# megvii-research/basedet

Hardware: AMD Instinct MI355X
Metric: images/sec training RetinaNet-R50-FPN 1333x800 (higher is better)
Workload: dtype bf16; 1 GPU; retinanet_r50_800x1344 train step (fwd+bwd+allreduce+SGD), DummyLoader boxes, random-init weights, inputs resident in HBM; per_gpu_batch=16, global_batch=16, parallelism=dp1

## Files before the change

### basedet_amd/_lib.py

```python
import ctypes as C
import os

import torch

_HERE = os.path.dirname(os.path.abspath(__file__))
LIB_PATH = os.environ.get("BASEDET_HIP_LIB") or os.path.join(_HERE, "lib", "libbasedet_hip.so")

BD_MAX_SEGS = 8
ABI_VERSION = 106
EPI_RELU, EPI_ADD_BEFORE, EPI_ADD_AFTER, EPI_MASK, EPI_SPARSE = 1, 2, 4, 8, 16


class BasedetHipError(RuntimeError):
    pass


class ConvDesc(C.Structure):
    _fields_ = [
        ("N", C.c_int32), ("Cin", C.c_int32), ("Cout", C.c_int32), ("R", C.c_int32), ("S", C.c_int32),
        ("stride", C.c_int32), ("pad", C.c_int32), ("nseg", C.c_int32),
        ("Hi", C.c_int32 * BD_MAX_SEGS), ("Wi", C.c_int32 * BD_MAX_SEGS),
        ("Ho", C.c_int32 * BD_MAX_SEGS), ("Wo", C.c_int32 * BD_MAX_SEGS),
        ("in_off", C.c_int32 * BD_MAX_SEGS), ("out_off", C.c_int32 * BD_MAX_SEGS),
        ("in_pix_per_img", C.c_int32), ("out_pix_per_img", C.c_int32),
        ("route", C.c_int32 * 4), ("sr_seed", C.c_uint32),
        ("gskip", C.c_int32), ("gskip_ws", C.c_void_p), ("gskip_ws_bytes", C.c_size_t),
        ("gskip_gmap", C.c_void_p), ("gskip_gmap_bytes", C.c_size_t), ("gskip_dxmap", C.c_void_p), ("gskip_dxmap_bytes", C.c_size_t),
        ("gskip_dx_clean", C.c_int32),
    ]


class PackDesc(C.Structure):
    _fields_ = [("w", C.c_void_p), ("row_scale", C.c_void_p), ("w_fwd", C.c_void_p), ("w_dgrad", C.c_void_p),
                ("Cout", C.c_int32), ("RS", C.c_int32), ("Cin", C.c_int32), ("block_start", C.c_int32)]


class ImageDesc(C.Structure):
    _fields_ = [("offset", C.c_int64), ("src_h", C.c_int32), ("src_w", C.c_int32), ("dst_h", C.c_int32), ("dst_w", C.c_int32),
                ("flip", C.c_int32), ("reserved_", C.c_int32 * 1)]


_P, _I, _L, _F, _Z = C.c_void_p, C.c_int, C.c_int64, C.c_float, C.c_size_t
_D = C.POINTER(ConvDesc)

SIGNATURES = {
    "bd_last_error_string": (C.c_char_p, []),
    "bd_version": (_I, []),
    "bd_conv_last_kernel": (C.c_char_p, []),
    "bd_probe_mfma_rate": (_I, [C.c_double, C.POINTER(C.c_double), C.POINTER(C.c_double), _P]),
    "bd_probe_kernel_clock": (_I, [C.c_char_p, _I, C.POINTER(C.c_double), C.POINTER(C.c_double)]),
    "bd_conv2d_fwd": (_I, [_D, _P, _P, _P, _P, _P, _I, _P]),
    "bd_conv2d_dgrad": (_I, [_D, _P, _P, _P, _P, _P, _I, _P]),
    "bd_conv2d_dgrad_gskip_bytes": (_Z, [_D]),
    "bd_conv2d_gskip_map_bytes": (_Z, [_D, _I]),
    "bd_gskip_map_scan": (_I, [_D, _I, _P, _P, _Z, _P]),
    "bd_conv2d_fwd_bits": (_I, [_D, _P, _P, _P, _P, _P, _P, _I, _P]),
    "bd_conv2d_fwd_ex": (_I, [_D, _P, _P, _P, _P, _P, _P, _P, _F, _I, _P]),
    "bd_conv2d_dgrad_ex": (_I, [_D, _P, _P, _P, _P, _P, _P, _P, _F, _I, _P]),
    "bd_conv2d_dgrad_bits": (_I, [_D, _P, _P, _P, _P, _P, _I, _P]),
    "bd_conv2d_wgrad_workspace_bytes": (_Z, [_D]),
    "bd_conv2d_wgrad": (_I, [_D, _P, _P, _P, _P, _I, _P, _Z, _P]),
    "bd_conv2d_wgrad_bias_workspace_bytes": (_Z, [_D]),
    "bd_conv2d_wgrad_bias": (_I, [_D, _P, _P, _P, _P, _P, _I, _P, _Z, _P]),
    "bd_fpn_deconv_pack": (_I, [_P, _I, _P, _P, _P]),
    "bd_fpn_deconv_fwd": (_I, [_P, _P, _P, _P, _I, _I, _I, _I, _I, _I, _P]),
    "bd_fpn_deconv_dgrad": (_I, [_P, _P, _P, _P, _I, _I, _I, _I, _I, _I, _P]),
    "bd_fpn_deconv_wgrad_workspace_bytes": (_Z, [_I, _I, _I, _I]),
    "bd_fpn_deconv_wgrad": (_I, [_P, _P, _P, _I, _P, _Z, _I, _I, _I, _I, _I, _I, _P]),
    "bd_wgrad_queue_create": (_I, [_P]),
    "bd_wgrad_queue_destroy": (_I, [_P]),
    "bd_wgrad_queue_pending": (_I, [_P]),
    "bd_conv2d_wgrad_queued": (_I, [_P, _D, _P, _P, _P, _P, _P, _I, _P, _Z, _P]),
    "bd_wgrad_queue_flush": (_I, [_P, _P]),
    "bd_stem_conv7x7_fwd": (_I, [_I, _I, _I, _P, _P, _P, _P, _P]),
    "bd_stem_pool_fwd": (_I, [_I, _I, _I, _P, _P, _P, _P, _P]),
    "bd_stem_weight_pack": (_I, [_P, _P, _P, _P]),
    "bd_weight_pack": (_I, [_P, _P, _P, _P, _I, _I, _I, _P]),
    "bd_weight_pack_blocks": (_I, [_I, _I, _I]),
    "bd_weight_pack_multi": (_I, [_P, _I, _I, _P]),
    "bd_colsum_workspace_bytes": (_Z, [_I]),
    "bd_colsum_bf16": (_I, [_P, _I, _L, _L, _L, _I, _P, _I, _P, _Z, _P]),
    "bd_pad_normalize": (_I, [_P, _I, _I, _I, _I, _I, _P, _P, _P, _P]),
    "bd_bottleneck_fwd_supported": (_I, [_I, _I, _I, _I, _I, _I, _I]),
    "bd_bottleneck_fwd": (_I, [_I, _I, _I, _I, _I, _I, _P, _P, _P, _P, _P, _P, _P, _P, _P, _P, _P]),
    "bd_h2d_create": (_I, [C.POINTER(C.c_void_p), _I, _I]),
    "bd_h2d_threads": (_I, [_P]),
    "bd_h2d_submit": (_I, [_P, _P, _I, _L, _P, _L, _P]),
    "bd_h2d_destroy": (_I, [_P]),
    "bd_pad_normalize_nchw": (_I, [_P, _I, _I, _I, _I, _I, _P, _P, _P, _P]),
    "bd_resize_pad_normalize": (_I, [_P, _L, C.POINTER(ImageDesc), _I, _I, _I, _P, _P, _P, _P]),
    "bd_maxpool3x3s2_fwd": (_I, [_P, _I, _I, _I, _I, _P, _P]),
    "bd_upsample2x_add_fwd": (_I, [_P, _L, _L, _P, _L, _L, _I, _I, _I, _I, _P]),
    "bd_upsample2x_add_bwd": (_I, [_P, _L, _L, _P, _L, _L, _I, _I, _I, _I, _I, _P]),
    "bd_relu_bf16": (_I, [_P, _P, _L, _P]),
    "bd_relu_bwd_bf16": (_I, [_P, _P, _P, _P, _L, _P]),
    "bd_add_bf16": (_I, [_P, _P, _P, _L, _P]),
    "bd_anchors_generate": (_I, [_I, _I, _I, _F, _P, _I, _P, _P]),
    "bd_points_generate": (_I, [_I, _I, _I, _F, _I, _P, _P]),
    "bd_box_pairwise": (_I, [_P, _I, _P, _I, _I, _P, _P]),
    "bd_box_encode": (_I, [_P, _P, _L, _P, _P, _P, _P]),
    "bd_box_decode": (_I, [_P, _P, _L, _P, _P, _P, _P]),
    "bd_retina_assign_encode": (_I, [_P, _I, _P, _P, _I, _I, _F, _F, _I, _P, _P, _P, _P, _P, _P, _P, _Z, _P]),
    "bd_fcos_assign": (_I, [_P, _I, _P, _P, _P, _I, _F, _P, _P, _I, _I, _P, _P, _P, _P, _P]),
    "bd_ota_assign_workspace_bytes": (_Z, [_I, _I]),
    "bd_ota_assign": (_I, [_P, _I, _P, _P, _I, _P, _I, _P, _P, _P, _I, _I, _F, _F, _F, _F, _I, _P, _P, _P, _P, _P, _Z, _P]),
    "bd_ota_assign_ld": (_I, [_P, _I, _P, _P, _I, _P, _I, _I, _P, _P, _P, _I, _I, _F, _F, _F, _F, _I, _P, _P, _P, _P, _P, _Z, _P]),
    "bd_ota_sinkhorn_workspace_bytes": (_Z, [_I, _I, _I]),
    "bd_ota_assign_sinkhorn": (_I, [_P, _I, _P, _P, _I, _P, _I, _P, _P, _P, _I, _I, _F, _F, _F, _F, _I, _F, _I, _P, _P, _P, _P, _P, _Z, _P]),
    "bd_ota_assign_sinkhorn_ld": (_I, [_P, _I, _P, _P, _I, _P, _I, _I, _P, _P, _P, _I, _I, _F, _F, _F, _F, _I, _F, _I, _P, _P, _P, _P, _P, _Z, _P]),
    "bd_freeanchor_workspace_bytes": (_Z, [_I, _I, _I, _I]),
    "bd_freeanchor_loss_fwd_bwd": (_I, [_P, _P, _I, _I, _P, _I, _I, _P, _P, _I, _I, _P, _P, _F, _I, _F, _F, _F, _F, _P, _P, _P, _P, _Z, _P]),
    "bd_freeanchor_loss_fwd_bwd_ld": (_I, [_P, _I, _P, _I, _I, _P, _I, _I, _P, _P, _I, _I, _P, _P, _F, _I, _F, _F, _F, _F, _P, _P, _P, _P, _Z, _P]),
    "bd_atss_assign_workspace_bytes": (_Z, [_I, _I]),
    "bd_atss_assign": (_I, [_P, _I, _P, _P, _I, _I, _F, _P, _P, _I, _I, _P, _P, _P, _P, _P, _Z, _P]),
    "bd_nms_workspace_bytes": (_Z, [_I]),
    "bd_batched_nms": (_I, [_P, _P, _P, _I, _F, _I, _P, _P, _P, _Z, _P]),
    "bd_focal_loss_fwd_bwd": (_I, [_P, _P, _L, _I, _F, _F, _P, _I, _F, _P, _P, _P]),
    "bd_focal_loss_fwd_bwd_general": (_I, [_P, _P, _L, _I, _F, _F, _P, _I, _F, _P, _P, _P]),
    "bd_focal_loss_fwd_bwd_ld": (_I, [_P, _P, _L, _I, _I, _F, _F, _P, _I, _F, _P, _P, _I, _P]),
    "bd_smooth_l1_fwd_bwd": (_I, [_P, _P, _P, _L, _I, _I, _F, _P, _I, _F, _P, _P, _P]),
    "bd_loss_grid_cap": (_I, []),
    "bd_iou_ltrb_fwd_bwd": (_I, [_P, _P, _P, _P, _L, _I, _P, _F, _P, _P, _P]),
    "bd_giou_ltrb_fwd_bwd": (_I, [_P, _P, _P, _P, _L, _P, _F, _P, _P, _P]),
    "bd_bce_logits_fwd_bwd": (_I, [_P, _I, _I, _P, _P, _L, _P, _P, _P, _P]),
    "bd_groupnorm_workspace_bytes": (_Z, [_I, _I, _I, _L]),
    "bd_groupnorm_fwd": (_I, [_P, _P, _P, _I, _I, _P, _P, _L, _I, _F, _I, _P, _P, _P, _Z, _P]),
    "bd_conv2d_fwd_gnstats_bytes": (_Z, [_D]),
    "bd_conv2d_fwd_gnstats": (_I, [_D, _P, _P, _P, _P, _P, _Z, _P]),
    "bd_groupnorm_fwd_parts": (_I, [_D, _P, _P, _P, _P, _F, _I, _P, _P, _P]),
    "bd_groupnorm_bwd": (_I, [_P, _P, _P, _P, _P, _I, _I, _P, _P, _L, _I, _I, _P, _P, _P, _I, _P, _Z, _P]),
    "bd_fcos_offsets_fwd": (_I, [_P, _I, _P, _I, _I, _P, _P, _P, _L, _P, _P]),
    "bd_fcos_offsets_workspace_bytes": (_Z, []),
    "bd_fcos_offsets_bwd": (_I, [_P, _I, _P, _I, _I, _P, _P, _P, _L, _P, _P, _P, _P, _P, _Z, _P]),
    "bd_rpn_assign_encode": (_I, [_P, _I, _P, _P, _I, _I, _F, _F, _I, _P, _P, _P, _P, _P, _P, _P, _Z, _P]),
    "bd_sample_labels": (_I, [_P, _P, _P, _I, _I, _I, _I, _P, _P]),
    "bd_segment_topk": (_I, [_P, _I, _I, _L, _I, _I, _I, _I, _P, _P, _I, _F, _I, _P, _P, _P, _P]),
    "bd_nms_batched_workspace_bytes": (_Z, [_I, _I]),
    "bd_nms_batched": (_I, [_P, _P, _P, _I, _I, _F, _I, _I, _P, _P, _P, _Z, _P]),
    "bd_rpn_proposals_workspace_bytes": (_Z, [_I, _I, _P, _I, _I, _I]),
    "bd_rpn_proposals": (_I, [_P, _I, _I, _I, _I, _I, _L, _I, _P, _P, _P, _P, _I, _P, _P, _I, _F, _I, _P, _P, _P, _Z, _P]),
    "bd_rpn_proposals_joint": (_I, [_P, _I, _I, _I, _I, _I, _L, _I, _P, _P, _P, _P, _I, _P, _P, _I, _F, _I, _P, _P, _P, _Z, _P]),
    "bd_rcnn_sample_targets": (_I, [_P, _P, _I, _P, _P, _I, _I, _P, _P, _I, _I, _I, _F, _F, _F, _P, _P, _P, _P, _P, _P, _P, _P]),
    "bd_roi_align_fwd": (_I, [_P, _L, _I, _I, _P, _P, _P, _P, _P, _P, _I, _I, _I, _I, _I, _P, _P]),
    "bd_conv1x1_thin_bwd_workspace_bytes": (_Z, []),
    "bd_conv1x1_thin_fwd": (_I, [_P, _P, _P, _L, _I, _I, _P, _P]),
    "bd_conv1x1_thin_bwd": (_I, [_P, _P, _P, _L, _I, _I, _P, _P, _P, _I, _P, _Z, _P]),
    "bd_roi_align_bwd": (_I, [_P, _L, _I, _I, _P, _P, _P, _P, _P, _P, _I, _I, _I, _I, _I, _P, _P]),
    "bd_roi_align_bwd_bf16_workspace_bytes": (_Z, [_I, _I, _P, _P, _I]),
    "bd_roi_align_bwd_bf16": (_I, [_P, _L, _I, _I, _I, _P, _P, _P, _P, _P, _P, _I, _I, _I, _I, _I, _P, _I, _P, _Z, _P]),
    "bd_roi_pool_fwd": (_I, [_P, _L, _I, _I, _P, _P, _P, _P, _P, _P, _I, _I, _I, _I, _P, _P]),
    "bd_roi_pool_bwd_bf16_workspace_bytes": (_Z, [_I, _I, _P, _P, _I]),
    "bd_roi_pool_bwd_bf16": (_I, [_P, _P, _L, _I, _I, _I, _P, _P, _P, _P, _P, _P, _I, _I, _I, _I, _P, _I, _P, _Z, _P]),
    "bd_subsample2x_fwd": (_I, [_P, _L, _L, _I, _I, _P, _L, _L, _I, _I, _P]),
    "bd_subsample2x_bwd_add": (_I, [_P, _L, _L, _P, _L, _L, _I, _I, _I, _I, _P]),
    "bd_f32_to_bf16": (_I, [_P, _P, _L, _P]),
    "bd_f32_to_bf16_add": (_I, [_P, _P, _L, _P]),
    "bd_rpn_loss_fwd_bwd": (_I, [_P, _I, _I, _I, _I, _P, _P, _L, _F, _P, _P, _P, _P]),
    "bd_rcnn_loss_fwd_bwd": (_I, [_P, _I, _I, _I, _P, _P, _I, _F, _P, _P, _P, _P]),
    "bd_det_scores": (_I, [_P, _P, _I, _I, _L, _I, _P, _P]),
    "bd_det_scores_ld": (_I, [_P, _I, _P, _I, _I, _L, _I, _P, _P]),
    "bd_det_select_workspace_bytes": (_Z, [_I, _I, _L, _I, _I]),
    "bd_det_select": (_I, [_P, _P, _I, _I, _I, _L, _I, _I, _P, _P, _I, _F, _P, _P, _P, _P, _Z, _P]),
    "bd_det_select_ld": (_I, [_P, _I, _P, _I, _I, _I, _L, _I, _I, _P, _P, _I, _F, _P, _P, _P, _P, _Z, _P]),
    "bd_rcnn_predict": (_I, [_P, _I, _I, _I, _P, _P, _I, _I, _P, _P, _P, _P, _P]),
    "bd_det_candidates": (_I, [_I, _P, _P, _P, _I, _I, _P, _I, _P, _P, _I, _I, _P, _P, _P, _P, _P, _P, _P]),
    "bd_det_finalize": (_I, [_P, _P, _P, _P, _P, _I, _P, _P, _P, _P, _P]),
    "bd_det_candidates_batched": (_I, [_I, _P, _P, _P, _I, _I, _I, _P, _I, _P, _P, _L, _I, _I, _P, _P, _P, _L, _P, _P, _P, _P]),
    "bd_det_finalize_batched": (_I, [_P, _P, _P, _P, _P, _I, _I, _I, _P, _I, _P, _P, _P, _P]),
    "bd_sgd_momentum_step": (_I, [_P, _P, _P, _L, _F, _F, _F, _F, _P]),
    "bd_ema_update": (_I, [_P, _P, _L, _F, _F, _P]),
    "bd_sgd_momentum_ema_step": (_I, [_P, _P, _P, _P, _L, _F, _F, _F, _F, _F, _F, _P]),
    "bd_swap_f32": (_I, [_P, _P, _L, _P]),
    "bd_adam_step": (_I, [_P, _P, _P, _P, _L] + [_F] * 10 + [_I, _P]),
    "bd_adam_ema_step": (_I, [_P, _P, _P, _P, _P, _L] + [_F] * 10 + [_I, _F, _F, _P]),
    "bd_sgd_nesterov_step": (_I, [_P, _P, _P, _L, _F, _F, _F, _F, _P]),
    "bd_sgd_nesterov_ema_step": (_I, [_P, _P, _P, _P, _L, _F, _F, _F, _F, _F, _F, _P]),
    "bd_clip_grad_value": (_I, [_P, _L, _F, _F, _F, _P]),
    "bd_clip_grad_norm_workspace_bytes": (_Z, []),
    "bd_clip_grad_norm": (_I, [_P, _L, _F, _F, _F, _P, _P, _Z, _P]),
    "bd_quantize_fp8": (_I, [_P, _L, _F, _P, _P]),
    "bd_weight_pack_fp8": (_I, [_P, _P, _I, _I, _I, _F, _P, _P, _P]),
    "bd_conv2d_fwd_fp8": (_I, [_D, _P, _P, _P, _P, _P, _P, _I, _P]),
    "bd_conv2d_fwd_fp8_ex": (_I, [_D, _P, _P, _P, _P, _P, _P, _P, _F, _I, _P]),
    "bd_quantize_bf8": (_I, [_P, _L, _F, _P, C.c_uint32, _P]),
    "bd_absmax_bf16": (_I, [_P, _L, _P, _P]),
    "bd_weight_pack_fp8_t": (_I, [_P, _P, _I, _I, _I, _F, _P, _P, _P]),
    "bd_conv2d_dgrad_fp8": (_I, [_D, _P, _P, _P, _P, _P, _P, _P, _F, _I, _P]),
    "bd_conv2d_wgrad_fp8_workspace_bytes": (_Z, [_D]),
    "bd_conv2d_wgrad_fp8": (_I, [_D, _P, _P, _F, _P, _P, _I, _P, _Z, _P]),
    "bd_conv1x1_fp8": (_I, [_D, _I, _P, _P, _P, _P, _P, _P, _P, _P, _P, _P, _F, _I, _P]),
    "bd_sigmoid_focal_loss_elem": (_I, [_P, _P, _L, _F, _F, _P, _P, _P, _P]),
    "bd_bce_elem": (_I, [_P, _P, _L, _I, _P, _P, _P, _P]),
    "bd_smooth_l1_elem": (_I, [_P, _P, _L, _F, _P, _P, _P, _P]),
    "bd_iou_loss_ltrb": (_I, [_P, _P, _L, _I, _F, _P, _P, _P, _P, _P]),
    "bd_iou_to_loss": (_I, [_P, _L, _I, _F, _P, _P]),
    "bd_matcher_matrix": (_I, [_P, _I, _L, _P, _P, _I, _I, _P, _P, _P, _P]),
    "bd_assign_roi_levels": (_I, [_P, _I, _I, _I, _I, _P, _P]),
    "bd_roi_pool_max_fwd": (_I, [_P, _I, _I, _I, _I, _P, _I, _F, _I, _I, _P, _P]),
    "bd_comm_unique_id": (_I, [_P]),
    "bd_comm_init": (_I, [C.POINTER(C.c_void_p), _P, _I, _I, _I]),
    "bd_comm_rank": (_I, [_P]),
    "bd_comm_world": (_I, [_P]),
    "bd_comm_stream": (_P, [_P]),
    "bd_comm_bcast": (_I, [_P, _P, _Z, _I, _I, _P]),
    "bd_comm_allreduce": (_I, [_P, _P, _Z, _I, _I, _P]),
    "bd_comm_allreduce_async": (_I, [_P, _P, _Z, _I, _I, C.POINTER(C.c_void_p), _I]),
    "bd_comm_allreduce_async_bf16": (_I, [_P, _P, _P, _Z, _I, C.POINTER(C.c_void_p), _I]),
    "bd_comm_wait": (_I, [_P, _P]),
# ... 58 lines not shown
```

### basedet_amd/csrc/common.h

```cpp
#pragma once
#include <hip/hip_runtime.h>
#include <stdint.h>
#include <stdio.h>
#include <mutex>
#include <string>

#include "../../include/basedet_hip.h"

typedef unsigned short bf16_raw;
typedef __attribute__((ext_vector_type(8))) __bf16 bf16x8_t;
typedef __attribute__((ext_vector_type(4))) __bf16 bf16x4_t;
typedef __attribute__((ext_vector_type(4))) float f32x4_t;
typedef __attribute__((ext_vector_type(2))) float f32x2_t;
typedef __attribute__((ext_vector_type(4))) short s16x4_t;
typedef __attribute__((ext_vector_type(4))) unsigned int u32x4_t;
typedef __attribute__((ext_vector_type(2))) unsigned int u32x2_t;

__device__ __forceinline__ float bf2f(bf16_raw h) { return __uint_as_float(((uint32_t)h) << 16); }
__device__ __forceinline__ bf16_raw f2bf(float f) {
    __bf16 b = (__bf16)f;
    return __builtin_bit_cast(bf16_raw, b);
}
extern thread_local unsigned g_fp8_sr_seed;
__device__ __forceinline__ unsigned bd_mix32(unsigned x) {
    x ^= x >> 16; x *= 0x7feb352du; x ^= x >> 15; x *= 0x846ca68bu; x ^= x >> 16;
    return x;
}
__device__ __forceinline__ unsigned bd_pack4_e5m2_sr(float a, float b, float c, float d, unsigned r) {
    a = fminf(fmaxf(a, -57344.f), 57344.f); b = fminf(fmaxf(b, -57344.f), 57344.f);
    c = fminf(fmaxf(c, -57344.f), 57344.f); d = fminf(fmaxf(d, -57344.f), 57344.f);
    int v = 0;
    v = __builtin_amdgcn_cvt_sr_bf8_f32(a, r, v, 0);
    v = __builtin_amdgcn_cvt_sr_bf8_f32(b, __builtin_rotateright32(r, 8), v, 1);
    v = __builtin_amdgcn_cvt_sr_bf8_f32(c, __builtin_rotateright32(r, 16), v, 2);
    v = __builtin_amdgcn_cvt_sr_bf8_f32(d, __builtin_rotateright32(r, 24), v, 3);
    return (unsigned)v;
}

__device__ __forceinline__ unsigned pack4_e4m3(float a, float b, float c, float d) {
    a = fminf(fmaxf(a, -448.f), 448.f); b = fminf(fmaxf(b, -448.f), 448.f);
    c = fminf(fmaxf(c, -448.f), 448.f); d = fminf(fmaxf(d, -448.f), 448.f);
    int v = __builtin_amdgcn_cvt_pk_fp8_f32(a, b, 0, false);
    v = __builtin_amdgcn_cvt_pk_fp8_f32(c, d, v, true);
    return (unsigned)v;
}

__device__ __forceinline__ unsigned pack4_e5m2(float a, float b, float c, float d) {
    a = fminf(fmaxf(a, -57344.f), 57344.f); b = fminf(fmaxf(b, -57344.f), 57344.f);
    c = fminf(fmaxf(c, -57344.f), 57344.f); d = fminf(fmaxf(d, -57344.f), 57344.f);
    int v = __builtin_amdgcn_cvt_pk_bf8_f32(a, b, 0, false);
    v = __builtin_amdgcn_cvt_pk_bf8_f32(c, d, v, true);
    return (unsigned)v;
}

__device__ __forceinline__ u32x2_t e5m2_pair(const float* v, float qs, unsigned seed, long long idx) {
    u32x2_t o8;
    if (seed) {
        const unsigned g0 = (unsigned)(idx >> 2);
        const unsigned r0 = bd_mix32(seed ^ g0);
        o8[0] = bd_pack4_e5m2_sr(v[0] * qs, v[1] * qs, v[2] * qs, v[3] * qs, r0);
        o8[1] = bd_pack4_e5m2_sr(v[4] * qs, v[5] * qs, v[6] * qs, v[7] * qs, r0 * 0x9e3779b1u + 0x7f4a7c15u);
    } else {
        o8[0] = pack4_e5m2(v[0] * qs, v[1] * qs, v[2] * qs, v[3] * qs);
        o8[1] = pack4_e5m2(v[4] * qs, v[5] * qs, v[6] * qs, v[7] * qs);
    }
    return o8;
}

__device__ __forceinline__ u32x4_t twin_pair(u32x2_t h0, u32x2_t h1, int cg, int* off) {
    const bool odd = cg & 1;
    const u32x2_t send = odd ? h0 : h1;
    u32x2_t recv;
    recv[0] = (unsigned)__shfl_xor((int)send[0], 16, 64);
    recv[1] = (unsigned)__shfl_xor((int)send[1], 16, 64);
    *off = odd ? 32 + 8 * (cg - 1) : 8 * cg;
    return odd ? (u32x4_t){recv[0], recv[1], h1[0], h1[1]} : (u32x4_t){h0[0], h0[1], recv[0], recv[1]};
}

__device__ __forceinline__ uint32_t pack_bf2(float lo, float hi) {
    return (uint32_t)f2bf(lo) | ((uint32_t)f2bf(hi) << 16);
}
__device__ __forceinline__ float bf_lo(uint32_t u) { return __uint_as_float(u << 16); }
__device__ __forceinline__ float bf_hi(uint32_t u) { return __uint_as_float(u & 0xffff0000u); }

__device__ __forceinline__ float wave_sum(float v) {
#pragma unroll
    for (int o = 32; o > 0; o >>= 1) v += __shfl_xor(v, o, 64);
    return v;
}

__device__ __forceinline__ float ema_elem(float e, float w, float m, float one_minus_m) {
#pragma clang fp contract(off)
    const float a = e * m;
    const float b = one_minus_m * w;
    return a + b;
}

__device__ __forceinline__ void bd_clk_mark(unsigned long long* acc, bool end) {
#ifdef BD_NO_CLK_PROBE
    return;
#endif
    const unsigned long long c = __builtin_amdgcn_s_memtime(), r = __builtin_amdgcn_s_memrealtime();
    atomicAdd(acc, end ? c : 0ull - c);
    atomicAdd(acc + 1, end ? r : 0ull - r);
}

#define BD_KNOB thread_local
struct BdRouteScope {
    int rc;
    explicit BdRouteScope(const bd_conv_desc* d);
};
#define BD_ROUTE(d)                                   \
    BdRouteScope route_scope__(d);                    \
    if (route_scope__.rc != BD_OK) return route_scope__.rc

void bd_set_error(const char* fmt, ...);
void bd_note_kernel(const char* name);

#define BD_REQUIRE(cond, ...)            \
    do {                                 \
        if (!(cond)) {                   \
            bd_set_error(__VA_ARGS__);   \
            return BD_EINVAL;            \
        }                                \
    } while (0)

#define BD_CHECK_LAUNCH(name)                                                     \
    do {                                                                          \
        hipError_t e__ = hipGetLastError();                                       \
        if (e__ != hipSuccess) {                                                  \
            bd_set_error("%s: launch failed: %s", name, hipGetErrorString(e__)); \
            return BD_ELAUNCH;                                                    \
        }                                                                         \
    } while (0)

#ifdef BD_TUNING
#include <stdlib.h>
static inline int bd_tune_env(const char* name, int dflt) { const char* e = getenv(name); return e ? atoi(e) : dflt; }
static inline const char* bd_tune_env_str(const char* name) { return getenv(name); }
#else
static inline int bd_tune_env(const char*, int dflt) { return dflt; }
static inline const char* bd_tune_env_str(const char*) { return nullptr; }
#endif

struct BdGskipMap { int p4, p8, m4, m8, live, list; size_t ints; };
void bd_gskip_map_layout(const bd_conv_desc* d, int side, BdGskipMap* out);

static inline int grid_for(long long n, int block = 256, int cap = 4096) {
    long long g = (n + block - 1) / block;
    if (g < 1) g = 1;
    return (int)(g < cap ? g : cap);
}
static inline int64_t cdiv64(int64_t a, int64_t b) { return (a + b - 1) / b; }
static inline int cdiv(int a, int b) { return (a + b - 1) / b; }

struct BdDeviceOnce {
    std::mutex mu;
    unsigned long long done[4] = {0, 0, 0, 0};
    struct Guard {
        BdDeviceOnce& o; int dev = 0; bool first_;
        explicit Guard(BdDeviceOnce& o_) : o(o_) {
            o.mu.lock();
            if (hipGetDevice(&dev) != hipSuccess || dev < 0 || dev > 255) dev = 0;
            first_ = !((o.done[dev >> 6] >> (dev & 63)) & 1ull);
        }
        bool first() const { return first_; }
        ~Guard() { if (first_) o.done[dev >> 6] |= 1ull << (dev & 63); o.mu.unlock(); }
    };
};
#define BD_ONCE_PER_DEVICE(...)                 \
    do {                                        \
        static BdDeviceOnce once__;             \
        BdDeviceOnce::Guard guard__(once__);    \
        if (guard__.first()) { __VA_ARGS__; }   \
    } while (0)
int bd_num_cus();
```

### basedet_amd/csrc/conv3x3_pp.hip

```cpp
#include "conv3x3_pp128_body.h"

namespace {

constexpr int PH = 4, PW = 16, IH = PH + 2, IW = PW + 2;
constexpr int NPATCH = 4;
constexpr int XROWS = NPATCH * IH * IW;
constexpr int X_PITCH = 144;
constexpr int X_BYTES = XROWS * X_PITCH;
constexpr int XPASSES = 7;
constexpr int TILE_CO = 256;
constexpr int W_SLOT = TILE_CO * 128;
constexpr int NSLOT = 3;
constexpr int W_BYTES = NSLOT * W_SLOT;
constexpr int GTAB_TILES = 16;
constexpr int GTAB_BYTES = GTAB_TILES * NPATCH * 32;
constexpr int LDS_BYTES = W_BYTES + X_BYTES + TILE_CO * 4 + GTAB_BYTES;
constexpr int MAX_SEG = BD_MAX_SEGS;
constexpr int TAIL_CO = 64;

struct PSeg { int patch_start, H, W, pw, src_off, dst_off; float inv_pw; };

struct PParams {
    const bf16_raw* src;
    const bf16_raw* w;
    const float* bias;
    const bf16_raw* add;
    const bf16_raw* mask;
    bf16_raw* dst;
    int CK, CO, flags, nseg;
    int src_ppi, dst_ppi;
    unsigned src_bytes;
    int patches_per_img, total_patches, n_tiles;
    int main_grid;
    int px_tiles;
    int tail_end;
    float inv_ppi;
    PSeg seg[MAX_SEG];
    float* gn_part;
    const int* sp_live;
    const int* sp_list;
    const int* sp_count;
    int sp_keep_dead;
    const int* sp_hdr;
    int* sp_ohdr;
    const int* sp_olist;
    int sp_stride, sp_clean;
};

typedef __attribute__((address_space(3))) void lds_void_t;
typedef __attribute__((address_space(1))) const void glb_void_t;

__device__ __forceinline__ int pp_div(int n, int d, float inv) {
    int q = (int)((float)n * inv);
    const int r = n - q * d;
    q += (r >= d) - (r < 0);
    return q;
}

__device__ __forceinline__ int swz(int row, int chunk) { return row * 128 + ((chunk ^ (row & 7)) << 4); }
__device__ __forceinline__ int colperm(int f) { return f < 4 ? 2 * f : (f < 12 ? 2 * (f - 4) + 1 : 2 * (f - 8)); }
__device__ __forceinline__ int xpos(int chunk) { return (chunk >> 2) * 64 + ((((chunk & 1) << 1) | ((chunk >> 1) & 1)) << 4); }

#ifdef BD_PP_STAMP
__device__ unsigned long long g_pp_stamp[64];
__device__ unsigned long long g_pp_span[2048];
#endif
#ifndef BD_PP_ABLATE
#define BD_PP_ABLATE 0
#endif
__device__ unsigned long long g_pp_clk[2];
#define PP_FENCE() __builtin_amdgcn_sched_barrier(0)
#define PP_BARRIER() do { asm volatile("" ::: "memory"); __builtin_amdgcn_s_barrier(); asm volatile("" ::: "memory"); } while (0)

template <int MODE, bool GNS = false, bool SPARSE = false>
__global__ __launch_bounds__(512, 1) void conv3x3_pp_kernel(const PParams p) {
    extern __shared__ __attribute__((aligned(16))) unsigned char smem[];
    if (!SPARSE && (int)blockIdx.x >= p.main_grid) {
        pp128::body<MODE, TAIL_CO>(p, smem, (int)blockIdx.x - p.main_grid, (int)gridDim.x - p.main_grid, p.total_patches, p.tail_end,
                                   (p.CO + TAIL_CO - 1) / TAIL_CO);
        return;
    }
    if (!SPARSE && blockIdx.x == 0 && threadIdx.x == 0) bd_clk_mark(g_pp_clk, false);
    unsigned char* wbuf = smem;
    unsigned char* xbuf = smem + W_BYTES;
    float* sbias = reinterpret_cast<float*>(smem + W_BYTES + X_BYTES);

#ifdef BD_PP_STAMP
    int st_n = 0;
    const bool st_on = blockIdx.x == 100 % gridDim.x && threadIdx.x == 0;
#define PP_STAMP() do { if (st_on && st_n < 62) g_pp_stamp[st_n] = __builtin_amdgcn_s_memtime(); ++st_n; } while (0)
    PP_STAMP();
    if (st_on) g_pp_stamp[62] = __builtin_amdgcn_s_memrealtime();
    if (threadIdx.x == 0 && blockIdx.x < 1024) g_pp_span[2 * blockIdx.x] = __builtin_amdgcn_s_memrealtime();
#else
#define PP_STAMP() do { } while (0)
#endif
    const int tid = threadIdx.x, lane = tid & 63, wave = __builtin_amdgcn_readfirstlane(tid >> 6);
    const int wm = wave >> 2, wp = wave & 3;
    int bid = blockIdx.x;
    {
        const int nwg = p.main_grid;
        const int q = nwg >> 3, r = nwg & 7, xcd = bid & 7;
        bid = (xcd < r ? xcd * (q + 1) : r * (q + 1) + (xcd - r) * q) + (bid >> 3);
    }
    const int ct = bid % p.n_tiles;
    int pt = bid / p.n_tiles;
    const int pt_step = p.main_grid / p.n_tiles;
    const int co0 = ct * TILE_CO;

    auto zero_dead = [&](int z0, int zn) {
        if (p.sp_keep_dead) return;
        const int cpp = p.CO >> 3;
        const int items = PH * PW * cpp;
        int zt = p.total_patches;
        const int* plist = nullptr;
        if (p.sp_clean) {
            const int oc = __builtin_amdgcn_readfirstlane(p.sp_ohdr[0]) & 1;
            const int pc = __builtin_amdgcn_readfirstlane(p.sp_ohdr[2 + oc]);
            zt = pc < 0 ? 0 : (pc < zt ? pc : zt);
            plist = p.sp_olist + oc * p.sp_stride;
        }
        for (int k0 = 0; z0 + k0 * zn < zt; k0 += 512) {
            const int k = k0 + wave * 64 + lane;
            const int idx = z0 + k * zn;
            int q = idx;
            if (plist) q = idx < zt ? plist[idx] : -1;
            const bool dead = idx < zt && q >= 0 && q < p.total_patches && p.sp_live[q] == 0;
            unsigned long long m = __ballot(dead);
            while (m) {
                const int l = __builtin_ctzll(m);
                m &= m - 1;
                const int qq = __builtin_amdgcn_readfirstlane(__shfl(q, l, 64));
                const int n = qq / p.patches_per_img, rem = qq - n * p.patches_per_img;
                int sgi = 0;
#pragma unroll
                for (int z = 1; z < MAX_SEG; ++z)
                    if (z < p.nseg && rem >= p.seg[z].patch_start) sgi = z;
                const int H = p.seg[sgi].H, W = p.seg[sgi].W, pwn = p.seg[sgi].pw;
                const int local = rem - p.seg[sgi].patch_start, by = local / pwn, bx = local - by * pwn;
                const long long img = (long long)n * p.dst_ppi + p.seg[sgi].dst_off;
                for (int i = lane; i < items; i += 64) {
                    const int px = i / cpp, ch = i - px * cpp;
                    const int y = by * PH + px / PW, x = bx * PW + (px & (PW - 1));
                    if (y < H && x < W)
                        *reinterpret_cast<u32x4_t*>(p.dst + (img + (long long)y * W + x) * p.CO + ch * 8) = (u32x4_t){0u, 0u, 0u, 0u};
                }
            }
        }
    };
    int n_px = p.px_tiles, n_live = p.total_patches;
    int z_first = 0;
    const int* sp_list = p.sp_list;
    if constexpr (SPARSE) {
        if (p.sp_ohdr && blockIdx.x == 0 && threadIdx.x == 0) p.sp_ohdr[1] = 0;
        const int cur = p.sp_hdr ? __builtin_amdgcn_readfirstlane(p.sp_hdr[0]) & 1 : 0;
        const int* cntp = p.sp_hdr ? p.sp_hdr + 2 + cur : p.sp_count;
        n_live = __builtin_amdgcn_readfirstlane(*cntp);
        sp_list += cur * p.sp_stride;
        n_live = __builtin_amdgcn_readfirstlane(n_live < 0 ? 0 : (n_live < p.total_patches ? n_live : p.total_patches));
        n_px = (n_live + NPATCH - 1) / NPATCH;
        z_first = n_px * p.n_tiles < p.main_grid ? n_px * p.n_tiles : p.main_grid;
        if (pt >= n_px) {
            zero_dead(bid - z_first, p.main_grid - z_first);
            return;
        }
    }

    constexpr unsigned X_NONE = 0x80000000u;
    const int x_lds0 = (tid >> 3) * X_PITCH + xpos(tid & 7);
    unsigned x_off[XPASSES];

    int* gtab = reinterpret_cast<int*>(smem + W_BYTES + X_BYTES + TILE_CO * 4);
    const int pt_first = pt;
    auto build_table = [&](int k0) {
        const int k = k0 + (lane >> 2);
        const int ptile = pt_first + k * pt_step;
        int pid = ptile * NPATCH + (lane & (NPATCH - 1));
        if (SPARSE) pid = (ptile < n_px && pid < n_live) ? sp_list[pid] : p.total_patches;
        int vH = 0, vW = 0, vy = 0, vx = 0, vs = 0, vd = 0;
        if (ptile < n_px && pid < p.total_patches) {
            const int n = pp_div(pid, p.patches_per_img, p.inv_ppi);
            const int rem = pid - n * p.patches_per_img;
            int g_start = p.seg[0].patch_start, g_H = p.seg[0].H, g_W = p.seg[0].W, g_pw = p.seg[0].pw;
            int g_src = p.seg[0].src_off, g_dst = p.seg[0].dst_off;
            float g_inv = p.seg[0].inv_pw;
#pragma unroll
            for (int q = 1; q < MAX_SEG; ++q) {
                const bool in = q < p.nseg && rem >= p.seg[q].patch_start;
                g_start = in ? p.seg[q].patch_start : g_start; g_H = in ? p.seg[q].H : g_H; g_W = in ? p.seg[q].W : g_W;
                g_pw = in ? p.seg[q].pw : g_pw; g_src = in ? p.seg[q].src_off : g_src; g_dst = in ? p.seg[q].dst_off : g_dst;
                g_inv = in ? p.seg[q].inv_pw : g_inv;
            }
            const int local = rem - g_start;
            const int by = pp_div(local, g_pw, g_inv), bx = local - by * g_pw;
            vy = by * PH; vx = bx * PW; vH = g_H; vW = g_W;
            vs = n * p.src_ppi + g_src;
            vd = n * p.dst_ppi + g_dst;
        }
        typedef __attribute__((ext_vector_type(4))) int i32x4_t;
        i32x4_t* e = reinterpret_cast<i32x4_t*>(gtab + ((k & (GTAB_TILES - 1)) * NPATCH + (lane & (NPATCH - 1))) * 8);
        e[0] = (i32x4_t){vy, vx, vH, vW};
        e[1] = (i32x4_t){vs, vd, 0, 0};
    };
    auto decode = [&](int k, int& e_oy0, int& e_px0, int& e_H, int& e_W, int& e_dst) {
        int py0[NPATCH], px0[NPATCH], pH[NPATCH], pWd[NPATCH];
        int psrc[NPATCH], pdst[NPATCH];
        int tq = tid;
        asm volatile("" : "+v"(tq));
        {
            typedef __attribute__((ext_vector_type(4))) int i32x4_t;
            const i32x4_t* e = reinterpret_cast<const i32x4_t*>(gtab + ((k & (GTAB_TILES - 1)) * NPATCH + (tq & (NPATCH - 1))) * 8);
            const i32x4_t e0 = e[0], e1 = e[1];
#pragma unroll
            for (int q = 0; q < NPATCH; ++q) {
                py0[q] = __builtin_amdgcn_readlane(e0[0], q); px0[q] = __builtin_amdgcn_readlane(e0[1], q);
                pH[q] = __builtin_amdgcn_readlane(e0[2], q); pWd[q] = __builtin_amdgcn_readlane(e0[3], q);
                psrc[q] = __builtin_amdgcn_readlane(e1[0], q); pdst[q] = __builtin_amdgcn_readlane(e1[1], q);
            }
        }
#pragma unroll
        for (int k = 0; k < XPASSES; ++k) {
            const int row = (tq >> 3) + 64 * k;
            unsigned off = X_NONE;
            if (row < XROWS) {
                const int lo = (64 * k) / (IH * IW), hi = (64 * k + 63) / (IH * IW) < NPATCH ? (64 * k + 63) / (IH * IW) : NPATCH - 1;
                const bool up = row >= hi * (IH * IW);
                const int pk = up ? hi : lo;
                const int rr = row - pk * (IH * IW);
                const int iy = rr / IW, ix = rr - iy * IW;
                const int qy = up ? py0[hi] : py0[lo], qx = up ? px0[hi] : px0[lo], H = up ? pH[hi] : pH[lo];
                const int W = up ? pWd[hi] : pWd[lo], qs = up ? psrc[hi] : psrc[lo];
                const int y = qy - 1 + iy, x = qx - 1 + ix;
                if (y >= 0 && x >= 0 && y < H && x < W) off = (unsigned)((qs + y * W + x) * p.CK + (tq & 7) * 8) * 2u;
            }
            x_off[k] = off;
        }
        e_oy0 = py0[0]; e_px0 = px0[0]; e_H = pH[0]; e_W = pWd[0]; e_dst = pdst[0];
#pragma unroll
        for (int q = 1; q < NPATCH; ++q)
            if (wp == q) { e_oy0 = py0[q]; e_px0 = px0[q]; e_H = pH[q]; e_W = pWd[q]; e_dst = pdst[q]; }
    };
    int c_oy0, c_px0, c_H, c_W, c_dst;
    int kt = 0;
    if (wave == 0) build_table(0);
    asm volatile("s_waitcnt lgkmcnt(0)" ::: "memory");
    PP_BARRIER();
    decode(0, c_oy0, c_px0, c_H, c_W, c_dst);
    const __amdgpu_buffer_rsrc_t x_rsrc =
        __builtin_amdgcn_make_buffer_rsrc(const_cast<bf16_raw*>(p.src), 0, p.src_bytes, 0x00020000);
    u32x4_t rx[XPASSES];
    auto load_x = [&](int cb) {
        int so = cb * 128;
        asm volatile("" : "+s"(so));
        const bool dead = cb * 64 + (tid & 7) * 8 >= p.CK;
#pragma unroll
        for (int k = 0; k < XPASSES; ++k) rx[k] = __builtin_amdgcn_raw_buffer_load_b128(x_rsrc, dead ? X_NONE : x_off[k], so, 0);
    };
    auto write_x = [&]() {
#pragma unroll
        for (int k = 0; k < XPASSES; ++k)
            if (k < XPASSES - 1 || (tid >> 3) + 64 * k < XROWS)
                *reinterpret_cast<u32x4_t*>(xbuf + x_lds0 + k * (64 * X_PITCH)) = rx[k];
    };

    unsigned dma_src[4];
#pragma unroll
    for (int k = 0; k < 4; ++k) {
        const int pc = wave + 8 * k;
        const int lrow = 8 * pc + (lane >> 3);
        const int chunk = (lane & 7) ^ (lane >> 3);
        const int rho = lrow & 15;
        int co = co0 + (lrow & 192) + 32 * ((lrow >> 5) & 1) + 8 * (rho >> 2) + 4 * ((lrow >> 4) & 1) + (rho & 3);
        if (co >= p.CO) co = p.CO - 1;
        dma_src[k] = (unsigned)(co * 9 * p.CK + chunk * 8) * 2u;
    }
    const __amdgpu_buffer_rsrc_t w_rsrc =
        __builtin_amdgcn_make_buffer_rsrc(const_cast<bf16_raw*>(p.w), 0, (unsigned)(p.CO * 9 * p.CK) * 2u, 0x00020000);
    bool dma_on = true;
    auto dma_piece = [&](int tap, int cb, int slot, int k) {
        if ((BD_PP_ABLATE & 2) && !dma_on) return;
        unsigned char* l = wbuf + slot * W_SLOT + (wave + 8 * k) * 1024;
        int so = (tap * p.CK + cb * 64) * 2;
        asm volatile("" : "+s"(so));
        __builtin_amdgcn_raw_ptr_buffer_load_lds(w_rsrc, (lds_void_t*)l, 16, dma_src[k], so, 0, 0);
    };

    f32x4_t acc[8][4];

    const int frow = lane & 15, fchunk = lane >> 4;
    const unsigned char* a_base[2];
#pragma unroll
    for (int kk = 0; kk < 2; ++kk) a_base[kk] = wbuf + swz(wm * 128 + frow, kk * 4 + fchunk);
    typedef __attribute__((address_space(3))) const unsigned char lds_u8_t;
    typedef __attribute__((address_space(3))) const bf16x8_t lds_bf16x8_t;
    unsigned a_hi[2];
#pragma unroll
    for (int kk = 0; kk < 2; ++kk) {
        a_hi[kk] = (unsigned)(size_t)(lds_u8_t*)(a_base[kk]) + 2 * W_SLOT;
        asm volatile("" : "+v"(a_hi[kk]));
    }
    const unsigned char* b_base = xbuf + (wp * (IH * IW) + colperm(frow)) * X_PITCH + xpos(fchunk);

    bf16x8_t fa[8], fb[4];
    auto load_a = [&](int kk, int slot) {
#pragma unroll
        for (int i = 0; i < 8; ++i) {
            if (slot == 2) fa[i] = *(lds_bf16x8_t*)(size_t)(a_hi[kk] + i * 2048);
// ... 194 lines not shown
                PP_STAMP();
                if (more) asm volatile("s_waitcnt vmcnt(4)" ::: "memory");
                else asm volatile("s_waitcnt vmcnt(0)" ::: "memory");
                PP_STAMP();
                PP_FENCE();
#pragma unroll
                for (int j = 0; j < 4; ++j) {
                    if (BD_PP_ABLATE & 4) asm volatile("" :: "v"(o0[j]));
                    else if (okh && okj[j]) *reinterpret_cast<u32x4_t*>(drow[j]) = o0[j];
                }
            } else {
#pragma unroll
                for (int j = 0; j < 4; ++j) {
                    const u32x4_t o = unit(h, j, b0, b1);
                    if (BD_PP_ABLATE & 4) asm volatile("" :: "v"(o));
                    else if (okh && okj[j]) *reinterpret_cast<u32x4_t*>(drow[j] + 32 * h) = o;
                }
            }
        }
        if constexpr (GNS) {
            const int pid = pt * NPATCH + wp;
#pragma unroll
            for (int h = 0; h < 4; ++h) {
                float a = gsum[h], b = gsq[h];
#pragma unroll
                for (int m = 8; m >= 1; m >>= 1) { a += __shfl_xor(a, m, 64); b += __shfl_xor(b, m, 64); }
                if (erow == 0 && pid < p.total_patches && cbase + 32 * h < p.CO) {
                    float* o = p.gn_part + ((long long)pid * 32 + ((cbase + 32 * h) >> 3)) * 2;
                    *reinterpret_cast<f32x2_t*>(o) = (f32x2_t){a, b};
                }
            }
        }
    } else {
    if (more) {
#pragma unroll
        for (int k = 0; k < 4; ++k) dma_piece(2, 0, 2, k);
    }
    long long erow_off[4];
#pragma unroll
    for (int j = 0; j < 4; ++j) erow_off[j] = (long long)(dbase + (oy0 + j) * W + ox) * p.CO + cbase;
#pragma unroll
    for (int hp = 0; hp < 2; ++hp) {
        u32x4_t av[2][4], mv[2][4];
#pragma unroll
        for (int hh = 0; hh < 2; ++hh) {
            const int h = 2 * hp + hh;
#pragma unroll
            for (int j = 0; j < 4; ++j) {
                const int oy = oy0 + j;
                const bool ok = cbase + 32 * h < p.CO && oy < H && ox < W;
                const long long idx = erow_off[j] + 32 * h;
                av[hh][j] = (u32x4_t){0u, 0u, 0u, 0u}; mv[hh][j] = (u32x4_t){0u, 0u, 0u, 0u};
                if (ok && (add_before || add_after)) av[hh][j] = *reinterpret_cast<const u32x4_t*>(p.add + idx);
                if (ok && do_mask) mv[hh][j] = *reinterpret_cast<const u32x4_t*>(p.mask + idx);
            }
        }
        if (hp == 0) asm volatile("s_waitcnt vmcnt(0)" ::: "memory");
#pragma unroll
        for (int hh = 0; hh < 2; ++hh) {
            const int h = 2 * hp + hh;
            if (cbase + 32 * h >= p.CO) continue;
            float bias[8];
            {
                const f32x4_t b0 = *reinterpret_cast<const f32x4_t*>(sbias + wm * 128 + 8 * cg + 32 * h);
                const f32x4_t b1 = *reinterpret_cast<const f32x4_t*>(sbias + wm * 128 + 8 * cg + 32 * h + 4);
#pragma unroll
                for (int k = 0; k < 4; ++k) { bias[k] = b0[k]; bias[4 + k] = b1[k]; }
            }
#pragma unroll
            for (int j = 0; j < 4; ++j) {
                const int oy = oy0 + j;
                if (oy >= H || ox >= W) continue;
                const long long idx = erow_off[j] + 32 * h;
                float v[8];
#pragma unroll
                for (int k = 0; k < 8; ++k) v[k] = acc[2 * h + (k >> 2)][j][k & 3] + bias[k];
                const u32x4_t a4 = av[hh][j], m4 = mv[hh][j];
                if (add_before) {
#pragma unroll
                    for (int k = 0; k < 4; ++k) { v[2 * k] += bf_lo(a4[k]); v[2 * k + 1] += bf_hi(a4[k]); }
                }
                if (do_relu) {
#pragma unroll
                    for (int k = 0; k < 8; ++k) v[k] = fmaxf(v[k], 0.f);
                }
                if (do_mask) {
#pragma unroll
                    for (int k = 0; k < 4; ++k) {
                        if (!(bf_lo(m4[k]) > 0.f)) v[2 * k] = 0.f;
                        if (!(bf_hi(m4[k]) > 0.f)) v[2 * k + 1] = 0.f;
                    }
                }
                if (add_after) {
#pragma unroll
                    for (int k = 0; k < 4; ++k) { v[2 * k] += bf_lo(a4[k]); v[2 * k + 1] += bf_hi(a4[k]); }
                }
                u32x4_t o;
#pragma unroll
                for (int k = 0; k < 4; ++k) o[k] = pack_bf2(v[2 * k], v[2 * k + 1]);
                *reinterpret_cast<u32x4_t*>(p.dst + idx) = o;
            }
        }
    }
    }
    PP_STAMP();
    if (!more) break;
    ++kt;
    pt = pt_next;
    c_oy0 = n_oy0; c_px0 = n_px0; c_H = n_H; c_W = n_W; c_dst = n_dst;
    PP_FENCE();
    PP_STAMP();
    }
    if constexpr (SPARSE) {
        if (z_first == p.main_grid) zero_dead(bid, p.main_grid);
    }
    if (!SPARSE && blockIdx.x == 0 && threadIdx.x == 0) bd_clk_mark(g_pp_clk, true);
#ifdef BD_PP_STAMP
    if (st_on) { g_pp_stamp[63] = __builtin_amdgcn_s_memrealtime(); g_pp_stamp[61] = __builtin_amdgcn_s_memtime(); }
    if (threadIdx.x == 0 && blockIdx.x < 1024) { asm volatile("s_waitcnt vmcnt(0)" ::: "memory"); g_pp_span[2 * blockIdx.x + 1] = __builtin_amdgcn_s_memrealtime(); }
#endif
}

}

BD_KNOB int g_pp_tail_split = 1;
BD_KNOB int g_pp_persistent = 1;
extern BD_KNOB int g_patch_pp;
int bd_gskip_patches(const bd_conv_desc* d, int ph, int pw);
void bd_gskip_fill(const bd_conv_desc* d, int side, const void* t, const int* live_in, int* map, hipStream_t stream);
void bd_gskip_scan(const bd_conv_desc* d, const void* g, int ph, int pw, int* mask, hipStream_t stream);
void bd_gskip_compact(const bd_conv_desc* d, int ph, int pw, const int* mask, int* live, int* list, int* count, hipStream_t stream);

extern "C" size_t bd_conv2d_dgrad_gskip_bytes(const bd_conv_desc* d) {
    if (!d || d->nseg < 1 || d->nseg > BD_MAX_SEGS || !(d->R == 3 && d->S == 3 && d->stride == 1 && d->pad == 1)) return 0;
    return ((size_t)3 * bd_gskip_patches(d, PH, PW) + 4) * sizeof(int);
}

static bool pp_sparse_epilogue(int flags, const void* add, const void* dst) {
    const bool in_place = (flags & BD_EPI_ADD_BEFORE) && add && add == dst;
    return !(flags & BD_EPI_ADD_AFTER) && (!((flags & BD_EPI_ADD_BEFORE) && add) || (in_place && !(flags & BD_EPI_MASK)));
}

bool bd_conv3x3_pp_maps_ok(const bd_conv_desc* d, int flags, const void* add, const void* dst) {
    if (g_patch_pp < 2 || !(d->R == 3 && d->S == 3 && d->stride == 1 && d->pad == 1)) return false;
    if (d->Cout % 8 != 0 || d->Cin <= 128 || d->Cin % 8 != 0) return false;
    if ((long long)d->N * d->out_pix_per_img * d->Cout * 2 >= 0x7fffffffll || (long long)d->N * d->in_pix_per_img >= 0x7fffffffll ||
        (long long)d->Cin * 9 * d->Cout >= 0x7fffffffll) return false;
    for (int s = 0; s < d->nseg; ++s)
        if (d->Hi[s] != d->Ho[s] || d->Wi[s] != d->Wo[s]) return false;
    if (bd_gskip_patches(d, PH, PW) >= (1 << 24)) return false;
    const bool in_place = (flags & BD_EPI_ADD_BEFORE) && add && add == dst;
    if (d->gskip_dxmap && in_place) return false;
    return pp_sparse_epilogue(flags, add, dst);
}

static int pp_launch(const bd_conv_desc* d, int mode, const void* src, const void* w, const float* bias, const void* add,
                     const void* mask, void* dst, int flags, float* gn_part, hipStream_t stream) {
    PParams p{};
    p.gn_part = gn_part;
    p.CK = mode == 0 ? d->Cin : d->Cout;
    p.CO = mode == 0 ? d->Cout : d->Cin;
    p.src_ppi = mode == 0 ? d->in_pix_per_img : d->out_pix_per_img;
    p.dst_ppi = mode == 0 ? d->out_pix_per_img : d->in_pix_per_img;
    if (p.CK % 8 != 0 || p.CO <= 128 || p.CO % 8 != 0) return 1;
    if ((long long)d->N * p.src_ppi * p.CK * 2 >= 0x7fffffffll || (long long)d->N * p.dst_ppi >= 0x7fffffffll ||
        (long long)p.CO * 9 * p.CK >= 0x7fffffffll) return 1;
    p.src = (const bf16_raw*)src; p.w = (const bf16_raw*)w; p.bias = bias;
    p.add = (const bf16_raw*)add; p.mask = (const bf16_raw*)mask; p.dst = (bf16_raw*)dst;
    p.flags = flags; p.nseg = d->nseg;
    p.src_bytes = (unsigned)((long long)d->N * p.src_ppi * p.CK * 2);
    int ps = 0;
    for (int s = 0; s < d->nseg; ++s) {
        PSeg& sg = p.seg[s];
        sg.patch_start = ps; sg.H = d->Ho[s]; sg.W = d->Wo[s]; sg.pw = cdiv(d->Wo[s], PW); sg.inv_pw = 1.0f / (float)sg.pw;
        sg.src_off = mode == 0 ? d->in_off[s] : d->out_off[s];
        sg.dst_off = mode == 0 ? d->out_off[s] : d->in_off[s];
        ps += cdiv(d->Ho[s], PH) * sg.pw;
    }
    p.patches_per_img = ps;
    p.inv_ppi = 1.0f / (float)ps;
    p.total_patches = ps * d->N;
    if (p.total_patches >= (1 << 24)) return 1;
    p.n_tiles = cdiv(p.CO, TILE_CO);
    int grid = cdiv(p.total_patches, NPATCH) * p.n_tiles;
    int tail_wgs = 0;
    int px_tiles = cdiv(p.total_patches, NPATCH);
    p.tail_end = p.total_patches;
    const int num_cus = bd_num_cus();
    const bool in_place = (flags & BD_EPI_ADD_BEFORE) && add && add == dst;
    const bool sparse = mode == 1 && d->gskip && !gn_part && pp_sparse_epilogue(flags, add, dst);
    if (g_pp_tail_split && !sparse && !gn_part && p.n_tiles == 1 && px_tiles > num_cus) {
        const int r = px_tiles % num_cus;
        if (r > 0 && r * (TILE_CO / TAIL_CO) <= num_cus) {
            px_tiles -= r;
            p.total_patches = px_tiles * NPATCH;
            tail_wgs = cdiv(p.tail_end - p.total_patches, NPATCH) * cdiv(p.CO, TAIL_CO);
        }
    }
    p.px_tiles = px_tiles;
    p.main_grid = px_tiles * p.n_tiles;
    if (g_pp_persistent) {
        const int g1 = (num_cus / p.n_tiles) * p.n_tiles;
        const int rounds = cdiv(px_tiles * p.n_tiles, g1 * GTAB_TILES);
        if (g1 * rounds < p.main_grid) p.main_grid = g1 * rounds;
    }
    {
        const int grid128 = cdiv(p.total_patches, NPATCH) * cdiv(p.CO, 128);
        if (!gn_part && g_patch_pp < 2 && 3 * cdiv(grid, 256) >= 2 * cdiv(grid128, 256)) return 1;
    }
    BD_ONCE_PER_DEVICE(
        (void)hipFuncSetAttribute(reinterpret_cast<const void*>(&conv3x3_pp_kernel<0>), hipFuncAttributeMaxDynamicSharedMemorySize, LDS_BYTES);
        (void)hipFuncSetAttribute(reinterpret_cast<const void*>(&conv3x3_pp_kernel<1>), hipFuncAttributeMaxDynamicSharedMemorySize, LDS_BYTES);
        (void)hipFuncSetAttribute(reinterpret_cast<const void*>(&conv3x3_pp_kernel<1, false, true>), hipFuncAttributeMaxDynamicSharedMemorySize,
                                  LDS_BYTES));
    bd_note_kernel("conv3x3_pp_kernel");
    if (sparse) {
        const int tot = p.total_patches;
        p.sp_keep_dead = in_place ? 1 : 0;
        p.sp_stride = tot;
        if (d->gskip_gmap) {
            BdGskipMap gm;
            bd_gskip_map_layout(d, 0, &gm);
            const int* m = (const int*)d->gskip_gmap;
            p.sp_hdr = m; p.sp_live = m + gm.live; p.sp_list = m + gm.list;
        } else {
            int* mk = (int*)d->gskip_ws;
            p.sp_live = mk + tot; p.sp_list = mk + 2 * tot; p.sp_count = mk + 3 * tot;
            bd_gskip_scan(d, src, PH, PW, mk, stream);
            bd_gskip_compact(d, PH, PW, mk, mk + tot, mk + 2 * tot, mk + 3 * tot, stream);
        }
        if (d->gskip_dxmap) {
            BdGskipMap xm;
            bd_gskip_map_layout(d, 1, &xm);
            p.sp_ohdr = (int*)d->gskip_dxmap; p.sp_olist = p.sp_ohdr + xm.list;
            p.sp_clean = d->gskip_dx_clean ? 1 : 0;
        }
        hipLaunchKernelGGL((conv3x3_pp_kernel<1, false, true>), dim3(p.main_grid), dim3(512), LDS_BYTES, stream, p);
        if (d->gskip_dxmap) bd_gskip_fill(d, 1, dst, p.sp_live, (int*)d->gskip_dxmap, stream);
    } else if (gn_part) {
        BD_ONCE_PER_DEVICE((void)hipFuncSetAttribute(reinterpret_cast<const void*>(&conv3x3_pp_kernel<0, true>), hipFuncAttributeMaxDynamicSharedMemorySize, LDS_BYTES));
        hipLaunchKernelGGL((conv3x3_pp_kernel<0, true>), dim3(p.main_grid), dim3(512), LDS_BYTES, stream, p);
    } else if (mode == 0) hipLaunchKernelGGL((conv3x3_pp_kernel<0>), dim3(p.main_grid + tail_wgs), dim3(512), LDS_BYTES, stream, p);
    else hipLaunchKernelGGL((conv3x3_pp_kernel<1>), dim3(p.main_grid + tail_wgs), dim3(512), LDS_BYTES, stream, p);
    return 0;
}

int bd_pp_clk_read(unsigned long long* out2, int reset) {
    if (hipMemcpyFromSymbol(out2, HIP_SYMBOL(g_pp_clk), 16) != hipSuccess) return 1;
    if (reset) { const unsigned long long z[2] = {0, 0}; if (hipMemcpyToSymbol(HIP_SYMBOL(g_pp_clk), z, 16) != hipSuccess) return 1; }
    return 0;
}

#ifdef BD_PP_STAMP
extern "C" int bd_debug_pp_stamp(unsigned long long* out2) {
    return hipMemcpyFromSymbol(out2, HIP_SYMBOL(g_pp_stamp), 512) == hipSuccess ? 0 : 1;
}
extern "C" int bd_debug_pp_span(unsigned long long* out2048) {
    return hipMemcpyFromSymbol(out2048, HIP_SYMBOL(g_pp_span), 2048 * 8) == hipSuccess ? 0 : 1;
}
#endif

int bd_conv3x3_pp_launch(const bd_conv_desc* d, int mode, const void* src, const void* w, const float* bias, const void* add,
                         const void* mask, void* dst, int flags, hipStream_t stream) {
    return pp_launch(d, mode, src, w, bias, add, mask, dst, flags, nullptr, stream);
}

int bd_conv3x3_pp_patch_starts(const bd_conv_desc* d, int* starts) {
    int ps = 0;
    for (int s = 0; s < d->nseg; ++s) { starts[s] = ps; ps += cdiv(d->Ho[s], PH) * cdiv(d->Wo[s], PW); }
    starts[d->nseg] = ps;
    return ps;
}

extern "C" size_t bd_conv2d_fwd_gnstats_bytes(const bd_conv_desc* d) {
    if (!d || d->nseg < 1 || d->nseg > BD_MAX_SEGS) return 0;
    int starts[BD_MAX_SEGS + 1];
    return (size_t)d->N * bd_conv3x3_pp_patch_starts(d, starts) * 32 * 2 * sizeof(float);
}

extern "C" int bd_conv2d_fwd_gnstats(const bd_conv_desc* d, const void* x, const void* w_packed, const float* bias, void* y, float* part,
                                     size_t part_bytes, bd_stream_t stream) {
    BD_ROUTE(d);
    BD_REQUIRE(d && x && w_packed && y && part, "conv2d_fwd_gnstats: null pointer");
    BD_REQUIRE(d->R == 3 && d->S == 3 && d->stride == 1 && d->pad == 1 && d->Cout == 256 && d->Cin % 64 == 0,
               "conv2d_fwd_gnstats: 3x3 / stride 1 / pad 1 into 256 channels (GroupNorm(32, 256)) only; got %dx%d s%d p%d %d -> %d", d->R, d->S,
               d->stride, d->pad, d->Cin, d->Cout);
    for (int s = 0; s < d->nseg; ++s)
        BD_REQUIRE(d->Hi[s] == d->Ho[s] && d->Wi[s] == d->Wo[s], "conv2d_fwd_gnstats: level %d changes size", s);
    if (part_bytes < bd_conv2d_fwd_gnstats_bytes(d)) { bd_set_error("conv2d_fwd_gnstats: statistics buffer too small"); return BD_EWORKSPACE; }
    if (pp_launch(d, 0, x, w_packed, bias, nullptr, nullptr, y, 0, part, (hipStream_t)stream) != 0) {
        bd_set_error("conv2d_fwd_gnstats: shape not taken by conv3x3_pp_kernel (tensor too large for 32-bit offsets?)");
        return BD_EINVAL;
    }
    BD_CHECK_LAUNCH("bd_conv2d_fwd_gnstats");
    return BD_OK;
}
```

### basedet_amd/csrc/conv_igemm.hip

```cpp
#include "igemm_params.h"

using namespace igemm;

namespace {

template <int BK>
struct Cfg {
    static constexpr int CHUNKS = BK / 8;
    static constexpr int ROWS_PER_PASS = 256 / CHUNKS;
    static constexpr int PASSES = 128 / ROWS_PER_PASS;
    static constexpr int LDS_STRIDE = BK == 64 ? 160 : 64;
    static constexpr int TILE_BYTES = 128 * LDS_STRIDE;
    __device__ static __forceinline__ int off(int row, int chunk) {
        if constexpr (BK == 64) return row * LDS_STRIDE + chunk * 16;
        else return row * 64 + ((chunk ^ ((row >> 1) & 3)) << 4);
    }
};

template <int BK, bool PRE, bool BUF>
__global__ __launch_bounds__(256) void conv_igemm_kernel(const IgemmParams p) {
    using C = Cfg<BK>;
    extern __shared__ __attribute__((aligned(16))) unsigned char smem[];
    unsigned char* tiles = smem;
    unsigned int* s_tapmask = reinterpret_cast<unsigned int*>(smem);
// ... 234 lines not shown
    }
    __syncthreads();
    int cur = 0;
    for (int t = 0; t < nsteps; ++t) {
        const bool more = (t + 1 < nsteps);
        if (more) stage_load();
        compute(cur);
        if (more) stage_write(cur ^ 1);
        __syncthreads();
        cur ^= 1;
    }

    const int cg = lane >> 4;
    const bool do_relu = p.flags & BD_EPI_RELU;
    const bool add_before = (p.flags & BD_EPI_ADD_BEFORE) && p.add;
    const bool add_after = (p.flags & BD_EPI_ADD_AFTER) && p.add;
    const bool do_mask = (p.flags & BD_EPI_MASK) && p.mask;
    const int cbase = co0 + wc * 64 + 8 * cg;
    float bias[16];
#pragma unroll
    for (int k = 0; k < 16; ++k) bias[k] = 0.f;
    if (p.bias) {
#pragma unroll
        for (int q = 0; q < 4; ++q)
            if (cbase + 32 * (q >> 1) + 4 * (q & 1) < p.CO) {
                const f32x4_t bv = *reinterpret_cast<const f32x4_t*>(p.bias + cbase + 32 * (q >> 1) + 4 * (q & 1));
                bias[4 * q] = bv[0]; bias[4 * q + 1] = bv[1]; bias[4 * q + 2] = bv[2]; bias[4 * q + 3] = bv[3];
            }
    }
#pragma unroll
    for (int j = 0; j < 4; ++j) {
        const int m = m0 + wp * 64 + j * 16 + (lane & 15);
        if (m >= p.M) continue;
        int dstpix;
        if (p.linear_dst) dstpix = m;
        else {
            int s = 0;
#pragma unroll
            for (int k = 1; k < MAX_SUB; ++k)
                if (k < p.nsub && m >= p.sub[k].m_start) s = k;
            const SubSeg ss = p.sub[s];
            const int local = m - ss.m_start;
            int n, rem, yy, xx;
            fast_divmod(local, ss.Hs * ss.Ws, ss.inv_per_img, n, rem);
            fast_divmod(rem, ss.Ws, ss.inv_ws, yy, xx);
            dstpix = n * p.dst_pix_per_img + ss.dst_off + (ss.y0 + ss.step * yy) * ss.Wd + ss.x0 + ss.step * xx;
        }
        const long long base = (long long)dstpix * p.CO + cbase;
#pragma unroll
        for (int half = 0; half < 2; ++half) {
            if (cbase + 32 * half >= p.CO) continue;
            const long long idx = base + 32 * half;
            float v[8];
#pragma unroll
            for (int k = 0; k < 8; ++k) v[k] = acc[2 * half + (k >> 2)][j][k & 3] + bias[8 * half + k];
            if (add_before) {
                const u32x4_t av = PRE ? pre_add[j * 2 + half] : *reinterpret_cast<const u32x4_t*>(p.add + idx);
#pragma unroll
                for (int k = 0; k < 4; ++k) { v[2 * k] += bf_lo(av[k]); v[2 * k + 1] += bf_hi(av[k]); }
            }
            if (do_relu) {
#pragma unroll
                for (int k = 0; k < 8; ++k) v[k] = fmaxf(v[k], 0.f);
            }
            if (do_mask) {
                const u32x4_t mv = PRE ? pre_mask[j * 2 + half] : *reinterpret_cast<const u32x4_t*>(p.mask + idx);
#pragma unroll
                for (int k = 0; k < 4; ++k) {
                    if (!(bf_lo(mv[k]) > 0.f)) v[2 * k] = 0.f;
                    if (!(bf_hi(mv[k]) > 0.f)) v[2 * k + 1] = 0.f;
                }
            }
            if (add_after) {
                const u32x4_t av = PRE ? pre_add[j * 2 + half] : *reinterpret_cast<const u32x4_t*>(p.add + idx);
#pragma unroll
                for (int k = 0; k < 4; ++k) { v[2 * k] += bf_lo(av[k]); v[2 * k + 1] += bf_hi(av[k]); }
            }
            u32x4_t o;
#pragma unroll
            for (int k = 0; k < 4; ++k) o[k] = pack_bf2(v[2 * k], v[2 * k + 1]);
            *reinterpret_cast<u32x4_t*>(p.dst + idx) = o;
        }
    }
}

BD_KNOB int g_igemm_prefetch_epi = 1;
BD_KNOB int g_igemm_buf = 1;

template <int BK>
int launch_igemm(const IgemmParams& p, hipStream_t stream) {
    using C = Cfg<BK>;
    const size_t lds = 4 * C::TILE_BYTES;
    BD_ONCE_PER_DEVICE(
        (void)hipFuncSetAttribute(reinterpret_cast<const void*>(&conv_igemm_kernel<BK, false, false>),
                                  hipFuncAttributeMaxDynamicSharedMemorySize, (int)lds);
        (void)hipFuncSetAttribute(reinterpret_cast<const void*>(&conv_igemm_kernel<BK, true, false>),
                                  hipFuncAttributeMaxDynamicSharedMemorySize, (int)lds);
        (void)hipFuncSetAttribute(reinterpret_cast<const void*>(&conv_igemm_kernel<BK, false, true>),
                                  hipFuncAttributeMaxDynamicSharedMemorySize, (int)lds);
        (void)hipFuncSetAttribute(reinterpret_cast<const void*>(&conv_igemm_kernel<BK, true, true>),
                                  hipFuncAttributeMaxDynamicSharedMemorySize, (int)lds));
    const int grid = p.m_tiles * p.n_tiles;
    bd_note_kernel(BK == 32 ? "conv_igemm_kernel<32>" : "conv_igemm_kernel<64>");
    const bool epi_ops = ((p.flags & (BD_EPI_ADD_BEFORE | BD_EPI_ADD_AFTER)) && p.add) || ((p.flags & BD_EPI_MASK) && p.mask);
    const int ksteps = (p.CK + BK - 1) / BK * p.R * p.S;
    const bool pre = g_igemm_prefetch_epi && p.linear_dst && epi_ops && ksteps <= 4;
    const bool buf = g_igemm_buf && p.src_bytes != 0 && p.w_bytes != 0;
    if (pre && buf) hipLaunchKernelGGL((conv_igemm_kernel<BK, true, true>), dim3(grid), dim3(256), lds, stream, p);
    else if (pre) hipLaunchKernelGGL((conv_igemm_kernel<BK, true, false>), dim3(grid), dim3(256), lds, stream, p);
    else if (buf) hipLaunchKernelGGL((conv_igemm_kernel<BK, false, true>), dim3(grid), dim3(256), lds, stream, p);
    else hipLaunchKernelGGL((conv_igemm_kernel<BK, false, false>), dim3(grid), dim3(256), lds, stream, p);
    return 0;
}

int check_desc(const bd_conv_desc* d) {
    BD_REQUIRE(d != nullptr, "conv: null descriptor");
    BD_REQUIRE(d->nseg >= 1 && d->nseg <= BD_MAX_SEGS, "conv: nseg=%d out of range", d->nseg);
    BD_REQUIRE(d->N >= 1 && d->Cin >= 1 && d->Cout >= 1, "conv: bad N/Cin/Cout");
    BD_REQUIRE(d->stride == 1 || d->stride == 2, "conv: stride %d unsupported (1 or 2)", d->stride);
    BD_REQUIRE(d->R * d->S <= 32, "conv: %dx%d kernel unsupported by the generic path", d->R, d->S);
    for (int s = 0; s < d->nseg; ++s) {
        BD_REQUIRE((d->Hi[s] + 2 * d->pad - d->R) / d->stride + 1 == d->Ho[s] &&
                   (d->Wi[s] + 2 * d->pad - d->S) / d->stride + 1 == d->Wo[s],
                   "conv: level %d output size inconsistent with input/stride/pad", s);
    }
    return 0;
}

void set_buffer_sizes(IgemmParams& p, int N) {
    const long long sb = (long long)N * p.src_pix_per_img * p.CK * 2, wb = (long long)p.CO * p.R * p.S * p.CK * 2;
    p.src_bytes = (sb > 0 && sb < 0x7fffffffll) ? (unsigned)sb : 0u;
    p.w_bytes = (wb > 0 && wb < 0x7fffffffll) ? (unsigned)wb : 0u;
}

bool is_3x3s1(const bd_conv_desc* d) {
    if (!(d->R == 3 && d->S == 3 && d->stride == 1 && d->pad == 1)) return false;
    for (int s = 0; s < d->nseg; ++s)
        if (d->Hi[s] != d->Ho[s] || d->Wi[s] != d->Wo[s]) return false;
    return true;
}
BD_KNOB int g_use_patch3x3 = 1;
#ifdef BD_AB_SKIP
BD_KNOB int g_skip_s2_3x3 = 0;
#endif
BD_KNOB int g_bk32_for_1x1 = 1;
BD_KNOB int g_bk32_s2 = 1;

}


int bd_conv3x3_patch_launch(const bd_conv_desc* d, int mode, const void* src, const void* w, const float* bias,
                            const void* add, const void* mask, void* dst, int flags, hipStream_t stream);
bool bd_conv3x3_pp_maps_ok(const bd_conv_desc* d, int flags, const void* add, const void* dst);

extern BD_KNOB int g_patch_dma;
extern BD_KNOB int g_patch_pp;
extern BD_KNOB int g_patch_pp128;
extern BD_KNOB int g_conv1x1_s2;
extern BD_KNOB int g_pp_tail_split;
extern BD_KNOB int g_pp_persistent;
static int bd_route_patch3x3(int enable) {
#ifdef BD_AB_SKIP
    g_skip_s2_3x3 = (enable >> 4) & 1;
#else
    if ((enable >> 4) & 1) {
        bd_set_error("bd_conv_desc.route[1]: bit 4 (skip the 3x3 / stride-2 launches: a timing A/B that leaves stale outputs) exists in "
                     "-DBD_AB_SKIP diagnostic builds only");
        return BD_EINVAL;
    }
#endif
    g_use_patch3x3 = enable & 1; g_bk32_for_1x1 = (enable >> 1) & 1;
    g_patch_dma = ((enable >> 3) & 1) ^ 1;
    g_patch_pp = ((enable >> 6) & 1) ? 0 : (((enable >> 7) & 1) ? 1 : 2);
    g_patch_pp128 = ((enable >> 9) & 1) ? -1 : ((enable >> 8) & 1);
    g_bk32_s2 = ((enable >> 10) & 1) ^ 1;
    g_igemm_prefetch_epi = ((enable >> 5) & 1) ^ 1;
    g_igemm_buf = ((enable >> 11) & 1) ^ 1;
    g_conv1x1_s2 = ((enable >> 12) & 1) ^ 1;
    g_pp_tail_split = ((enable >> 13) & 1) ^ 1;
    g_pp_persistent = ((enable >> 14) & 1) ^ 1;
    if ((enable >> 16) & 1) {
        bd_set_error("bd_conv_desc.route[1]: bit 16 (conv_igemm_wide.hip) is gone since round 6");
        return BD_EINVAL;
    }
    return BD_OK;
}

int bd_route_dense1x1(int depth);
int bd_route_wgrad(int use_tr);
extern BD_KNOB int g_fp8_patch;

BdRouteScope::BdRouteScope(const bd_conv_desc* d) : rc(BD_OK) {
    const int r0 = d ? d->route[0] : 0, r1 = d ? d->route[1] : 0, r2 = d ? d->route[2] : 0, r3 = d ? d->route[3] : 0;
    if (r0 < 0 || r1 < 0 || r2 < 0 || r3 < 0) {
        bd_set_error("bd_conv_desc.route: negative word (0 = the library's choice, otherwise the route + 1)");
        rc = BD_EINVAL;
        return;
    }
    if ((rc = bd_route_dense1x1(r0 ? r0 - 1 : 1)) != BD_OK) return;
    if ((rc = bd_route_patch3x3(r1 ? r1 - 1 : 3)) != BD_OK) return;
    if ((rc = bd_route_wgrad(r2 ? r2 - 1 : 1)) != BD_OK) return;
    g_fp8_patch = r3 ? (r3 - 1 != 0) : 1;
    g_fp8_sr_seed = d ? d->sr_seed : 0u;
}

int bd_conv1x1_dense_launch(const void* x, const void* w, const float* bias, const void* add, const void* mask, const unsigned* maskbits,
                            void* y, unsigned* ybits, void* y8, float q_scale, int y8_bf8, long long M, int CK, int CO, int flags,
                            hipStream_t stream);

int bd_conv1x1_s2_launch(const bd_conv_desc* d, int mode, const void* src, const void* w, const float* bias, const void* add, const void* mask,
                         const unsigned* maskbits, void* dst, int flags, hipStream_t stream);
namespace {
bool is_dense_1x1(const bd_conv_desc* d) {
    return d->R == 1 && d->S == 1 && d->stride == 1 && d->pad == 0 && d->nseg == 1 && d->in_off[0] == 0 && d->out_off[0] == 0 &&
           d->in_pix_per_img == d->Hi[0] * d->Wi[0] && d->out_pix_per_img == d->Ho[0] * d->Wo[0];
}
}

static int conv2d_fwd_impl(const bd_conv_desc* d, const void* x, const void* w_packed, const float* bias, const void* add, void* y,
                           unsigned* ybits, void* y8, float q_scale, int flags, bd_stream_t stream) {
    if (int e = check_desc(d)) return e;
    BD_REQUIRE(x && w_packed && y, "conv2d_fwd: null pointer");
    BD_REQUIRE(d->Cin % 8 == 0, "conv2d_fwd: Cin=%d must be a multiple of 8", d->Cin);
    BD_REQUIRE(d->Cout % 8 == 0, "conv2d_fwd: Cout=%d must be a multiple of 8", d->Cout);
    BD_REQUIRE(!(flags & BD_EPI_MASK), "conv2d_fwd: BD_EPI_MASK is a dgrad-only flag");
    if (is_dense_1x1(d) &&
        bd_conv1x1_dense_launch(x, w_packed, bias, add, nullptr, nullptr, y, ybits, y8, q_scale, 0, (long long)d->N * d->out_pix_per_img,
                                d->Cin, d->Cout, flags, (hipStream_t)stream) == 0) {
        BD_CHECK_LAUNCH("bd_conv2d_fwd(dense 1x1)");
        return BD_OK;
    }
    if (!ybits && !y8 && d->stride == 2 && d->R == 1 &&
        bd_conv1x1_s2_launch(d, 0, x, w_packed, bias, add, nullptr, nullptr, y, flags, (hipStream_t)stream) == 0) {
        BD_CHECK_LAUNCH("bd_conv2d_fwd(1x1 stride 2)");
        return BD_OK;
    }
    BD_REQUIRE(ybits == nullptr && y8 == nullptr, "conv2d_fwd_bits / _ex: the bit-packed ReLU mask and the e4m3 twin are written by the dense "
               "1x1 kernel only (1x1 / stride 1 over one dense level, Cout %% 32 == 0, tensors < 2 GB)");
#ifdef BD_AB_SKIP
    if (g_skip_s2_3x3 && d->R == 3 && d->S == 3 && d->stride == 2) return BD_OK;
#endif
    if (g_use_patch3x3 && is_3x3s1(d)) {
        bd_conv3x3_patch_launch(d, 0, x, w_packed, bias, add, nullptr, y, flags, (hipStream_t)stream);
        BD_CHECK_LAUNCH("bd_conv2d_fwd(3x3 patch)");
        return BD_OK;
    }
    IgemmParams p{};
    p.src = (const bf16_raw*)x; p.w = (const bf16_raw*)w_packed; p.bias = bias;
    p.add = (const bf16_raw*)add; p.mask = nullptr; p.dst = (bf16_raw*)y;
    p.CK = d->Cin; p.CO = d->Cout; p.R = d->R; p.S = d->S; p.stride = d->stride; p.pad = d->pad;
    p.mode = 0; p.flags = flags;
    p.nsub = d->nseg;
    long long m = 0;
    for (int s = 0; s < d->nseg; ++s) {
        SubSeg& ss = p.sub[s];
        ss.m_start = (int)m;
        ss.Hs = d->Ho[s]; ss.Ws = d->Wo[s]; ss.y0 = 0; ss.x0 = 0; ss.step = 1;
        ss.Wd = d->Wo[s]; ss.dst_off = d->out_off[s];
        ss.Hsrc = d->Hi[s]; ss.Wsrc = d->Wi[s]; ss.src_off = d->in_off[s];
        ss.inv_per_img = 1.0f / (float)(ss.Hs * ss.Ws); ss.inv_ws = 1.0f / (float)ss.Ws;
        m += (long long)d->N * d->Ho[s] * d->Wo[s];
    }
    BD_REQUIRE(m < (1ll << 24), "conv2d_fwd: too many pixels (2^24 limit of the fast index decode)");
    p.linear_dst = (d->nseg == 1 && d->out_off[0] == 0 && d->out_pix_per_img == d->Ho[0] * d->Wo[0]) ? 1 : 0;
    p.linear_src = (p.linear_dst && d->R == 1 && d->S == 1 && d->stride == 1 && d->pad == 0 && d->in_off[0] == 0 &&
                    d->in_pix_per_img == d->Hi[0] * d->Wi[0]) ? 1 : 0;
    p.M = (int)m;
    p.src_pix_per_img = d->in_pix_per_img; p.dst_pix_per_img = d->out_pix_per_img;
    set_buffer_sizes(p, d->N);
    p.m_tiles = cdiv(p.M, TILE_P); p.n_tiles = cdiv(p.CO, TILE_C);
    if (p.CK > 32 && !(g_bk32_for_1x1 && p.R * p.S == 1) && !(g_bk32_s2 && p.stride == 2 && p.m_tiles * p.n_tiles >= 512))
        launch_igemm<64>(p, (hipStream_t)stream);
    else launch_igemm<32>(p, (hipStream_t)stream);
    BD_CHECK_LAUNCH("bd_conv2d_fwd");
    return BD_OK;
}

extern "C" int bd_conv2d_fwd(const bd_conv_desc* d, const void* x, const void* w_packed, const float* bias,
                             const void* add, void* y, int flags, bd_stream_t stream) {
    BD_ROUTE(d);
    return conv2d_fwd_impl(d, x, w_packed, bias, add, y, nullptr, nullptr, 1.f, flags, stream);
}

extern "C" int bd_conv2d_fwd_ex(const bd_conv_desc* d, const void* x, const void* w_packed, const float* bias, const void* add, void* y,
                                uint32_t* ybits, void* y8, float q_scale, int flags, bd_stream_t stream) {
    BD_ROUTE(d);
    return conv2d_fwd_impl(d, x, w_packed, bias, add, y, ybits, y8, q_scale, flags, stream);
}

extern "C" int bd_conv2d_fwd_bits(const bd_conv_desc* d, const void* x, const void* w_packed, const float* bias, const void* add, void* y,
                                  uint32_t* ybits, int flags, bd_stream_t stream) {
    BD_ROUTE(d);
    BD_REQUIRE(ybits != nullptr, "conv2d_fwd_bits: null ybits");
    return conv2d_fwd_impl(d, x, w_packed, bias, add, y, ybits, nullptr, 1.f, flags, stream);
}

static int conv2d_dgrad_impl(const bd_conv_desc* d, const void* g, const void* w_packed_t, const void* add, const void* mask,
                             const unsigned* maskbits, void* dx, void* dx8, float q_scale, int flags, bd_stream_t stream) {
    if (int e = check_desc(d)) return e;
    BD_REQUIRE(g && w_packed_t && dx, "conv2d_dgrad: null pointer");
    if (d->gskip && is_3x3s1(d) && !d->gskip_gmap) {
        const size_t need = bd_conv2d_dgrad_gskip_bytes(d);
        BD_REQUIRE(d->gskip_ws && d->gskip_ws_bytes >= need, "conv2d_dgrad: gskip scratch %zu < required %zu bytes (or NULL)",
                   (size_t)d->gskip_ws_bytes, need);
    }
    if (d->gskip_gmap || d->gskip_dxmap || d->gskip_dx_clean) {
        BD_REQUIRE(d->gskip && is_3x3s1(d) && g_use_patch3x3 && !maskbits && !dx8 && bd_conv3x3_pp_maps_ok(d, flags, add, dx),
                   "conv2d_dgrad: liveness maps need gskip on a 3x3 / stride 1 / pad 1 descriptor into more than 128 channels with an overwriting "
                   "(or, without gskip_dxmap, in-place accumulating) epilogue on the default route");
        BD_REQUIRE(!d->gskip_gmap || d->gskip_gmap_bytes >= bd_conv2d_gskip_map_bytes(d, 0), "conv2d_dgrad: gskip_gmap %zu < required %zu bytes",
                   (size_t)d->gskip_gmap_bytes, bd_conv2d_gskip_map_bytes(d, 0));
        BD_REQUIRE(!d->gskip_dxmap || d->gskip_dxmap_bytes >= bd_conv2d_gskip_map_bytes(d, 1), "conv2d_dgrad: gskip_dxmap %zu < required %zu bytes",
                   (size_t)d->gskip_dxmap_bytes, bd_conv2d_gskip_map_bytes(d, 1));
        BD_REQUIRE(!d->gskip_dx_clean || d->gskip_dxmap, "conv2d_dgrad: gskip_dx_clean needs gskip_dxmap (the list the promise refers to)");
    }
    if (d->stride == 1) flags &= ~BD_EPI_SPARSE;
    BD_REQUIRE(d->Cout % 8 == 0, "conv2d_dgrad: Cout=%d must be a multiple of 8 (pad the gradient)", d->Cout);
    BD_REQUIRE(d->Cin % 8 == 0, "conv2d_dgrad: Cin=%d must be a multiple of 8", d->Cin);
    BD_REQUIRE(!(flags & BD_EPI_RELU), "conv2d_dgrad: BD_EPI_RELU is a forward-only flag");
    if (is_dense_1x1(d) &&
        bd_conv1x1_dense_launch(g, w_packed_t, nullptr, add, mask, maskbits, dx, nullptr, dx8, q_scale, 1, (long long)d->N * d->in_pix_per_img,
                                d->Cout, d->Cin, flags, (hipStream_t)stream) == 0) {
        BD_CHECK_LAUNCH("bd_conv2d_dgrad(dense 1x1)");
        return BD_OK;
    }
    if (!dx8 && d->stride == 2 && d->R == 1 &&
        bd_conv1x1_s2_launch(d, 1, g, w_packed_t, nullptr, add, mask, maskbits, dx, flags, (hipStream_t)stream) == 0) {
        BD_CHECK_LAUNCH("bd_conv2d_dgrad(1x1 stride 2)");
        return BD_OK;
    }
    BD_REQUIRE(maskbits == nullptr && dx8 == nullptr, "conv2d_dgrad_bits / _ex: the bit-packed ReLU mask is read, and the e5m2 twin written, by "
               "the dense 1x1 kernel only (1x1 / stride 1 over one dense level, Cin %% 32 == 0, tensors < 2 GB)");
#ifdef BD_AB_SKIP
    if (g_skip_s2_3x3 && d->R == 3 && d->S == 3 && d->stride == 2) return BD_OK;
#endif
    if (g_use_patch3x3 && is_3x3s1(d)) {
        bd_conv3x3_patch_launch(d, 1, g, w_packed_t, nullptr, add, mask, dx, flags, (hipStream_t)stream);
        BD_CHECK_LAUNCH("bd_conv2d_dgrad(3x3 patch)");
        return BD_OK;
    }
    IgemmParams p{};
    p.src = (const bf16_raw*)g; p.w = (const bf16_raw*)w_packed_t; p.bias = nullptr;
    p.add = (const bf16_raw*)add; p.mask = (const bf16_raw*)mask; p.dst = (bf16_raw*)dx;
    p.CK = d->Cout; p.CO = d->Cin; p.R = d->R; p.S = d->S; p.stride = d->stride; p.pad = d->pad;
    p.mode = 1; p.flags = flags;
    long long m = 0;
    int ns = 0;
    const int st = d->stride;
    const bool sparse = (flags & BD_EPI_SPARSE) && st > 1;
    BD_REQUIRE(!(flags & BD_EPI_SPARSE) || ((flags & BD_EPI_ADD_BEFORE) && add == dx),
               "conv2d_dgrad: BD_EPI_SPARSE needs an in-place accumulate (BD_EPI_ADD_BEFORE with add == dx)");
    p.flags = flags & ~BD_EPI_SPARSE;
    for (int s = 0; s < d->nseg; ++s) {
        for (int qy = 0; qy < st; ++qy)
            for (int qx = 0; qx < st; ++qx) {
                const int Hs = (d->Hi[s] - qy + st - 1) / st, Ws = (d->Wi[s] - qx + st - 1) / st;
                if (Hs <= 0 || Ws <= 0) continue;
                if (sparse) {
                    bool ry = false, rx = false;
                    for (int r = 0; r < d->R; ++r) ry = ry || ((qy + d->pad - r) % st + st) % st == 0;
                    for (int c = 0; c < d->S; ++c) rx = rx || ((qx + d->pad - c) % st + st) % st == 0;
                    if (!(ry && rx)) continue;
                }
                BD_REQUIRE(ns < MAX_SUB, "conv2d_dgrad: too many sub-segments (levels x stride^2 > %d)", MAX_SUB);
                SubSeg& ss = p.sub[ns++];
                ss.m_start = (int)m;
                ss.Hs = Hs; ss.Ws = Ws; ss.y0 = qy; ss.x0 = qx; ss.step = st;
                ss.Wd = d->Wi[s]; ss.dst_off = d->in_off[s];
                ss.Hsrc = d->Ho[s]; ss.Wsrc = d->Wo[s]; ss.src_off = d->out_off[s];
                ss.inv_per_img = 1.0f / (float)(Hs * Ws); ss.inv_ws = 1.0f / (float)Ws;
                m += (long long)d->N * Hs * Ws;
            }
    }
    p.nsub = ns;
    BD_REQUIRE(m < (1ll << 24), "conv2d_dgrad: too many pixels (2^24 limit of the fast index decode)");
    p.linear_dst = (d->nseg == 1 && st == 1 && d->in_off[0] == 0 && d->in_pix_per_img == d->Hi[0] * d->Wi[0]) ? 1 : 0;
    p.linear_src = (p.linear_dst && d->R == 1 && d->S == 1 && d->pad == 0 && d->out_off[0] == 0 &&
                    d->out_pix_per_img == d->Ho[0] * d->Wo[0]) ? 1 : 0;
// ... 31 lines not shown
```

### basedet_amd/csrc/gskip.hip

```cpp
#include "common.h"

namespace {

enum { GS_ANY = 1, GS_TOP = 2, GS_BOT = 4, GS_LEFT = 8, GS_RIGHT = 16, GS_TL = 32, GS_TR = 64, GS_BL = 128, GS_BR = 256 };

struct GsSeg { int patch_start, H, W, pw, off; };

struct GsParams {
    const bf16_raw* g;
    int* mask;
    int C, ppi, ph, pw_px, nseg, patches_per_img, total;
    GsSeg seg[BD_MAX_SEGS];
};

__device__ __forceinline__ int gs_level(const GsParams& p, int rem) {
    int s = 0;
#pragma unroll
    for (int k = 1; k < BD_MAX_SEGS; ++k)
        if (k < p.nseg && rem >= p.seg[k].patch_start) s = k;
    return s;
}

__global__ __launch_bounds__(256) void gskip_scan_kernel(const GsParams p) {
    __shared__ int sbits;
// ... 56 lines not shown
__device__ __forceinline__ void gs_compact_body(const GsParams& p, int* live, int* list, int* count, int* wsum) {
    constexpr int KP = 8;
    const int tid = threadIdx.x, wv = tid >> 6, ln = tid & 63;
    int base = 0;
    for (int c0 = 0; c0 < p.total; c0 += 1024 * KP) {
        int lv[KP];
#pragma unroll
        for (int j = 0; j < KP; ++j) {
            const int q = c0 + tid * KP + j;
            lv[j] = 0;
            if (q < p.total) {
                const int n = q / p.patches_per_img, rem = q - n * p.patches_per_img;
                const int s = gs_level(p, rem);
                const int pwn = p.seg[s].pw, rows = (p.seg[s].H + p.ph - 1) / p.ph;
                const int local = rem - p.seg[s].patch_start, by = local / pwn, bx = local - by * pwn;
                const int* m = p.mask + (long long)n * p.patches_per_img + p.seg[s].patch_start;
                const bool up = by > 0, dn = by + 1 < rows, lf = bx > 0, rt = bx + 1 < pwn;
                int v = gs_mask<FRESH>(m, by * pwn + bx) & GS_ANY;
                if (up) v |= gs_mask<FRESH>(m, (by - 1) * pwn + bx) & GS_BOT;
                if (dn) v |= gs_mask<FRESH>(m, (by + 1) * pwn + bx) & GS_TOP;
                if (lf) v |= gs_mask<FRESH>(m, by * pwn + bx - 1) & GS_RIGHT;
                if (rt) v |= gs_mask<FRESH>(m, by * pwn + bx + 1) & GS_LEFT;
                if (up && lf) v |= gs_mask<FRESH>(m, (by - 1) * pwn + bx - 1) & GS_BR;
                if (up && rt) v |= gs_mask<FRESH>(m, (by - 1) * pwn + bx + 1) & GS_BL;
                if (dn && lf) v |= gs_mask<FRESH>(m, (by + 1) * pwn + bx - 1) & GS_TR;
                if (dn && rt) v |= gs_mask<FRESH>(m, (by + 1) * pwn + bx + 1) & GS_TL;
                lv[j] = v != 0;
            }
        }
        int cnt = 0;
#pragma unroll
        for (int j = 0; j < KP; ++j) cnt += lv[j];
        int inc = cnt;
#pragma unroll
        for (int o = 1; o < 64; o <<= 1) {
            const int y = __shfl_up(inc, o, 64);
            if (ln >= o) inc += y;
        }
        if (ln == 63) wsum[wv] = inc;
        __syncthreads();
        int off = base + inc - cnt, tot = 0;
#pragma unroll
        for (int w = 0; w < 16; ++w) {
            off += w < wv ? wsum[w] : 0;
            tot += wsum[w];
        }
#pragma unroll
        for (int j = 0; j < KP; ++j) {
            const int q = c0 + tid * KP + j;
            if (q < p.total) live[q] = lv[j];
            if (lv[j]) list[off++] = q;
        }
        base += tot;
        __syncthreads();
    }
    if (tid == 0) *count = base;
}

__global__ __launch_bounds__(1024) void gskip_compact_kernel(const GsParams p, int* live, int* list, int* count) {
    __shared__ int wsum[16];
    gs_compact_body<false>(p, live, list, count, wsum);
}

enum { GM_HDR = 8 };

struct GmSeg { int H, W, off, s4, s8, ss; };

struct GmParams {
    const bf16_raw* t;
    const int* live_in;
    int* map;
    int C, ppi, nseg, pi4, pi8, pis, tot4, tot8;
    GmSeg seg[BD_MAX_SEGS];
};

__global__ __launch_bounds__(1024) void gskip_fill_kernel(const GmParams p, const GsParams cp, int total) {
    __shared__ int sbits, slast;
    __shared__ int wsum[16];
    const int tid = threadIdx.x;
    int* m4 = p.map + GM_HDR;
    int* m8 = m4 + p.tot4;
    const int cpp = p.C >> 3;
    const int items = 4 * 16 * cpp;
    for (int pid = blockIdx.x; pid < total; pid += gridDim.x) {
        const int n = pid / p.pis, rem = pid - n * p.pis;
        int s = 0;
#pragma unroll
        for (int k = 1; k < BD_MAX_SEGS; ++k)
            if (k < p.nseg && rem >= p.seg[k].ss) s = k;
        const int H = p.seg[s].H, W = p.seg[s].W;
        const int sc = (W + 15) >> 4, r4 = (H + 3) >> 2, c8 = (W + 7) >> 3;
        const int local = rem - p.seg[s].ss, sy = local / sc, sx = local - sy * sc;
        int q4[2], q8[2];
        bool ok4[2], ok8[2], lv[2];
#pragma unroll
        for (int h = 0; h < 2; ++h) {
            ok4[h] = 2 * sy + h < r4;
            q4[h] = n * p.pi4 + p.seg[s].s4 + (2 * sy + h) * sc + sx;
            ok8[h] = 2 * sx + h < c8;
            q8[h] = n * p.pi8 + p.seg[s].s8 + sy * c8 + 2 * sx + h;
            lv[h] = ok4[h] && (p.live_in == nullptr || p.live_in[q4[h]] != 0);
        }
        int b = 0;
        if (lv[0] || lv[1]) {
            if (tid == 0) sbits = 0;
            __syncthreads();
            const long long img = (long long)n * p.ppi + p.seg[s].off;
            int bits = 0;
#pragma unroll
            for (int h = 0; h < 2; ++h) {
                if (!lv[h]) continue;
                for (int i = tid; i < items; i += 1024) {
                    const int px = i / cpp, ch = i - px * cpp;
                    const int py = px >> 4, pxx = px & 15;
                    const int y = 8 * sy + 4 * h + py, x = 16 * sx + pxx;
                    if (y < H && x < W) {
                        const u32x4_t v = *reinterpret_cast<const u32x4_t*>(p.t + (img + (long long)y * W + x) * p.C + ch * 8);
                        if (v[0] | v[1] | v[2] | v[3]) {
                            const bool t = py == 0, bo = py == 3, l = pxx == 0, r = pxx == 15;
                            const int w = GS_ANY | (t ? GS_TOP : 0) | (bo ? GS_BOT : 0) | (l ? GS_LEFT : 0) | (r ? GS_RIGHT : 0) |
                                          (t && l ? GS_TL : 0) | (t && r ? GS_TR : 0) | (bo && l ? GS_BL : 0) | (bo && r ? GS_BR : 0);
                            bits |= (w << (9 * h)) | (1 << (18 + (pxx >> 3)));
                        }
                    }
                }
            }
#pragma unroll
            for (int m = 32; m >= 1; m >>= 1) bits |= __shfl_xor(bits, m, 64);
            if ((tid & 63) == 0 && bits) atomicOr(&sbits, bits);
            __syncthreads();
            b = sbits;
            __syncthreads();
        }
        if (tid == 0) {
            if (ok4[0]) m4[q4[0]] = b & 511;
            if (ok4[1]) m4[q4[1]] = (b >> 9) & 511;
            if (ok8[0]) m8[q8[0]] = (b >> 18) & 1;
            if (ok8[1]) m8[q8[1]] = (b >> 19) & 1;
        }
    }
    if (tid == 0) {
        __builtin_amdgcn_fence(__ATOMIC_RELEASE, "agent");
        slast = atomicAdd(p.map + 1, 1) == (int)gridDim.x - 1;
    }
    __syncthreads();
    if (!slast) return;
    __builtin_amdgcn_fence(__ATOMIC_ACQUIRE, "agent");
    const int nxt = (p.map[0] & 1) ^ 1;
    int* live = m8 + p.tot8;
    gs_compact_body<true>(cp, live, live + p.tot4 * (1 + nxt), p.map + 2 + nxt, wsum);
    if (tid == 0) { p.map[0] = nxt; p.map[1] = 0; }
}

GsParams gs_params(const bd_conv_desc* d, int ph, int pw, int side = 0) {
    GsParams p{};
    p.C = side ? d->Cin : d->Cout; p.ppi = side ? d->in_pix_per_img : d->out_pix_per_img; p.ph = ph; p.pw_px = pw; p.nseg = d->nseg;
    int ps = 0;
    for (int s = 0; s < d->nseg; ++s) {
        GsSeg& sg = p.seg[s];
        const int H = side ? d->Hi[s] : d->Ho[s], W = side ? d->Wi[s] : d->Wo[s];
        sg.patch_start = ps; sg.H = H; sg.W = W; sg.pw = cdiv(W, pw); sg.off = side ? d->in_off[s] : d->out_off[s];
        ps += cdiv(H, ph) * sg.pw;
    }
    p.patches_per_img = ps;
    p.total = ps * d->N;
    return p;
}

}

int bd_gskip_patches(const bd_conv_desc* d, int ph, int pw) {
    return gs_params(d, ph, pw).total;
}

void bd_gskip_scan(const bd_conv_desc* d, const void* g, int ph, int pw, int* mask, hipStream_t stream) {
    GsParams p = gs_params(d, ph, pw);
    p.g = (const bf16_raw*)g; p.mask = mask;
    if (p.total > 0) hipLaunchKernelGGL(gskip_scan_kernel, dim3(p.total), dim3(256), 0, stream, p);
}

void bd_gskip_compact(const bd_conv_desc* d, int ph, int pw, const int* mask, int* live, int* list, int* count, hipStream_t stream) {
    GsParams p = gs_params(d, ph, pw);
    p.mask = const_cast<int*>(mask);
    hipLaunchKernelGGL(gskip_compact_kernel, dim3(1), dim3(1024), 0, stream, p, live, list, count);
}

void bd_gskip_map_layout(const bd_conv_desc* d, int side, BdGskipMap* out) {
    const int p4 = gs_params(d, 4, 16, side).total, p8 = gs_params(d, 8, 8, side).total;
    out->p4 = p4; out->p8 = p8;
    out->m4 = GM_HDR; out->m8 = GM_HDR + p4; out->live = out->m8 + p8; out->list = out->live + p4;
    out->ints = (size_t)GM_HDR + (size_t)4 * p4 + p8;
}

extern "C" size_t bd_conv2d_gskip_map_bytes(const bd_conv_desc* d, int of_dx) {
    if (!d || d->nseg < 1 || d->nseg > BD_MAX_SEGS || !(d->R == 3 && d->S == 3 && d->stride == 1 && d->pad == 1)) return 0;
    BdGskipMap m;
    bd_gskip_map_layout(d, of_dx ? 1 : 0, &m);
    return m.ints * sizeof(int);
}

void bd_gskip_fill(const bd_conv_desc* d, int side, const void* t, const int* live_in, int* map, hipStream_t stream) {
    const GsParams g4 = gs_params(d, 4, 16, side), g8 = gs_params(d, 8, 8, side), gs = gs_params(d, 8, 16, side);
    GmParams p{};
    p.t = (const bf16_raw*)t; p.live_in = live_in; p.map = map;
    p.C = g4.C; p.ppi = g4.ppi; p.nseg = g4.nseg;
    p.pi4 = g4.patches_per_img; p.pi8 = g8.patches_per_img; p.pis = gs.patches_per_img; p.tot4 = g4.total; p.tot8 = g8.total;
    for (int s = 0; s < g4.nseg; ++s)
        p.seg[s] = GmSeg{g4.seg[s].H, g4.seg[s].W, g4.seg[s].off, g4.seg[s].patch_start, g8.seg[s].patch_start, gs.seg[s].patch_start};
    GsParams cp = g4;
    cp.mask = map + GM_HDR;
    const int grid = gs.total < 128 ? gs.total : 128;
    if (grid > 0) hipLaunchKernelGGL(gskip_fill_kernel, dim3(grid), dim3(1024), 0, stream, p, cp, gs.total);
}

extern "C" int bd_gskip_map_scan(const bd_conv_desc* d, int of_dx, const void* t, void* map, size_t map_bytes, bd_stream_t stream) {
    BD_REQUIRE(d && t && map, "gskip_map_scan: null pointer");
    const size_t need = bd_conv2d_gskip_map_bytes(d, of_dx);
    BD_REQUIRE(need > 0, "gskip_map_scan: liveness maps belong to 3x3 / stride 1 / pad 1 descriptors");
    BD_REQUIRE(map_bytes >= need, "gskip_map_scan: map %zu < required %zu bytes", map_bytes, need);
    const int side = of_dx ? 1 : 0;
    BdGskipMap m;
    bd_gskip_map_layout(d, side, &m);
    int* mp = (int*)map;
    if (hipMemsetAsync(mp, 0, GM_HDR * sizeof(int), (hipStream_t)stream) != hipSuccess) { bd_set_error("gskip_map_scan: memset failed"); return BD_ELAUNCH; }
    GsParams p4 = gs_params(d, 4, 16, side), p8 = gs_params(d, 8, 8, side);
    p4.g = p8.g = (const bf16_raw*)t;
    p4.mask = mp + m.m4; p8.mask = mp + m.m8;
    if (p4.total > 0) {
        hipLaunchKernelGGL(gskip_scan_kernel, dim3(p4.total), dim3(256), 0, (hipStream_t)stream, p4);
        hipLaunchKernelGGL(gskip_scan_kernel, dim3(p8.total), dim3(256), 0, (hipStream_t)stream, p8);
    }
    hipLaunchKernelGGL(gskip_compact_kernel, dim3(1), dim3(1024), 0, (hipStream_t)stream, p4, mp + m.live, mp + m.list, mp + 2);
    BD_CHECK_LAUNCH("bd_gskip_map_scan");
    return BD_OK;
}
```

### basedet_amd/csrc/image_ops.hip

```cpp
#include <stdarg.h>

#include <cmath>
#include "common.h"

static thread_local std::string g_bd_error = "";
int bd_num_cus() {
    static std::mutex mu;
    static int cached[256] = {0};
    int dev = 0;
    if (hipGetDevice(&dev) != hipSuccess || dev < 0 || dev > 255) return 256;
    std::lock_guard<std::mutex> g(mu);
    if (!cached[dev]) {
        int n = 0;
        cached[dev] = (hipDeviceGetAttribute(&n, hipDeviceAttributeMultiprocessorCount, dev) == hipSuccess && n > 0) ? n : 256;
    }
    return cached[dev];
}

void bd_set_error(const char* fmt, ...) {
    char buf[512];
    va_list ap;
    va_start(ap, fmt);
    vsnprintf(buf, sizeof(buf), fmt, ap);
    va_end(ap);
    g_bd_error = buf;
}
extern "C" const char* bd_last_error_string(void) { return g_bd_error.c_str(); }
static thread_local const char* g_bd_last_kernel = "";
void bd_note_kernel(const char* name) { g_bd_last_kernel = name; }
extern "C" const char* bd_conv_last_kernel(void) { return g_bd_last_kernel; }
extern "C" int bd_version(void) { return 106; }

namespace {

constexpr int HALO_Y = 3, HALO_X = 4;

__global__ void pad_normalize_kernel(const float* __restrict__ in, int N, int H, int W, int Hp, int Wp,
                                     float m0, float m1, float m2, float s0, float s1, float s2,
                                     bf16_raw* __restrict__ out) {
    const int Hb = Hp + 2 * HALO_Y, Wb = Wp + 2 * HALO_X;
    const long long total = (long long)N * Hb * Wb;
    for (long long i = (long long)blockIdx.x * blockDim.x + threadIdx.x; i < total; i += (long long)gridDim.x * blockDim.x) {
        const int xb = (int)(i % Wb);
        const long long t = i / Wb;
        const int yb = (int)(t % Hb);
        const int n = (int)(t / Hb);
        const int y = yb - HALO_Y, x = xb - HALO_X;
        u32x2_t o = {0u, 0u};
        if (y >= 0 && y < Hp && x >= 0 && x < Wp) {
            float v0 = 0.f, v1 = 0.f, v2 = 0.f;
            if (y < H && x < W) {
                const long long base = ((long long)n * 3 * H + y) * W + x;
                v0 = in[base]; v1 = in[base + (long long)H * W]; v2 = in[base + 2ll * H * W];
            }
            o[0] = pack_bf2((v0 - m0) / s0, (v1 - m1) / s1);
            o[1] = pack_bf2((v2 - m2) / s2, 0.f);
        }
        *reinterpret_cast<u32x2_t*>(out + i * 4) = o;
    }
}

__global__ void pad_normalize_nchw_kernel(const float* __restrict__ in, int N, int H, int W, int Hp, int Wp,
                                          float m0, float m1, float m2, float s0, float s1, float s2,
                                          float* __restrict__ out) {
    const long long total = (long long)N * 3 * Hp * Wp;
    for (long long i = (long long)blockIdx.x * blockDim.x + threadIdx.x; i < total; i += (long long)gridDim.x * blockDim.x) {
        const int x = (int)(i % Wp);
        long long t = i / Wp;
        const int y = (int)(t % Hp);
        t /= Hp;
        const int c = (int)(t % 3);
        const int n = (int)(t / 3);
        float v = 0.f;
        if (y < H && x < W) v = in[(((long long)n * 3 + c) * H + y) * W + x];
        const float m = c == 0 ? m0 : (c == 1 ? m1 : m2);
        const float s = c == 0 ? s0 : (c == 1 ? s1 : s2);
        out[i] = (v - m) / s;
    }
}

__device__ __forceinline__ u32x4_t max_bf16x8(u32x4_t a, u32x4_t b) {
    u32x4_t r;
#pragma unroll
    for (int k = 0; k < 4; ++k) r[k] = pack_bf2(fmaxf(bf_lo(a[k]), bf_lo(b[k])), fmaxf(bf_hi(a[k]), bf_hi(b[k])));
    return r;
}

__global__ void maxpool3x3s2_kernel(const bf16_raw* __restrict__ x, int N, int H, int W, int C, bf16_raw* __restrict__ y) {
    const int Ho = (H + 2 - 3) / 2 + 1, Wo = (W + 2 - 3) / 2 + 1;
    const int cv = C / 8;
    const long long total = (long long)N * Ho * Wo * cv;
    for (long long i = (long long)blockIdx.x * blockDim.x + threadIdx.x; i < total; i += (long long)gridDim.x * blockDim.x) {
        const int c = (int)(i % cv);
        long long t = i / cv;
        const int ox = (int)(t % Wo);
        t /= Wo;
        const int oy = (int)(t % Ho);
        const int n = (int)(t / Ho);
        const unsigned int NEG = 0xff80ff80u;
        u32x4_t m = {NEG, NEG, NEG, NEG};
#pragma unroll
        for (int r = 0; r < 3; ++r) {
            const int iy = 2 * oy - 1 + r;
            if (iy < 0 || iy >= H) continue;
#pragma unroll
            for (int s = 0; s < 3; ++s) {
                const int ix = 2 * ox - 1 + s;
                if (ix < 0 || ix >= W) continue;
                const u32x4_t v = *reinterpret_cast<const u32x4_t*>(x + (((long long)n * H + iy) * W + ix) * C + c * 8);
                m = max_bf16x8(m, v);
            }
        }
        *reinterpret_cast<u32x4_t*>(y + i * 8) = m;
    }
}

__device__ __forceinline__ void up2_taps(int o, int n, int& i0, int& i1, float& w0, float& w1) {
    const int j = o >> 1;
    if (o & 1) { i0 = j; i1 = j + 1 < n ? j + 1 : n - 1; w0 = 0.75f; w1 = 0.25f; }
    else       { i0 = j - 1 >= 0 ? j - 1 : 0; i1 = j; w0 = 0.25f; w1 = 0.75f; }
}

__global__ void upsample2x_add_fwd_kernel(const bf16_raw* __restrict__ top, long long top_ppi, long long top_off,
                                          bf16_raw* __restrict__ lat, long long lat_ppi, long long lat_off,
                                          int N, int H, int W, int C) {
    const int cv = C / 8, H2 = 2 * H, W2 = 2 * W;
    const long long total = (long long)N * H2 * W2 * cv;
    for (long long i = (long long)blockIdx.x * blockDim.x + threadIdx.x; i < total; i += (long long)gridDim.x * blockDim.x) {
        const int c = (int)(i % cv);
        long long t = i / cv;
        const int x = (int)(t % W2);
        t /= W2;
        const int y = (int)(t % H2);
        const int n = (int)(t / H2);
        int y0, y1, x0, x1; float wy0, wy1, wx0, wx1;
        up2_taps(y, H, y0, y1, wy0, wy1);
        up2_taps(x, W, x0, x1, wx0, wx1);
        const bf16_raw* tb = top + ((long long)n * top_ppi + top_off) * C + c * 8;
        const u32x4_t a = *reinterpret_cast<const u32x4_t*>(tb + ((long long)y0 * W + x0) * C);
        const u32x4_t b = *reinterpret_cast<const u32x4_t*>(tb + ((long long)y0 * W + x1) * C);
        const u32x4_t cc = *reinterpret_cast<const u32x4_t*>(tb + ((long long)y1 * W + x0) * C);
        const u32x4_t d = *reinterpret_cast<const u32x4_t*>(tb + ((long long)y1 * W + x1) * C);
        bf16_raw* lp = lat + (((long long)n * lat_ppi + lat_off) + (long long)y * W2 + x) * C + c * 8;
        u32x4_t l = *reinterpret_cast<u32x4_t*>(lp);
        u32x4_t o;
#pragma unroll
        for (int k = 0; k < 4; ++k) {
            const float lo = wy0 * (wx0 * bf_lo(a[k]) + wx1 * bf_lo(b[k])) + wy1 * (wx0 * bf_lo(cc[k]) + wx1 * bf_lo(d[k]));
            const float hi = wy0 * (wx0 * bf_hi(a[k]) + wx1 * bf_hi(b[k])) + wy1 * (wx0 * bf_hi(cc[k]) + wx1 * bf_hi(d[k]));
            o[k] = pack_bf2(bf_lo(l[k]) + lo, bf_hi(l[k]) + hi);
        }
        *reinterpret_cast<u32x4_t*>(lp) = o;
    }
}

__device__ __forceinline__ float up2_bwd_weight(int o, int j, int n) {
    int i0, i1; float w0, w1;
    up2_taps(o, n, i0, i1, w0, w1);
    float w = 0.f;
    if (i0 == j) w += w0;
    if (i1 == j) w += w1;
    return w;
}

__global__ void upsample2x_add_bwd_kernel(const bf16_raw* __restrict__ dlat, long long lat_ppi, long long lat_off,
                                          bf16_raw* __restrict__ dtop, long long top_ppi, long long top_off,
                                          int N, int H, int W, int C, int accumulate) {
    const int cv = C / 8, H2 = 2 * H, W2 = 2 * W;
    const long long total = (long long)N * H * W * cv;
    for (long long i = (long long)blockIdx.x * blockDim.x + threadIdx.x; i < total; i += (long long)gridDim.x * blockDim.x) {
        const int c = (int)(i % cv);
        long long t = i / cv;
        const int x = (int)(t % W);
        t /= W;
        const int y = (int)(t % H);
        const int n = (int)(t / H);
        float acc[8] = {0.f, 0.f, 0.f, 0.f, 0.f, 0.f, 0.f, 0.f};
        const bf16_raw* lb = dlat + ((long long)n * lat_ppi + lat_off) * C + c * 8;
        for (int oy = 2 * y - 1; oy <= 2 * y + 2; ++oy) {
            if (oy < 0 || oy >= H2) continue;
            const float wy = up2_bwd_weight(oy, y, H);
            if (wy == 0.f) continue;
            for (int ox = 2 * x - 1; ox <= 2 * x + 2; ++ox) {
                if (ox < 0 || ox >= W2) continue;
// ... 436 lines not shown
```

### basedet_amd/models/engine.py

```python
import numpy as np
import torch

from .. import ops
from ..ops import Geom

BN_EPS = 1e-5


class ParamArena:

    def __init__(self, device):
        self.device = device
        self.entries = []
        self.total = 0
        self.w = self.g = self.v = None

    def reserve(self, name, shape):
        n = int(np.prod(shape))
        off = self.total
        self.entries.append((name, tuple(shape), off, n))
        self.total += (n + 63) // 64 * 64
        return len(self.entries) - 1

    def allocate(self):
        self.w = torch.zeros(self.total, dtype=torch.float32, device=self.device)
        self.g = torch.zeros(self.total, dtype=torch.float32, device=self.device)
        self.v = torch.zeros(self.total, dtype=torch.float32, device=self.device)

    def view(self, which, idx):
        _, shape, off, n = self.entries[idx]
        return getattr(self, which)[off:off + n].view(shape)


class ConvLayer:

    def __init__(self, name, cin, cout, k, stride, pad, device, bn_prefix=None, has_bias=False, trainable=True,
                 cout_pad=None):
        self.name, self.cin, self.cout_real, self.k, self.stride, self.pad = name, cin, cout, k, stride, pad
        self.cout = cout_pad or cout
        self.bn_prefix, self.has_bias, self.trainable = bn_prefix, has_bias, trainable
        self.device = device
        self.w = self.b = self.gw = self.gb = None
        self.row_scale = None
        self.w_fwd = torch.empty((self.cout, k * k, cin), dtype=torch.bfloat16, device=device)
        self.w_dgrad = torch.empty((cin, k * k, self.cout), dtype=torch.bfloat16, device=device) if trainable else None
        self._desc_cache = {}
        self.gskip = False
        self._gskip_cache = {}
        self._gskip_ws = None
        self._chain = (None, None, False)
        self._chain_cache = {}
        self.fp8 = False
        self.fp8_dgrad = False
        self.fp8_wgrad = False
        self.fp8_1x1 = False
        self.fp8_1x1_dgrad = False
        self.w_q8 = self.w_scale8 = self.w_q8t = self.w_scale8t = None
        self.act_scale = 1.0
        self.grad_scale = 4096.0
        self.amax_slot = None
        self.probe_ctl = None
        self.q8_scratch = None

    def bind(self, arena, params):
        w = torch.from_numpy(params[self.name + ".weight"]).permute(0, 2, 3, 1).contiguous()
        if self.cout != self.cout_real:
            pad = torch.zeros((self.cout - self.cout_real,) + tuple(w.shape[1:]))
            w = torch.cat([w, pad], 0)
        if self.trainable:
            self.w = arena.view("w", self._wi); self.gw = arena.view("g", self._wi)
            self.w.copy_(w)
        else:
            self.w = w.to(self.device)
        if self.bn_prefix:
            g, b = params[self.bn_prefix + ".weight"], params[self.bn_prefix + ".bias"]
            m, v = params[self.bn_prefix + ".running_mean"], params[self.bn_prefix + ".running_var"]
            scale = g / np.sqrt(v + BN_EPS)
            self.row_scale = torch.from_numpy(scale.astype(np.float32)).to(self.device)
            self.b = torch.from_numpy((b - m * scale).astype(np.float32)).to(self.device)
        elif self.has_bias:
            b = torch.from_numpy(params[self.name + ".bias"])
            if self.cout != self.cout_real:
                b = torch.cat([b, torch.zeros(self.cout - self.cout_real)])
            if self.trainable:
                self.b = arena.view("w", self._bi); self.gb = arena.view("g", self._bi)
                self.b.copy_(b)
            else:
                self.b = b.to(self.device)

    def reserve(self, arena):
        if not self.trainable:
            return
        self._wi = arena.reserve(self.name + ".weight", (self.cout, self.k, self.k, self.cin))
        if self.has_bias:
            self._bi = arena.reserve(self.name + ".bias", (self.cout,))

    def export(self, out):
        out[self.name + ".weight"] = self.w[: self.cout_real].permute(0, 3, 1, 2).contiguous().cpu().numpy()
        if self.has_bias and not self.bn_prefix:
            out[self.name + ".bias"] = self.b[: self.cout_real].cpu().numpy().copy()

    def export_grad(self, out):
        out[self.name + ".weight"] = self.gw[: self.cout_real].permute(0, 3, 1, 2).contiguous().cpu()
        if self.gb is not None:
            out[self.name + ".bias"] = self.gb[: self.cout_real].cpu().clone()

    def enable_fp8(self, q8_scratch, act_scale=1.0, dgrad=False, grad_scale=4096.0, wgrad=False):
        assert self.cin % 16 == 0 and self.cout % 8 == 0
        self.fp8, self.q8_scratch, self.act_scale = True, q8_scratch, float(act_scale)
        self.w_q8 = torch.empty((self.cout, self.k * self.k, self.cin), dtype=torch.uint8, device=self.device)
        self.w_scale8 = torch.empty((self.cout,), dtype=torch.float32, device=self.device)
        if wgrad and self.trainable and self.k == 3 and self.stride == 1 and self.cin % 16 == 0 and self.cout % 16 == 0:
            self.fp8_wgrad, self.grad_scale = True, float(grad_scale)
        if dgrad and self.trainable and self.k == 3 and self.stride == 1 and self.cin > 128 and self.cout % 16 == 0:
            self.fp8_dgrad, self.grad_scale = True, float(grad_scale)
            self.w_q8t = torch.empty((self.cin, self.k * self.k, self.cout), dtype=torch.uint8, device=self.device)
            self.w_scale8t = torch.empty((self.cin,), dtype=torch.float32, device=self.device)

    def enable_fp8_1x1(self, act_scale=1.0, dgrad=False, grad_scale=4096.0, expanding=True):
        assert self.k == 1 and self.stride == 1 and self.cin % 32 == 0 and self.cout % 32 == 0
        self.act_scale, self.grad_scale = float(act_scale), float(grad_scale)
        if self.cin % 128 == 0 and (self.cin >= 2 * self.cout or expanding):
            self.fp8_1x1 = True
            self.w_q8 = torch.empty((self.cout, 1, self.cin), dtype=torch.uint8, device=self.device)
            self.w_scale8 = torch.empty((self.cout,), dtype=torch.float32, device=self.device)
        if dgrad and self.trainable and self.cout % 128 == 0 and (self.cout >= 2 * self.cin or expanding):
            self.fp8_1x1_dgrad = True
            self.w_q8t = torch.empty((self.cin, 1, self.cout), dtype=torch.uint8, device=self.device)
            self.w_scale8t = torch.empty((self.cin,), dtype=torch.float32, device=self.device)

    def pack_fp8(self):
        if self.k == 1 and (self.fp8_1x1 or self.fp8_1x1_dgrad):
            if self.fp8_1x1:
                ops.weight_pack_fp8(self.w, self.row_scale, self.cout, 1, self.cin, self.act_scale, self.w_q8, self.w_scale8)
            if self.fp8_1x1_dgrad:
                ops.weight_pack_fp8_t(self.w, self.row_scale, self.cout, 1, self.cin, self.grad_scale, self.w_q8t, self.w_scale8t)
            return
        ops.weight_pack_fp8(self.w, self.row_scale, self.cout, self.k * self.k, self.cin, self.act_scale, self.w_q8, self.w_scale8)
        if self.fp8_dgrad:
            ops.weight_pack_fp8_t(self.w, self.row_scale, self.cout, self.k * self.k, self.cin, self.grad_scale, self.w_q8t, self.w_scale8t)

    def pack(self):
        ops.weight_pack(self.w, self.row_scale, self.w_fwd, self.w_dgrad, self.cout, self.k * self.k, self.cin)
        if self.fp8 or self.fp8_1x1 or self.fp8_1x1_dgrad:
            self.pack_fp8()

    def desc(self, gin: Geom, gout: Geom):
        key = (gin.N, tuple(gin.H), tuple(gin.W), tuple(gin.off), gin.pix_per_img,
               tuple(gout.H), tuple(gout.W), tuple(gout.off), gout.pix_per_img)
        d = self._desc_cache.get(key)
        if d is None:
            d = ops.conv_desc(gin, gout, self.cin, self.cout, self.k, self.k, self.stride, self.pad)
            self._desc_cache[key] = d
        return d

    def bwd_desc(self, gin: Geom, gout: Geom):
        d = self.desc(gin, gout)
        if not self.gskip:
            return d
        h = self._gskip_cache.get(id(d))
        if h is None:
            n = (max(ops.conv2d_dgrad_gskip_bytes(d), 4) + 3) // 4
            if self._gskip_ws is None or self._gskip_ws.numel() < n:
                self._gskip_ws = torch.empty(n, dtype=torch.int32, device=self.device)
                self._gskip_cache.clear()
            h = self._gskip_cache[id(d)] = (ops.gskip_desc(d, self._gskip_ws), d)
        gmap, dxmap, clean = self._chain
        if gmap is None and dxmap is None:
            return h[0]
        key = (id(d), self._gskip_ws.data_ptr(), gmap.data_ptr() if gmap is not None else 0, dxmap.data_ptr() if dxmap is not None else 0, clean)
        c = self._chain_cache.get(key)
        if c is None:
            if len(self._chain_cache) > 64:
                self._chain_cache.clear()
            c = self._chain_cache[key] = (ops.gskip_desc(d, self._gskip_ws, gmap=gmap, dxmap=dxmap, dx_clean=clean), d)
        return c[0]

    def set_chain(self, gmap=None, dxmap=None, dx_clean=False):
        self._chain = (gmap, dxmap, bool(dx_clean) and dxmap is not None) if self.gskip else (None, None, False)

    def forward(self, x, gin, gout, y, add=None, relu=False, bits=None, x8=None, y8=None, q_scale=1.0):
        flags = (ops.EPI_RELU if relu else 0) | (ops.EPI_ADD_BEFORE if add is not None else 0)
        if self.fp8_1x1 and x8 is not None and ops.conv1x1_fp8_ok(self.desc(gin, gout), 0):
            return ops.conv1x1_fp8(self.desc(gin, gout), 0, x8, self.w_q8, self.w_scale8, self.b, y, add=add, bits=bits, y8=y8,
                                   q_scale=q_scale, flags=flags)
        if self.fp8 and bits is None:
            xq = x8 if x8 is not None else ops.quantize_fp8(x, self.act_scale, self.q8_scratch(x.numel())[: x.numel()])
            return ops.conv2d_fwd_fp8(self.desc(gin, gout), xq, self.w_q8, self.w_scale8, self.b, y, add=add, flags=flags, y8=y8,
                                      q_scale=self.act_scale)
        return ops.conv2d_fwd(self.desc(gin, gout), x, self.w_fwd, self.b, y, add=add, flags=flags, bits=bits,
                              y8=y8 if (y8 is not None and ops.dense_1x1_bits_ok(self.desc(gin, gout))) else None, q_scale=q_scale)

    def gnstats_ok(self):
        return (not self.fp8) and self.k == 3 and self.stride == 1 and self.pad == 1 and self.cout == 256 and self.cin % 64 == 0

    def forward_gnstats(self, x, gin, gout, y, part):
        return ops.conv2d_fwd_gnstats(self.desc(gin, gout), x, self.w_fwd, self.b, y, part)

    def dgrad(self, g, gin, gout, dx, first=True, mask=None, add_after=None, maskbits=None, g8=None, dx8=None, q_scale=1.0,
              add_before=None, sparse=False):
        flags, add = 0, None
        if add_after is not None:
            flags |= ops.EPI_ADD_AFTER
            add = add_after
        elif add_before is not None:
            flags |= ops.EPI_ADD_BEFORE
            add = add_before
        elif not first:
            flags |= ops.EPI_ADD_BEFORE
            add = dx
            if sparse and self.stride > 1:
                flags |= ops.EPI_SPARSE
        if mask is not None or maskbits is not None:
            flags |= ops.EPI_MASK
        if maskbits is not None:
            mask = None
        d = self.bwd_desc(gin, gout)
        if self.amax_slot is not None and self.probe_ctl[0] and (self.fp8_1x1_dgrad or self.fp8_dgrad):
            ops.absmax_bf16(g, self.amax_slot)
        if self.fp8_1x1_dgrad and g8 is not None and ops.conv1x1_fp8_ok(d, 1):
            ops.conv1x1_fp8(d, 1, g8, self.w_q8t, self.w_scale8t, None, dx, add=add, mask=mask, maskbits=maskbits, y8=dx8,
                            q_scale=q_scale, flags=flags)
            return dx8 is not None
        if self.fp8_dgrad and maskbits is None:
            gq = g8 if g8 is not None else ops.quantize_bf8(g, self.grad_scale, self.q8_scratch(g.numel())[: g.numel()])
            ops.conv2d_dgrad_fp8(d, gq, self.w_q8t, self.w_scale8t, dx, add=add, mask=mask, flags=flags, dx8=dx8, q_scale=q_scale)
            return dx8 is not None
        if dx8 is not None and not ops.dense_1x1_bits_ok(d):
            dx8 = None
        ops.conv2d_dgrad(d, g, self.w_dgrad, dx, add=add, mask=mask, flags=flags, maskbits=maskbits, dx8=dx8, q_scale=q_scale)
        return dx8 is not None

    def dgrad_writes_twin(self, gin, gout):
        return self.fp8_dgrad or ops.dense_1x1_bits_ok(self.desc(gin, gout))

    def wgrad(self, x, g, gin, gout, ws, colsum_ws=None, x8=None, g8=None, queue=None):
        d = self.bwd_desc(gin, gout)
        if self.fp8_wgrad and x8 is not None and g8 is not None:
            ops.conv2d_wgrad_fp8(d, x8, g8, 1.0 / (self.act_scale * self.grad_scale), self.gw, ws, row_scale=self.row_scale)
            if self.gb is not None:
                ops.colsum_bf16(g, g.shape[0], self.cout, self.gb, colsum_ws)
            return
        if queue is not None:
            queue.wgrad(d, x, g, self.gw, self.gb, ws, row_scale=self.row_scale)
        elif self.gb is not None:
            ops.conv2d_wgrad_bias(d, x, g, self.gw, self.gb, ws, row_scale=self.row_scale)
        else:
            ops.conv2d_wgrad(d, x, g, self.gw, ws, row_scale=self.row_scale)

    def thin_backward_ok(self, gin: Geom):
        return (self.k == 1 and self.stride == 1 and self.pad == 0 and self.cin == 256 and self.cout == 16 and self.trainable
                and self.row_scale is None and self.gb is not None and not (self.fp8 or self.fp8_1x1)
                and sum(h * w for h, w in zip(gin.H, gin.W)) == gin.pix_per_img)

    def thin_forward(self, x, gin: Geom, y):
        ops.conv1x1_thin_fwd(x, self.w, self.b, gin.pixels, self.cin, self.cout, y)

    def thin_backward(self, x, g, gin: Geom, dx, ws):
        ops.conv1x1_thin_bwd(x, g, self.w, gin.pixels, self.cin, self.cout, dx, self.gw, self.gb, self.cout_real, ws)

    def wgrad_ws_bytes(self, gin, gout):
        d = self.bwd_desc(gin, gout)
        n = ops.conv2d_wgrad_bias_workspace_bytes(d) if self.gb is not None else ops.conv2d_wgrad_workspace_bytes(d)
        return max(n, ops.conv2d_wgrad_fp8_workspace_bytes(d)) if self.fp8_wgrad else n


class FusedPredConv(ConvLayer):

    def __init__(self, name, parts, cin, k, stride, pad, device, cout_pad):
        self.parts = parts
        super().__init__(name, cin, sum(c for _, c in parts), k, stride, pad, device, has_bias=True, trainable=True, cout_pad=cout_pad)

    def bind(self, arena, params):
        merged = dict(params)
        merged[self.name + ".weight"] = np.concatenate([params[n + ".weight"] for n, _ in self.parts], 0)
        merged[self.name + ".bias"] = np.concatenate([params[n + ".bias"] for n, _ in self.parts], 0)
        super().bind(arena, merged)

    def export(self, out):
        o = 0
        for n, c in self.parts:
            out[n + ".weight"] = self.w[o:o + c].permute(0, 3, 1, 2).contiguous().cpu().numpy()
            out[n + ".bias"] = self.b[o:o + c].cpu().numpy().copy()
            o += c

    def export_grad(self, out):
        o = 0
        for n, c in self.parts:
            out[n + ".weight"] = self.gw[o:o + c].permute(0, 3, 1, 2).contiguous().cpu()
            out[n + ".bias"] = self.gb[o:o + c].cpu().clone()
            o += c


def cls_ld(K):
    return (int(K) + 7) // 8 * 8


def pad_class_rows(a, A, K):
    ld = cls_ld(K)
    a = np.asarray(a)
    assert a.shape[0] == A * K, (a.shape, A, K)
    if ld == K:
        return a
    out = np.zeros((A, ld) + a.shape[1:], a.dtype)
    out[:, :K] = a.reshape((A, K) + a.shape[1:])
    return out.reshape((A * ld,) + a.shape[1:])


def unpad_class_rows(a, A, K):
    ld = cls_ld(K)
    assert a.shape[0] == A * ld, (a.shape, A, K)
    if ld == K:
        return a
    return a.reshape((A, ld) + tuple(a.shape[1:]))[:, :K].reshape((A * K,) + tuple(a.shape[1:]))


class PaddedClsConv(ConvLayer):

    def __init__(self, name, cin, A, K, k, stride, pad, device):
        self.A, self.K, self.cls_ld = int(A), int(K), cls_ld(K)
        super().__init__(name, cin, self.A * self.K, k, stride, pad, device, has_bias=True, trainable=True, cout_pad=self.A * self.cls_ld)

    def bind(self, arena, params):
        w = pad_class_rows(np.asarray(params[self.name + ".weight"], np.float32), self.A, self.K)
        b = pad_class_rows(np.asarray(params[self.name + ".bias"], np.float32), self.A, self.K)
        self.w = arena.view("w", self._wi); self.gw = arena.view("g", self._wi)
        self.w.copy_(torch.from_numpy(w).permute(0, 2, 3, 1).contiguous())
        self.b = arena.view("w", self._bi); self.gb = arena.view("g", self._bi)
        self.b.copy_(torch.from_numpy(b))

    def export(self, out):
        out[self.name + ".weight"] = unpad_class_rows(self.w, self.A, self.K).permute(0, 3, 1, 2).contiguous().cpu().numpy()
        out[self.name + ".bias"] = unpad_class_rows(self.b, self.A, self.K).cpu().numpy().copy()

    def export_grad(self, out):
# ... 77 lines not shown
```

### basedet_amd/models/retinanet.py

```python
import torch

from .. import ops
from ..streams import fork, join
from ..utils.registry import registers
from . import params as P
from .engine import PaddedClsConv
from .fpn_base import FPNDetector, _round_up


@registers.models.register()
class RetinaNet(FPNDetector):
    READS_MATCHER = True

    @staticmethod
    def init_params(cfg, seed=0):
        return P.init_retinanet_params(cfg, seed)

    @classmethod
    def check_config(cls, cfg):
        super().check_config(cfg)
        cls.check_anchor_config(cfg, matcher=cls.READS_MATCHER)
        if not cfg.MODEL.HEAD.get("WITH_NORM", True):
            raise ValueError("MODEL.HEAD.WITH_NORM = False is not supported for the RetinaNet family: only True (the default) is implemented")

    def _build_head(self, add, params):
        m = self.cfg.MODEL
        ch = self.fpn_ch
        self.num_anchors = len(m.ANCHOR.SCALES[0]) * len(m.ANCHOR.RATIOS[0])
        nc = m.HEAD.NUM_CONVS
        self.cls_tower = [add(f"head.cls_subnet.{2 * i}", ch, ch, 3, 1, 1, bias=True) for i in range(nc)]
        self.box_tower = [add(f"head.bbox_subnet.{2 * i}", ch, ch, 3, 1, 1, bias=True) for i in range(nc)]
        A, K = self.num_anchors, self.num_classes
        self.cls_score = self.convs["head.cls_score"] = PaddedClsConv("head.cls_score", ch, A, K, 3, 1, 1, self.device)
        self.cls_ld = self.cls_score.cls_ld
        self.box_ld = _round_up(A * 4, 8)
        self.bbox_pred = add("head.bbox_pred", ch, A * 4, 3, 1, 1, bias=True, cout_pad=self.box_ld)
        if bool(m.get("SPARSE_BOX_BWD", True)) and m.get("WEIGHT_DTYPE", "bf16") == "bf16":
            for c in self.box_tower + [self.bbox_pred]:
                c.gskip = True
        self.sparse_chain = bool(m.get("SPARSE_BOX_CHAIN", True))
        self._build_base_anchors()

    def _head_convs(self):
        return self.cls_tower + self.box_tower + [self.cls_score, self.bbox_pred]

    def _plan_head(self, pl):
        ch = self.fpn_ch
        N = pl.N
        C = pl._carve
        bf = torch.bfloat16

        def act(g, c):
            return C.empty((g.pixels, c), bf)

        nc = len(self.cls_tower)
        pl.cls_act = [act(pl.pyr, ch) for _ in range(nc)]
        pl.box_act = [act(pl.pyr, ch) for _ in range(nc)]
        A, K = self.num_anchors, self.num_classes
        pl.logits = act(pl.pyr, A * self.cls_ld)
        pl.offsets = act(pl.pyr, self.box_ld)
        pl.d_logits = C.like(pl.logits)
        pl.d_offsets = C.like(pl.offsets)
        pl.g_tower = [[act(pl.pyr, ch) for _ in range(nc)] for _ in range(2)]
        pl.g_map = None
        if self.sparse_chain and all(c.gskip for c in self.box_tower + [self.bbox_pred]):
            nb = ops.conv2d_gskip_map_bytes(self.box_tower[0].desc(pl.pyr, pl.pyr))
            if nb:
                pl.g_map = [C.empty(((nb + 3) // 4,), torch.int32) for _ in range(nc)]
        pl.chain_epoch = None
        tw = lambda: C.empty((pl.pyr.pixels, ch), torch.uint8)
        pl.cls_act8 = [tw() if c.fp8 else None for c in self.cls_tower]
        pl.box_act8 = [tw() if c.fp8 else None for c in self.box_tower]
        tg = self.fp8_grad_twins
        pl.g_tower8 = [[tw() if (c.fp8_dgrad and tg) else None for c in tower] for tower in (self.cls_tower, self.box_tower)]
        pl.g_P8 = tw() if (tg and all(t[0].fp8_dgrad for t in (self.cls_tower, self.box_tower))) else None
        self._plan_anchors(pl)
        tot = pl.A_total
        pl.labels = C.empty((N, tot), torch.int32)
        pl.match_idx = C.empty((N, tot), torch.int32)
        pl.gt_offsets = C.empty((N, tot, 4), torch.float32)
        pl.num_fg = C.zeros((1,), torch.int32)
        pl.loss_buf = C.zeros((2,), torch.float32)

    def head_forward(self, pl):
        concurrent = bool(self.cfg.MODEL.get("HEAD_TOWERS_CONCURRENT", True)) and self.weight_dtype != "fp8_e4m3"
        side = self.streams.aux() if concurrent else None
        with fork(side):
            t, t8 = pl.P, getattr(pl, "P8", None)
            for c, a, a8 in zip(self.box_tower, pl.box_act, pl.box_act8):
                c.forward(t, pl.pyr, pl.pyr, a, relu=True, x8=t8, y8=a8); t, t8 = a, a8
            self.bbox_pred.forward(t, pl.pyr, pl.pyr, pl.offsets, x8=t8)
        t, t8 = pl.P, getattr(pl, "P8", None)
        for c, a, a8 in zip(self.cls_tower, pl.cls_act, pl.cls_act8):
            c.forward(t, pl.pyr, pl.pyr, a, relu=True, x8=t8, y8=a8); t, t8 = a, a8
        self.cls_score.forward(t, pl.pyr, pl.pyr, pl.logits, x8=t8)
        join(side)

    def get_losses(self, inputs):
        assert self.training
        pre = self.pre_process(inputs)
        pl = pre["plan"]
        self._cur = pl
        m = self.cfg.MODEL
        gt = pre["gt_boxes"]
        num_gt = pre["img_info"][:, 4].to(torch.int32).contiguous()
        N, Gmax = gt.shape[0], gt.shape[1]
        ws = self._scratch("assign", N * Gmax * 4).view(torch.float32)
        thr = m.MATCHER.THRESHOLDS
        side = self.streams.aux() if m.get("ASSIGN_ON_SIDE_STREAM", True) else None
        with fork(side):
            ops.retina_assign_encode(pl.anchors, gt, num_gt, thr[0], thr[1], m.MATCHER.ALLOW_LOW_QUALITY, m.BOX_REG.MEAN,
                                     m.BOX_REG.STD, pl.labels, pl.match_idx, pl.gt_offsets, pl.num_fg, ws)
        self.network_forward(pl)
        join(side)
        pl.loss_buf.zero_()
        rows = N * pl.A_total
        ops.focal_loss_fwd_bwd(pl.logits, pl.labels, rows, self.num_classes, m.LOSSES.FOCAL_LOSS_ALPHA,
                               m.LOSSES.FOCAL_LOSS_GAMMA, pl.num_fg, 1.0, pl.loss_buf[0:1], pl.d_logits,
                               ld=self.cls_ld if self.cls_ld != self.num_classes else None)
        ops.smooth_l1_fwd_bwd(pl.offsets, pl.gt_offsets, pl.labels, pl.pyr.pixels, self.num_anchors, self.box_ld,
                              m.LOSSES.SMOOTH_L1_BETA, pl.num_fg, m.LOSSES.REG_LOSS_WEIGHT, pl.loss_buf[1:2], pl.d_offsets)
        cls_loss, reg_loss = pl.loss_buf[0], pl.loss_buf[1]
        return {"total_loss": cls_loss + reg_loss, "cls_loss": cls_loss, "reg_loss": reg_loss}

    def head_backward(self, pl, ws, cws):
        pyr = pl.pyr
        for ti, (tower, acts, pred, dpred) in enumerate(((self.cls_tower, pl.cls_act, self.cls_score, pl.d_logits),
                                                         (self.box_tower, pl.box_act, self.bbox_pred, pl.d_offsets))):
            gbuf, g8 = pl.g_tower[ti], pl.g_tower8[ti]
            n = len(tower)
            maps = pl.g_map if (ti == 1 and self.sparse_chain and all(c.gskip for c in tower + [pred])) else None
            if ti == 1:
                clean = maps is not None and pl.chain_epoch == self.plan_arena.epoch
                pl.chain_epoch = self.plan_arena.epoch if maps is not None else None
                if maps is not None:
                    pred.set_chain(None, maps[n - 1], clean)
                    for i in range(n):
                        tower[i].set_chain(maps[i], maps[i - 1] if i > 0 else None, clean)
            gs = tower[n - 1].grad_scale
            self._wgrad(pred, acts[-1], dpred, pyr, pyr, ws, cws)
            tw = g8[n - 1] if pred.dgrad_writes_twin(pyr, pyr) else None
            if not pred.dgrad(dpred, pyr, pyr, gbuf[n - 1], mask=acts[-1], dx8=tw, q_scale=gs):
                tw = None
            act8 = pl.cls_act8 if ti == 0 else pl.box_act8
            for i in range(n - 1, -1, -1):
                x = acts[i - 1] if i > 0 else pl.P
                x8 = (act8[i - 1] if i > 0 else pl.P8) if tw is not None else None
                self._wgrad(tower[i], x, gbuf[i], pyr, pyr, ws, cws, x8=x8, g8=tw)
                if i > 0:
                    nxt = g8[i - 1] if tower[i].dgrad_writes_twin(pyr, pyr) else None
                    wrote = tower[i].dgrad(gbuf[i], pyr, pyr, gbuf[i - 1], mask=acts[i - 1], g8=tw, dx8=nxt, q_scale=tower[i - 1].grad_scale)
                    tw = nxt if wrote else None
                else:
                    wrote_p = tower[i].dgrad(gbuf[i], pyr, pyr, pl.g_P, first=(ti == 0), g8=tw,
                                             dx8=pl.g_P8 if tower[i].dgrad_writes_twin(pyr, pyr) else None,
                                             q_scale=self.output[self.fpn_stages[0]].grad_scale)
        for c in self.box_tower + [self.bbox_pred]:
            c.set_chain()
        pl.g_P8_ready = pl.g_P8 is not None and bool(wrote_p)

    def _debug_head(self, pl, out, lvl):
        for i in range(pl.pyr.nlev):
            for k in range(len(self.cls_tower)):
                out[f"cls{k}_{i}"] = lvl(pl.cls_act[k], i)
                out[f"box{k}_{i}"] = lvl(pl.box_act[k], i)
            lg = lvl(pl.logits, i)
            out[f"logits_{i}"] = self.cls_score.real_logits(lg.permute(0, 2, 3, 1)).permute(0, 3, 1, 2).contiguous()
            out[f"offs_{i}"] = lvl(pl.offsets, i, self.num_anchors * 4)

    def inference_batch(self, inputs):
        assert not self.training
        pre = self.pre_process(inputs)
        pl = pre["plan"]
        self.network_forward(pl)
        K, A = self.num_classes, self.num_anchors
        m = self.cfg.MODEL
        return self._detect(pl.N, [h * w * A for h, w in pl.sizes], K, 0, pre["img_info"], logits=pl.logits, anchors=pl.anchors,
                            offsets=pl.offsets, off_ld=self.box_ld, A=A, mean=m.BOX_REG.MEAN, std=m.BOX_REG.STD, cls_ld=self.cls_ld)
```

### basedet_amd/ops.py

```python
import ctypes as C
from dataclasses import dataclass, field
from typing import List, Optional

import torch

from . import _lib
from ._lib import ConvDesc, EPI_ADD_AFTER, EPI_ADD_BEFORE, EPI_MASK, EPI_RELU, EPI_SPARSE, check, f32arr, i32arr, ptr, stream_ptr


@dataclass
class Geom:
    N: int
    H: List[int]
    W: List[int]
    off: List[int] = field(default_factory=list)
    pix_per_img: int = 0

    def __post_init__(self):
        if not self.off:
            o = 0
            self.off = []
            for h, w in zip(self.H, self.W):
                self.off.append(o)
                o += h * w
            if not self.pix_per_img:
                self.pix_per_img = o
        if not self.pix_per_img:
            self.pix_per_img = sum(h * w for h, w in zip(self.H, self.W))

    @property
    def nlev(self):
        return len(self.H)

    @property
    def pixels(self):
        return self.N * self.pix_per_img

    def level(self, i):
        return Geom(self.N, [self.H[i]], [self.W[i]], [self.off[i]], self.pix_per_img)

    def conv_out(self, R, stride, pad):
        H = [(h + 2 * pad - R) // stride + 1 for h in self.H]
        W = [(w + 2 * pad - R) // stride + 1 for w in self.W]
        return Geom(self.N, H, W)


def single(N, H, W):
    return Geom(N, [H], [W])


def conv_desc(gin: Geom, gout: Geom, Cin, Cout, R, S, stride, pad) -> ConvDesc:
    d = ConvDesc()
    d.N, d.Cin, d.Cout, d.R, d.S, d.stride, d.pad, d.nseg = gin.N, Cin, Cout, R, S, stride, pad, gin.nlev
    assert gin.nlev == gout.nlev <= _lib.BD_MAX_SEGS
    for i in range(gin.nlev):
        d.Hi[i], d.Wi[i], d.Ho[i], d.Wo[i] = gin.H[i], gin.W[i], gout.H[i], gout.W[i]
        d.in_off[i], d.out_off[i] = gin.off[i], gout.off[i]
    d.in_pix_per_img, d.out_pix_per_img = gin.pix_per_img, gout.pix_per_img
    return d


def L():
    return _lib.load()


_ROUTE = [0, 0, 0, 0]
_SR_SEED = [0]
_ROUTE_NAMES = {"dense1x1": 0, "patch3x3": 1, "wgrad": 2, "fp8_patch": 3}


def set_route(**kw):
    for k, v in kw.items():
        _ROUTE[_ROUTE_NAMES[k]] = 0 if v is None else int(v) + 1


def reset_route():
    _ROUTE[:] = [0, 0, 0, 0]
    _SR_SEED[0] = 0


def _stamp(d):
    d.route[0], d.route[1], d.route[2], d.route[3] = _ROUTE
    d.sr_seed = _SR_SEED[0]
    return d


def conv2d_fwd(d, x, w_packed, bias, y, add=None, flags=0, bits=None, y8=None, q_scale=1.0):
    if y8 is not None:
        check(L().bd_conv2d_fwd_ex(C.byref(_stamp(d)), ptr(x), ptr(w_packed), ptr(bias), ptr(add), ptr(y), ptr(bits), ptr(y8), float(q_scale), flags,
                                   stream_ptr()), "bd_conv2d_fwd_ex")
        return y
    if bits is not None:
        check(L().bd_conv2d_fwd_bits(C.byref(_stamp(d)), ptr(x), ptr(w_packed), ptr(bias), ptr(add), ptr(y), ptr(bits), flags, stream_ptr()),
              "bd_conv2d_fwd_bits")
        return y
    check(L().bd_conv2d_fwd(C.byref(_stamp(d)), ptr(x), ptr(w_packed), ptr(bias), ptr(add), ptr(y), flags, stream_ptr()), "bd_conv2d_fwd")
    return y


def conv2d_dgrad(d, g, w_packed_t, dx, add=None, mask=None, flags=0, maskbits=None, dx8=None, q_scale=1.0):
    if dx8 is not None:
        check(L().bd_conv2d_dgrad_ex(C.byref(_stamp(d)), ptr(g), ptr(w_packed_t), ptr(add), ptr(mask), ptr(maskbits), ptr(dx), ptr(dx8),
                                     float(q_scale), flags, stream_ptr()), "bd_conv2d_dgrad_ex")
        return dx
    if maskbits is not None:
        check(L().bd_conv2d_dgrad_bits(C.byref(_stamp(d)), ptr(g), ptr(w_packed_t), ptr(add), ptr(maskbits), ptr(dx), flags, stream_ptr()),
              "bd_conv2d_dgrad_bits")
        return dx
    check(L().bd_conv2d_dgrad(C.byref(_stamp(d)), ptr(g), ptr(w_packed_t), ptr(add), ptr(mask), ptr(dx), flags, stream_ptr()), "bd_conv2d_dgrad")
    return dx


def conv2d_dgrad_gskip_bytes(d):
    return int(L().bd_conv2d_dgrad_gskip_bytes(C.byref(d)))


def conv2d_gskip_map_bytes(d, of_dx=False):
    return int(L().bd_conv2d_gskip_map_bytes(C.byref(d), int(bool(of_dx))))


def gskip_map_scan(d, t, gmap, of_dx=False):
    check(L().bd_gskip_map_scan(C.byref(d), int(bool(of_dx)), ptr(t), ptr(gmap), gmap.numel() * gmap.element_size(), stream_ptr()),
          "bd_gskip_map_scan")
    return gmap


def gskip_desc(d, scratch=None, gmap=None, dxmap=None, dx_clean=False):
    h = ConvDesc.from_buffer_copy(d)
    h.gskip = 1
    if scratch is not None:
        h.gskip_ws = scratch.data_ptr()
        h.gskip_ws_bytes = scratch.numel() * scratch.element_size()
    if gmap is not None:
        h.gskip_gmap = gmap.data_ptr()
        h.gskip_gmap_bytes = gmap.numel() * gmap.element_size()
    if dxmap is not None:
        h.gskip_dxmap = dxmap.data_ptr()
        h.gskip_dxmap_bytes = dxmap.numel() * dxmap.element_size()
    h.gskip_dx_clean = int(bool(dx_clean))
    return h


def quantize_fp8(x, scale, q):
    check(L().bd_quantize_fp8(ptr(x), x.numel(), float(scale), ptr(q), stream_ptr()), "bd_quantize_fp8")
    return q


def weight_pack_fp8(w, row_scale, Cout, RS, Cin, act_scale, wq, wscale):
    check(L().bd_weight_pack_fp8(ptr(w), ptr(row_scale), Cout, RS, Cin, float(act_scale), ptr(wq), ptr(wscale), stream_ptr()),
          "bd_weight_pack_fp8")


def conv2d_fwd_fp8(d, xq, wq, wscale, bias, y, add=None, flags=0, y8=None, q_scale=1.0):
    check(L().bd_conv2d_fwd_fp8_ex(C.byref(_stamp(d)), ptr(xq), ptr(wq), ptr(wscale), ptr(bias), ptr(add), ptr(y), ptr(y8), float(q_scale), flags,
                                   stream_ptr()), "bd_conv2d_fwd_fp8")
    return y


def quantize_bf8(x, scale, q):
    check(L().bd_quantize_bf8(ptr(x), x.numel(), float(scale), ptr(q), _SR_SEED[0], stream_ptr()), "bd_quantize_bf8")
    return q


def fp8_set_stochastic_rounding(seed):
    _SR_SEED[0] = int(seed) & 0xFFFFFFFF


def absmax_bf16(x, out):
    check(L().bd_absmax_bf16(ptr(x), x.numel(), ptr(out), stream_ptr()), "bd_absmax_bf16")


def weight_pack_fp8_t(w, row_scale, Cout, RS, Cin, grad_scale, wq_t, wscale_t):
    check(L().bd_weight_pack_fp8_t(ptr(w), ptr(row_scale), Cout, RS, Cin, float(grad_scale), ptr(wq_t), ptr(wscale_t), stream_ptr()),
          "bd_weight_pack_fp8_t")


def conv2d_dgrad_fp8(d, g8, wq_t, wscale_t, dx, add=None, mask=None, flags=0, dx8=None, q_scale=1.0):
    check(L().bd_conv2d_dgrad_fp8(C.byref(_stamp(d)), ptr(g8), ptr(wq_t), ptr(wscale_t), ptr(add), ptr(mask), ptr(dx), ptr(dx8), float(q_scale),
                                  flags, stream_ptr()), "bd_conv2d_dgrad_fp8")
    return dx


def conv1x1_fp8(d, mode, xq, wq, wscale, bias, y, add=None, mask=None, maskbits=None, bits=None, y8=None, q_scale=1.0, flags=0):
    check(L().bd_conv1x1_fp8(C.byref(_stamp(d)), mode, ptr(xq), ptr(wq), ptr(wscale), ptr(bias), ptr(add), ptr(mask), ptr(maskbits), ptr(y),
                             ptr(bits), ptr(y8), float(q_scale), flags, stream_ptr()), "bd_conv1x1_fp8")
    return y


def conv2d_wgrad_fp8_workspace_bytes(d):
    return int(L().bd_conv2d_wgrad_fp8_workspace_bytes(C.byref(_stamp(d))))


def conv2d_wgrad_fp8(d, x8, g8, inv_scale, dw, ws, row_scale=None, accumulate=False):
    check(L().bd_conv2d_wgrad_fp8(C.byref(_stamp(d)), ptr(x8), ptr(g8), float(inv_scale), ptr(row_scale), ptr(dw), int(accumulate), ptr(ws),
                                  ws.numel() * ws.element_size(), stream_ptr()), "bd_conv2d_wgrad_fp8")
    return dw


def conv1x1_fp8_ok(d, mode):
    K, CO = (d.Cin, d.Cout) if mode == 0 else (d.Cout, d.Cin)
    return dense_1x1_bits_ok(d) and K % 128 == 0 and CO % 32 == 0


def fp8_dgrad_ok(d):
    same = all(d.Hi[i] == d.Ho[i] and d.Wi[i] == d.Wo[i] for i in range(d.nseg))
    return d.R == 3 and d.S == 3 and d.stride == 1 and d.pad == 1 and same and d.Cin > 128 and d.Cin % 8 == 0 and d.Cout % 16 == 0


def dense_1x1_bits_ok(d):
    return (d.R == 1 and d.S == 1 and d.stride == 1 and d.pad == 0 and d.nseg == 1 and d.in_off[0] == 0 and d.out_off[0] == 0
            and d.in_pix_per_img == d.Hi[0] * d.Wi[0] and d.out_pix_per_img == d.Ho[0] * d.Wo[0]
            and d.Cin % 32 == 0 and d.Cout % 32 == 0 and d.N * d.in_pix_per_img * max(d.Cin, d.Cout) * 2 < 0x7fffffff)


def conv2d_wgrad_workspace_bytes(d):
    return int(L().bd_conv2d_wgrad_workspace_bytes(C.byref(_stamp(d))))


def conv2d_wgrad(d, x, g, dw, ws, row_scale=None, accumulate=False):
    check(L().bd_conv2d_wgrad(C.byref(_stamp(d)), ptr(x), ptr(g), ptr(row_scale), ptr(dw), int(accumulate), ptr(ws),
                              ws.numel() * ws.element_size(), stream_ptr()), "bd_conv2d_wgrad")
    return dw


def conv2d_wgrad_bias_workspace_bytes(d):
    return int(L().bd_conv2d_wgrad_bias_workspace_bytes(C.byref(_stamp(d))))


def conv2d_wgrad_bias(d, x, g, dw, dbias, ws, row_scale=None, accumulate=False):
    check(L().bd_conv2d_wgrad_bias(C.byref(_stamp(d)), ptr(x), ptr(g), ptr(row_scale), ptr(dw), ptr(dbias), int(accumulate), ptr(ws),
                                   ws.numel() * ws.element_size(), stream_ptr()), "bd_conv2d_wgrad_bias")
    return dw


def fpn_deconv_pack(w, C, w_fwd, w_dgrad):
    check(L().bd_fpn_deconv_pack(ptr(w), C, ptr(w_fwd), ptr(w_dgrad), stream_ptr()), "bd_fpn_deconv_pack")


def fpn_deconv_fwd(x, w_fwd, y, N, Hc, Wc, C, add=None):
    check(L().bd_fpn_deconv_fwd(ptr(x), ptr(w_fwd), ptr(add), ptr(y), N, Hc, Wc, 2 * Hc, 2 * Wc, C, stream_ptr()), "bd_fpn_deconv_fwd")
    return y


def fpn_deconv_dgrad(dy, w_dgrad, dx, N, Hc, Wc, C, add=None):
    check(L().bd_fpn_deconv_dgrad(ptr(dy), ptr(w_dgrad), ptr(add), ptr(dx), N, Hc, Wc, 2 * Hc, 2 * Wc, C, stream_ptr()), "bd_fpn_deconv_dgrad")
    return dx


def fpn_deconv_wgrad_workspace_bytes(N, Hc, Wc, C):
    return int(L().bd_fpn_deconv_wgrad_workspace_bytes(N, Hc, Wc, C))


def fpn_deconv_wgrad(x, dy, dw, ws, N, Hc, Wc, C, accumulate=False):
    check(L().bd_fpn_deconv_wgrad(ptr(x), ptr(dy), ptr(dw), int(accumulate), ptr(ws), ws.numel() * ws.element_size(), N, Hc, Wc,
                                  2 * Hc, 2 * Wc, C, stream_ptr()), "bd_fpn_deconv_wgrad")
    return dw


def stem_conv7x7_fwd(N, H, W, x_halo, w_stem, bias, y):
    check(L().bd_stem_conv7x7_fwd(N, H, W, ptr(x_halo), ptr(w_stem), ptr(bias), ptr(y), stream_ptr()), "bd_stem_conv7x7_fwd")
    return y


def stem_weight_pack(w, row_scale, w_stem):
    check(L().bd_stem_weight_pack(ptr(w), ptr(row_scale), ptr(w_stem), stream_ptr()), "bd_stem_weight_pack")


def weight_pack(w, row_scale, w_fwd, w_dgrad, Cout, RS, Cin):
    check(L().bd_weight_pack(ptr(w), ptr(row_scale), ptr(w_fwd), ptr(w_dgrad), Cout, RS, Cin, stream_ptr()), "bd_weight_pack")


def build_pack_table(entries, device):
    import ctypes as C
    import numpy as np
    from ._lib import PackDesc
    arr = (PackDesc * len(entries))()
    start = 0
    for i, (w, rs, wf, wd, co, r, ci) in enumerate(entries):
        arr[i].w = w.data_ptr()
        arr[i].row_scale = rs.data_ptr() if rs is not None else None
        arr[i].w_fwd = wf.data_ptr() if wf is not None else None
        arr[i].w_dgrad = wd.data_ptr() if wd is not None else None
        arr[i].Cout, arr[i].RS, arr[i].Cin, arr[i].block_start = co, r, ci, start
        start += int(L().bd_weight_pack_blocks(co, r, ci))
    raw = np.frombuffer(bytes(arr), dtype=np.uint8).copy()
    return torch.from_numpy(raw).to(device), len(entries), start


def weight_pack_multi(table):
    t, n, blocks = table
    check(L().bd_weight_pack_multi(ptr(t), n, blocks, stream_ptr()), "bd_weight_pack_multi")

# ... 645 lines not shown
```

### include/basedet_hip.h

```cpp
#ifndef BASEDET_HIP_H
#define BASEDET_HIP_H

#include <stddef.h>
#include <stdint.h>

#ifdef __cplusplus
extern "C" {
#endif

#define BD_OK 0
#define BD_EINVAL (-1)
#define BD_ELAUNCH (-2)
#define BD_EWORKSPACE (-3)

#define BD_MAX_SEGS 8

#define BD_EPI_RELU 1
#define BD_EPI_ADD_BEFORE 2
#define BD_EPI_ADD_AFTER 4
#define BD_EPI_MASK 8
#define BD_EPI_SPARSE 16

typedef void* bd_stream_t;

typedef struct bd_conv_desc {
    int32_t N;
    int32_t Cin, Cout;
    int32_t R, S;
    int32_t stride, pad;
    int32_t nseg;
    int32_t Hi[BD_MAX_SEGS], Wi[BD_MAX_SEGS];
    int32_t Ho[BD_MAX_SEGS], Wo[BD_MAX_SEGS];
    int32_t in_off[BD_MAX_SEGS], out_off[BD_MAX_SEGS];
    int32_t in_pix_per_img, out_pix_per_img;
    int32_t route[4];
    uint32_t sr_seed;
    int32_t gskip;
    void* gskip_ws;
    size_t gskip_ws_bytes;
    void* gskip_gmap;
    size_t gskip_gmap_bytes;
    void* gskip_dxmap;
    size_t gskip_dxmap_bytes;
    int32_t gskip_dx_clean;
} bd_conv_desc;

const char* bd_last_error_string(void);
int bd_version(void);
const char* bd_conv_last_kernel(void);
int bd_probe_mfma_rate(double seconds, double* tflops_out, double* clock_mhz_out, bd_stream_t stream);

int bd_probe_kernel_clock(const char* kernel, int reset, double* clock_mhz_out, double* busy_ms_out);


int bd_conv2d_fwd(const bd_conv_desc* d, const void* x, const void* w_packed, const float* bias,
                  const void* add, void* y, int flags, bd_stream_t stream);

int bd_conv2d_dgrad(const bd_conv_desc* d, const void* g, const void* w_packed_t, const void* add,
                    const void* mask, void* dx, int flags, bd_stream_t stream);
size_t bd_conv2d_dgrad_gskip_bytes(const bd_conv_desc* d);
size_t bd_conv2d_gskip_map_bytes(const bd_conv_desc* d, int of_dx);
int bd_gskip_map_scan(const bd_conv_desc* d, int of_dx, const void* t, void* map, size_t map_bytes, bd_stream_t stream);

int bd_conv2d_fwd_bits(const bd_conv_desc* d, const void* x, const void* w_packed, const float* bias, const void* add, void* y,
                       uint32_t* ybits, int flags, bd_stream_t stream);
int bd_conv2d_dgrad_bits(const bd_conv_desc* d, const void* g, const void* w_packed_t, const void* add, const uint32_t* maskbits,
                         void* dx, int flags, bd_stream_t stream);
int bd_conv2d_fwd_ex(const bd_conv_desc* d, const void* x, const void* w_packed, const float* bias, const void* add, void* y,
                     uint32_t* ybits, void* y8, float q_scale, int flags, bd_stream_t stream);
int bd_conv2d_dgrad_ex(const bd_conv_desc* d, const void* g, const void* w_packed_t, const void* add, const void* mask,
                       const uint32_t* maskbits, void* dx, void* dx8, float q_scale, int flags, bd_stream_t stream);

size_t bd_conv2d_wgrad_workspace_bytes(const bd_conv_desc* d);
int bd_conv2d_wgrad(const bd_conv_desc* d, const void* x, const void* g, const float* row_scale, float* dw,
                    int accumulate, void* ws, size_t ws_bytes, bd_stream_t stream);

size_t bd_conv2d_wgrad_bias_workspace_bytes(const bd_conv_desc* d);
int bd_conv2d_wgrad_bias(const bd_conv_desc* d, const void* x, const void* g, const float* row_scale, float* dw, float* dbias,
                         int accumulate, void* ws, size_t ws_bytes, bd_stream_t stream);

typedef struct bd_wgrad_queue* bd_wgrad_queue_t;
int bd_wgrad_queue_create(bd_wgrad_queue_t* out);
int bd_wgrad_queue_destroy(bd_wgrad_queue_t q);
int bd_wgrad_queue_pending(bd_wgrad_queue_t q);
int bd_conv2d_wgrad_queued(bd_wgrad_queue_t q, const bd_conv_desc* d, const void* x, const void* g, const float* row_scale, float* dw,
                           float* dbias, int accumulate, void* ws, size_t ws_bytes, bd_stream_t stream);
int bd_wgrad_queue_flush(bd_wgrad_queue_t q, bd_stream_t stream);



int bd_stem_conv7x7_fwd(int N, int H, int W, const void* x_halo, const void* w_stem, const float* bias,
                        void* y, bd_stream_t stream);
int bd_stem_pool_fwd(int N, int H, int W, const void* x_halo, const void* w_stem, const float* bias, void* y_pool,
                     bd_stream_t stream);
int bd_stem_weight_pack(const float* w , const float* row_scale, void* w_stem,
                        bd_stream_t stream);

int bd_weight_pack(const float* w, const float* row_scale, void* w_fwd, void* w_dgrad, int Cout, int RS,
                   int Cin, bd_stream_t stream);

typedef struct bd_pack_desc {
    const float* w;
    const float* row_scale;
    void* w_fwd;
    void* w_dgrad;
    int32_t Cout, RS, Cin, block_start;
} bd_pack_desc;
int bd_weight_pack_blocks(int Cout, int RS, int Cin);
int bd_weight_pack_multi(const bd_pack_desc* descs_dev, int n, int total_blocks, bd_stream_t stream);

size_t bd_colsum_workspace_bytes(int C);
int bd_colsum_bf16(const void* g, int N, int64_t pix_per_img, int64_t off, int64_t cnt, int C, float* out,
                   int accumulate, void* ws, size_t ws_bytes, bd_stream_t stream);

int bd_bottleneck_fwd_supported(int N, int H, int W, int Cin, int Cmid, int Cout, int has_downsample);
int bd_bottleneck_fwd(int N, int H, int W, int Cin, int Cmid, int Cout, const void* x, const void* w1, const float* b1, const void* w2,
                      const float* b2, const void* w3, const float* b3, const void* wd, const float* bd, void* y, bd_stream_t stream);


int bd_pad_normalize(const float* in, int N, int H, int W, int Hp, int Wp, const float* mean3,
                     const float* std3, void* out, bd_stream_t stream);
typedef struct bd_h2d* bd_h2d_t;
#define BD_HOST_F64 0
#define BD_HOST_F32 1
#define BD_HOST_U8 2
int bd_h2d_create(bd_h2d_t* out, int device, int threads);
int bd_h2d_threads(bd_h2d_t h);
int bd_h2d_submit(bd_h2d_t h, const void* src_host, int src_dtype, int64_t n, float* dst_dev, int64_t chunk_elems, bd_stream_t stream);
int bd_h2d_destroy(bd_h2d_t h);

int bd_pad_normalize_nchw(const float* in, int N, int H, int W, int Hp, int Wp, const float* mean3,
                          const float* std3, float* out, bd_stream_t stream);

typedef struct bd_image_desc {
    int64_t offset;
    int32_t src_h, src_w, dst_h, dst_w, flip;
    int32_t reserved_[1];
} bd_image_desc;
int bd_resize_pad_normalize(const uint8_t* packed_dev, int64_t packed_bytes, const bd_image_desc* descs_host, int N, int Hp, int Wp,
                            const float* mean3, const float* std3, void* x_halo, bd_stream_t stream);

int bd_maxpool3x3s2_fwd(const void* x, int N, int H, int W, int C, void* y, bd_stream_t stream);

int bd_upsample2x_add_fwd(const void* top, int64_t top_pix_per_img, int64_t top_off, void* lateral,
                          int64_t lat_pix_per_img, int64_t lat_off, int N, int H, int W, int C,
                          bd_stream_t stream);
int bd_upsample2x_add_bwd(const void* dlat, int64_t lat_pix_per_img, int64_t lat_off, void* dtop,
                          int64_t top_pix_per_img, int64_t top_off, int N, int H, int W, int C,
                          int accumulate, bd_stream_t stream);

int bd_fpn_deconv_pack(const float* w, int C, void* w_fwd, void* w_dgrad, bd_stream_t stream);
int bd_fpn_deconv_fwd(const void* x, const void* w_fwd, const void* add, void* y, int N, int Hc, int Wc, int Hf, int Wf, int C,
                      bd_stream_t stream);
int bd_fpn_deconv_dgrad(const void* dy, const void* w_dgrad, const void* add, void* dx, int N, int Hc, int Wc, int Hf, int Wf, int C,
                        bd_stream_t stream);
size_t bd_fpn_deconv_wgrad_workspace_bytes(int N, int Hc, int Wc, int C);
int bd_fpn_deconv_wgrad(const void* x, const void* dy, float* dw, int accumulate, void* ws, size_t ws_bytes, int N, int Hc, int Wc,
                        int Hf, int Wf, int C, bd_stream_t stream);

int bd_relu_bf16(const void* x, void* y, int64_t n, bd_stream_t stream);
int bd_relu_bwd_bf16(const void* g, const void* mask, const void* add, void* y, int64_t n, bd_stream_t stream);
int bd_add_bf16(const void* a, const void* b, void* y, int64_t n, bd_stream_t stream);


int bd_anchors_generate(int H, int W, int stride, float offset, const float* base, int A, float* out,
                        bd_stream_t stream);
int bd_points_generate(int H, int W, int stride, float offset, int A, float* out, bd_stream_t stream);

int bd_box_pairwise(const float* b1, int m, const float* b2, int n, int mode, float* out, bd_stream_t stream);

int bd_box_encode(const float* anchors, const float* gt, int64_t n, const float* mean4_host,
                  const float* std4_host, float* out, bd_stream_t stream);
int bd_box_decode(const float* anchors, const float* deltas, int64_t n, const float* mean4_host,
                  const float* std4_host, float* out, bd_stream_t stream);

int bd_retina_assign_encode(const float* anchors, int A, const float* gt_boxes, const int32_t* num_gt, int N,
                            int Gmax, float thr_lo, float thr_hi, int allow_low_quality,
                            const float* mean4_host, const float* std4_host, int32_t* labels,
                            int32_t* match_idx, float* offsets, int32_t* num_fg, void* ws, size_t ws_bytes,
                            bd_stream_t stream);

int bd_fcos_assign(const float* points, int P, const int32_t* lvl_start_host, const float* soi_host,
                   const int32_t* strides_host, int L, float radius, const float* gt_boxes,
                   const int32_t* num_gt, int N, int Gmax, int32_t* labels, float* offsets, float* ctrness,
                   float* stats, bd_stream_t stream);

size_t bd_atss_assign_workspace_bytes(int N, int P);
int bd_atss_assign(const float* points, int P, const int32_t* lvl_start_host, const int32_t* strides_host, int L, int topk,
                   float anchor_scale, const float* gt_boxes, const int32_t* num_gt, int N, int Gmax, int32_t* labels,
                   float* offsets, float* ctrness, float* stats, void* ws, size_t ws_bytes, bd_stream_t stream);

size_t bd_ota_assign_workspace_bytes(int N, int P);
int bd_ota_assign(const float* points, int P, const int32_t* lvl_start_host, const int32_t* strides_host, int L, const void* logits,
                  int K, const void* pred_ltrb, const float* gt_boxes, const int32_t* num_gt, int N, int Gmax, float alpha,
                  float gamma, float reg_weight, float center_radius, int candidate_k, int32_t* labels, float* targets,
                  float* gt_ious, float* stats, void* ws, size_t ws_bytes, bd_stream_t stream);
int bd_ota_assign_ld(const float* points, int P, const int32_t* lvl_start_host, const int32_t* strides_host, int L, const void* logits,
                     int K, int ld, const void* pred_ltrb, const float* gt_boxes, const int32_t* num_gt, int N, int Gmax, float alpha,
                     float gamma, float reg_weight, float center_radius, int candidate_k, int32_t* labels, float* targets,
                     float* gt_ious, float* stats, void* ws, size_t ws_bytes, bd_stream_t stream);

size_t bd_ota_sinkhorn_workspace_bytes(int N, int P, int Gmax);
int bd_ota_assign_sinkhorn(const float* points, int P, const int32_t* lvl_start_host, const int32_t* strides_host, int L,
                           const void* logits, int K, const void* pred_ltrb, const float* gt_boxes, const int32_t* num_gt, int N,
                           int Gmax, float alpha, float gamma, float reg_weight, float center_radius, int topq, float eps, int iters,
                           int32_t* labels, float* targets, float* gt_ious, float* stats, void* ws, size_t ws_bytes,
                           bd_stream_t stream);
int bd_ota_assign_sinkhorn_ld(const float* points, int P, const int32_t* lvl_start_host, const int32_t* strides_host, int L,
                              const void* logits, int K, int ld, const void* pred_ltrb, const float* gt_boxes, const int32_t* num_gt,
                              int N, int Gmax, float alpha, float gamma, float reg_weight, float center_radius, int topq, float eps,
                              int iters, int32_t* labels, float* targets, float* gt_ious, float* stats, void* ws, size_t ws_bytes,
                              bd_stream_t stream);

size_t bd_freeanchor_workspace_bytes(int N, int Gmax, int bucket, int A);
int bd_freeanchor_loss_fwd_bwd(const void* logits, const void* offsets, int box_ld, int anchors_per_pix, const float* anchors,
// ... 263 lines not shown
```

Before: 692.1 images/sec.

## Skip box-tower forward conv patches that cannot reach foreground anchors

Adds a kernel that turns the anchor labels into per-depth patch liveness maps: foreground pixels are dilated by one 3x3 step per tower layer, then compacted into patch lists. The box-tower 3x3 convolutions then run a sparse forward variant that computes only the listed patches. The intent is to avoid forward compute for box-regression activations whose outputs never feed the foreground-only box loss. In exchange it adds a liveness kernel on the aux stream, extra per-level map buffers, and more ordering between label assignment and the head forward. Activations in dead regions are left stale, so a debug path recomputes them densely.

```diff
diff --git a/basedet_amd/_lib.py b/basedet_amd/_lib.py
--- a/basedet_amd/_lib.py
+++ b/basedet_amd/_lib.py
@@ -7,7 +7,7 @@
 LIB_PATH = os.environ.get("BASEDET_HIP_LIB") or os.path.join(_HERE, "lib", "libbasedet_hip.so")
 
 BD_MAX_SEGS = 8
-ABI_VERSION = 106
+ABI_VERSION = 107
 EPI_RELU, EPI_ADD_BEFORE, EPI_ADD_AFTER, EPI_MASK, EPI_SPARSE = 1, 2, 4, 8, 16
 
 
@@ -27,6 +27,7 @@
         ("gskip", C.c_int32), ("gskip_ws", C.c_void_p), ("gskip_ws_bytes", C.c_size_t),
         ("gskip_gmap", C.c_void_p), ("gskip_gmap_bytes", C.c_size_t), ("gskip_dxmap", C.c_void_p), ("gskip_dxmap_bytes", C.c_size_t),
         ("gskip_dx_clean", C.c_int32),
+        ("fwd_map", C.c_void_p), ("fwd_map_bytes", C.c_size_t), ("fwd_clean", C.c_int32),
     ]
 
 
@@ -54,6 +55,8 @@
     "bd_conv2d_dgrad_gskip_bytes": (_Z, [_D]),
     "bd_conv2d_gskip_map_bytes": (_Z, [_D, _I]),
     "bd_gskip_map_scan": (_I, [_D, _I, _P, _P, _Z, _P]),
+    "bd_fwd_live_map_bytes": (_Z, [_D]),
+    "bd_fwd_live_maps": (_I, [_D, _P, _I, _I, C.POINTER(C.c_void_p), _Z, _I, _P]),
     "bd_conv2d_fwd_bits": (_I, [_D, _P, _P, _P, _P, _P, _P, _I, _P]),
     "bd_conv2d_fwd_ex": (_I, [_D, _P, _P, _P, _P, _P, _P, _P, _F, _I, _P]),
     "bd_conv2d_dgrad_ex": (_I, [_D, _P, _P, _P, _P, _P, _P, _P, _F, _I, _P]),
diff --git a/basedet_amd/csrc/common.h b/basedet_amd/csrc/common.h
--- a/basedet_amd/csrc/common.h
+++ b/basedet_amd/csrc/common.h
@@ -145,6 +145,8 @@
 
 struct BdGskipMap { int p4, p8, m4, m8, live, list; size_t ints; };
 void bd_gskip_map_layout(const bd_conv_desc* d, int side, BdGskipMap* out);
+struct BdFwdMap { int p4, live, list; size_t ints; };
+void bd_fwd_map_layout(const bd_conv_desc* d, BdFwdMap* out);
 
 static inline int grid_for(long long n, int block = 256, int cap = 4096) {
     long long g = (n + block - 1) / block;
diff --git a/basedet_amd/csrc/conv3x3_pp.hip b/basedet_amd/csrc/conv3x3_pp.hip
--- a/basedet_amd/csrc/conv3x3_pp.hip
+++ b/basedet_amd/csrc/conv3x3_pp.hip
@@ -45,6 +45,7 @@
     int* sp_ohdr;
     const int* sp_olist;
     int sp_stride, sp_clean;
+    int sp_oflip;
 };
 
 typedef __attribute__((address_space(3))) void lds_void_t;
@@ -115,7 +116,7 @@
         int zt = p.total_patches;
         const int* plist = nullptr;
         if (p.sp_clean) {
-            const int oc = __builtin_amdgcn_readfirstlane(p.sp_ohdr[0]) & 1;
+            const int oc = (__builtin_amdgcn_readfirstlane(p.sp_ohdr[0]) & 1) ^ p.sp_oflip;
             const int pc = __builtin_amdgcn_readfirstlane(p.sp_ohdr[2 + oc]);
             zt = pc < 0 ? 0 : (pc < zt ? pc : zt);
             plist = p.sp_olist + oc * p.sp_stride;
@@ -152,7 +153,7 @@
     int z_first = 0;
     const int* sp_list = p.sp_list;
     if constexpr (SPARSE) {
-        if (p.sp_ohdr && blockIdx.x == 0 && threadIdx.x == 0) p.sp_ohdr[1] = 0;
+        if (p.sp_ohdr && !p.sp_oflip && blockIdx.x == 0 && threadIdx.x == 0) p.sp_ohdr[1] = 0;
         const int cur = p.sp_hdr ? __builtin_amdgcn_readfirstlane(p.sp_hdr[0]) & 1 : 0;
         const int* cntp = p.sp_hdr ? p.sp_hdr + 2 + cur : p.sp_count;
         n_live = __builtin_amdgcn_readfirstlane(*cntp);
@@ -653,6 +654,17 @@
     const bool in_place = (flags & BD_EPI_ADD_BEFORE) && add && add == dst;
     if (d->gskip_dxmap && in_place) return false;
     return pp_sparse_epilogue(flags, add, dst);
+}
+
+bool bd_conv3x3_pp_fwd_map_ok(const bd_conv_desc* d, int flags, const void* add) {
+    if (g_patch_pp < 2 || !(d->R == 3 && d->S == 3 && d->stride == 1 && d->pad == 1)) return false;
+    if (d->Cin % 8 != 0 || d->Cout <= 128 || d->Cout % 8 != 0) return false;
+    if ((long long)d->N * d->in_pix_per_img * d->Cin * 2 >= 0x7fffffffll || (long long)d->N * d->out_pix_per_img >= 0x7fffffffll ||
+        (long long)d->Cin * 9 * d->Cout >= 0x7fffffffll) return false;
+    for (int s = 0; s < d->nseg; ++s)
+        if (d->Hi[s] != d->Ho[s] || d->Wi[s] != d->Wo[s]) return false;
+    if (bd_gskip_patches(d, PH, PW) >= (1 << 24) || bd_gskip_patches(d, PH, PW) < 1) return false;
+    return !add && !(flags & (BD_EPI_ADD_BEFORE | BD_EPI_ADD_AFTER | BD_EPI_MASK));
 }
 
 static int pp_launch(const bd_conv_desc* d, int mode, const void* src, const void* w, const float* bias, const void* add,
@@ -690,7 +702,8 @@
     const int num_cus = bd_num_cus();
     const bool in_place = (flags & BD_EPI_ADD_BEFORE) && add && add == dst;
     const bool sparse = mode == 1 && d->gskip && !gn_part && pp_sparse_epilogue(flags, add, dst);
-    if (g_pp_tail_split && !sparse && !gn_part && p.n_tiles == 1 && px_tiles > num_cus) {
+    const bool fsparse = mode == 0 && d->fwd_map && !gn_part;
+    if (g_pp_tail_split && !sparse && !fsparse && !gn_part && p.n_tiles == 1 && px_tiles > num_cus) {
         const int r = px_tiles % num_cus;
         if (r > 0 && r * (TILE_CO / TAIL_CO) <= num_cus) {
             px_tiles -= r;
@@ -713,6 +726,8 @@
         (void)hipFuncSetAttribute(reinterpret_cast<const void*>(&conv3x3_pp_kernel<0>), hipFuncAttributeMaxDynamicSharedMemorySize, LDS_BYTES);
         (void)hipFuncSetAttribute(reinterpret_cast<const void*>(&conv3x3_pp_kernel<1>), hipFuncAttributeMaxDynamicSharedMemorySize, LDS_BYTES);
         (void)hipFuncSetAttribute(reinterpret_cast<const void*>(&conv3x3_pp_kernel<1, false, true>), hipFuncAttributeMaxDynamicSharedMemorySize,
+                                  LDS_BYTES);
+        (void)hipFuncSetAttribute(reinterpret_cast<const void*>(&conv3x3_pp_kernel<0, false, true>), hipFuncAttributeMaxDynamicSharedMemorySize,
                                   LDS_BYTES));
     bd_note_kernel("conv3x3_pp_kernel");
     if (sparse) {
@@ -738,6 +753,15 @@
         }
         hipLaunchKernelGGL((conv3x3_pp_kernel<1, false, true>), dim3(p.main_grid), dim3(512), LDS_BYTES, stream, p);
         if (d->gskip_dxmap) bd_gskip_fill(d, 1, dst, p.sp_live, (int*)d->gskip_dxmap, stream);
+    } else if (fsparse) {
+        const int tot = p.total_patches;
+        BdFwdMap fm;
+        bd_fwd_map_layout(d, &fm);
+        int* m = (int*)d->fwd_map;
+        p.sp_hdr = m; p.sp_live = m + fm.live; p.sp_list = m + fm.list; p.sp_stride = tot;
+        p.sp_ohdr = m; p.sp_olist = m + fm.list; p.sp_oflip = 1;
+        p.sp_clean = d->fwd_clean ? 1 : 0;
+        hipLaunchKernelGGL((conv3x3_pp_kernel<0, false, true>), dim3(p.main_grid), dim3(512), LDS_BYTES, stream, p);
     } else if (gn_part) {
         BD_ONCE_PER_DEVICE((void)hipFuncSetAttribute(reinterpret_cast<const void*>(&conv3x3_pp_kernel<0, true>), hipFuncAttributeMaxDynamicSharedMemorySize, LDS_BYTES));
         hipLaunchKernelGGL((conv3x3_pp_kernel<0, true>), dim3(p.main_grid), dim3(512), LDS_BYTES, stream, p);
diff --git a/basedet_amd/csrc/conv_igemm.hip b/basedet_amd/csrc/conv_igemm.hip
--- a/basedet_amd/csrc/conv_igemm.hip
+++ b/basedet_amd/csrc/conv_igemm.hip
@@ -410,6 +410,7 @@
 int bd_conv3x3_patch_launch(const bd_conv_desc* d, int mode, const void* src, const void* w, const float* bias,
                             const void* add, const void* mask, void* dst, int flags, hipStream_t stream);
 bool bd_conv3x3_pp_maps_ok(const bd_conv_desc* d, int flags, const void* add, const void* dst);
+bool bd_conv3x3_pp_fwd_map_ok(const bd_conv_desc* d, int flags, const void* add);
 
 extern BD_KNOB int g_patch_dma;
 extern BD_KNOB int g_patch_pp;
@@ -482,6 +483,13 @@
     BD_REQUIRE(d->Cin % 8 == 0, "conv2d_fwd: Cin=%d must be a multiple of 8", d->Cin);
     BD_REQUIRE(d->Cout % 8 == 0, "conv2d_fwd: Cout=%d must be a multiple of 8", d->Cout);
     BD_REQUIRE(!(flags & BD_EPI_MASK), "conv2d_fwd: BD_EPI_MASK is a dgrad-only flag");
+    if (d->fwd_map || d->fwd_clean) {
+        BD_REQUIRE(d->fwd_map && is_3x3s1(d) && g_use_patch3x3 && !ybits && !y8 && bd_conv3x3_pp_fwd_map_ok(d, flags, add),
+                   "conv2d_fwd: fwd_map needs a 3x3 / stride 1 / pad 1 descriptor into more than 128 channels without residual operand on the "
+                   "default route (fwd_clean needs fwd_map)");
+        BD_REQUIRE(d->fwd_map_bytes >= bd_fwd_live_map_bytes(d), "conv2d_fwd: fwd_map %zu < required %zu bytes", (size_t)d->fwd_map_bytes,
+                   bd_fwd_live_map_bytes(d));
+    }
     if (is_dense_1x1(d) &&
         bd_conv1x1_dense_launch(x, w_packed, bias, add, nullptr, nullptr, y, ybits, y8, q_scale, 0, (long long)d->N * d->out_pix_per_img,
                                 d->Cin, d->Cout, flags, (hipStream_t)stream) == 0) {
diff --git a/basedet_amd/csrc/gskip.hip b/basedet_amd/csrc/gskip.hip
--- a/basedet_amd/csrc/gskip.hip
+++ b/basedet_amd/csrc/gskip.hip
@@ -232,6 +232,103 @@
     if (tid == 0) { p.map[0] = nxt; p.map[1] = 0; }
 }
 
+enum { FL_HDR = 8, FL_MAX_DEPTH = 8 };
+
+struct FlSeg { int H, W, off, s4, pw; };
+
+struct FlParams {
+    const int* labels;
+    int* map[FL_MAX_DEPTH];
+    int A, ppi, nseg, depths, pi4, tot4;
+    FlSeg seg[BD_MAX_SEGS];
+};
+
+__global__ __launch_bounds__(1024) void fwd_live_kernel(const FlParams p) {
+    extern __shared__ __attribute__((aligned(16))) unsigned char fl_bm[];
+    __shared__ int slast;
+    __shared__ int wsum[16];
+    const int tid = threadIdx.x;
+    const int n = blockIdx.x / p.nseg, s = blockIdx.x - n * p.nseg;
+    const int H = p.seg[s].H, W = p.seg[s].W, HW = H * W, pwn = p.seg[s].pw;
+    const int npatch = ((H + 3) >> 2) * pwn;
+    unsigned char* cur = fl_bm;
+    unsigned char* nxt = fl_bm + HW;
+    for (int i = tid; i < HW; i += 1024) cur[i] = 0;
+    __syncthreads();
+    const int* lab = p.labels + ((long long)n * p.ppi + p.seg[s].off) * p.A;
+    for (int i = tid; i < HW * p.A; i += 1024)
+        if (lab[i] > 0) cur[i / p.A] = 1;
+    __syncthreads();
+    for (int k = 0; k < p.depths; ++k) {
+        for (int i = tid; i < HW; i += 1024) {
+            const int y = i / W, x = i - y * W;
+            const int y0 = y > 0 ? y - 1 : 0, y1 = y + 1 < H ? y + 1 : H - 1, x0 = x > 0 ? x - 1 : 0, x1 = x + 1 < W ? x + 1 : W - 1;
+            int v = 0;
+            for (int yy = y0; yy <= y1; ++yy)
+                for (int xx = x0; xx <= x1; ++xx) v |= cur[yy * W + xx];
+            nxt[i] = (unsigned char)v;
+        }
+        __syncthreads();
+        int* live = p.map[k] + FL_HDR + n * p.pi4 + p.seg[s].s4;
+        for (int q = tid; q < npatch; q += 1024) {
+            const int by = q / pwn, bx = q - by * pwn;
+            const int ye = by * 4 + 4 < H ? by * 4 + 4 : H, xe = bx * 16 + 16 < W ? bx * 16 + 16 : W;
+            int v = 0;
+            for (int y = by * 4; y < ye; ++y)
+                for (int x = bx * 16; x < xe; ++x) v |= nxt[y * W + x];
+            live[q] = v;
+        }
+        unsigned char* t = cur; cur = nxt; nxt = t;
+        __syncthreads();
+    }
+    __builtin_amdgcn_fence(__ATOMIC_RELEASE, "agent");
+    __syncthreads();
+    if (tid == 0) slast = atomicAdd(p.map[0] + 1, 1) == (int)gridDim.x - 1;
+    __syncthreads();
+    if (!slast) return;
+    __builtin_amdgcn_fence(__ATOMIC_ACQUIRE, "agent");
+    constexpr int KP = 8;
+    const int wv = tid >> 6, ln = tid & 63;
+    for (int k = 0; k < p.depths; ++k) {
+        int* hdr = p.map[k];
+        const int* live = hdr + FL_HDR;
+        const int to = (hdr[0] & 1) ^ 1;
+        int* list = hdr + FL_HDR + p.tot4 * (1 + to);
+        int base = 0;
+        for (int c0 = 0; c0 < p.tot4; c0 += 1024 * KP) {
+            int lv[KP];
+            int cnt = 0;
+#pragma unroll
+            for (int j = 0; j < KP; ++j) {
+                const int q = c0 + tid * KP + j;
+                lv[j] = q < p.tot4 ? (__hip_atomic_load(live + q, __ATOMIC_RELAXED, __HIP_MEMORY_SCOPE_AGENT) != 0) : 0;
+                cnt += lv[j];
+            }
+            int inc = cnt;
+#pragma unroll
+            for (int o = 1; o < 64; o <<= 1) {
+                const int y = __shfl_up(inc, o, 64);
+                if (ln >= o) inc += y;
+            }
+            if (ln == 63) wsum[wv] = inc;
+            __syncthreads();
+            int off = base + inc - cnt, tot = 0;
+#pragma unroll
+            for (int w = 0; w < 16; ++w) {
+                off += w < wv ? wsum[w] : 0;
+                tot += wsum[w];
+            }
+#pragma unroll
+            for (int j = 0; j < KP; ++j)
+                if (lv[j]) list[off++] = c0 + tid * KP + j;
+            base += tot;
+            __syncthreads();
+        }
+        if (tid == 0) { hdr[2 + to] = base; hdr[0] = to; }
+    }
+    if (tid == 0) p.map[0][1] = 0;
+}
+
 GsParams gs_params(const bd_conv_desc* d, int ph, int pw, int side = 0) {
     GsParams p{};
     p.C = side ? d->Cin : d->Cout; p.ppi = side ? d->in_pix_per_img : d->out_pix_per_img; p.ph = ph; p.pw_px = pw; p.nseg = d->nseg;
@@ -314,3 +411,51 @@
     BD_CHECK_LAUNCH("bd_gskip_map_scan");
     return BD_OK;
 }
+
+void bd_fwd_map_layout(const bd_conv_desc* d, BdFwdMap* out) {
+    const int p4 = gs_params(d, 4, 16, 0).total;
+    out->p4 = p4; out->live = FL_HDR; out->list = FL_HDR + p4;
+    out->ints = (size_t)FL_HDR + (size_t)3 * p4;
+}
+
+extern "C" size_t bd_fwd_live_map_bytes(const bd_conv_desc* d) {
+    if (!d || d->nseg < 1 || d->nseg > BD_MAX_SEGS || !(d->R == 3 && d->S == 3 && d->stride == 1 && d->pad == 1)) return 0;
+    BdFwdMap m;
+    bd_fwd_map_layout(d, &m);
+    return m.ints * sizeof(int);
+}
+
+extern "C" int bd_fwd_live_maps(const bd_conv_desc* d, const int32_t* labels, int A, int depths, void* const* maps, size_t map_bytes,
+                                int reset, bd_stream_t stream) {
+    BD_REQUIRE(d && labels && maps, "fwd_live_maps: null pointer");
+    const size_t need = bd_fwd_live_map_bytes(d);
+    BD_REQUIRE(need > 0, "fwd_live_maps: forward liveness maps belong to 3x3 / stride 1 / pad 1 descriptors");
+    BD_REQUIRE(A >= 1 && depths >= 1 && depths <= FL_MAX_DEPTH, "fwd_live_maps: A=%d depths=%d (1 .. %d)", A, depths, (int)FL_MAX_DEPTH);
+    BD_REQUIRE(map_bytes >= need, "fwd_live_maps: map %zu < required %zu bytes", map_bytes, need);
+    const GsParams g4 = gs_params(d, 4, 16, 0);
+    FlParams p{};
+    p.labels = labels; p.A = A; p.ppi = g4.ppi; p.nseg = g4.nseg; p.depths = depths; p.pi4 = g4.patches_per_img; p.tot4 = g4.total;
+    size_t lds = 0;
+    for (int s = 0; s < g4.nseg; ++s) {
+        BD_REQUIRE(d->Hi[s] == d->Ho[s] && d->Wi[s] == d->Wo[s], "fwd_live_maps: level %d changes size", s);
+        p.seg[s] = FlSeg{g4.seg[s].H, g4.seg[s].W, g4.seg[s].off, g4.seg[s].patch_start, g4.seg[s].pw};
+        const size_t b = (size_t)2 * g4.seg[s].H * g4.seg[s].W;
+        BD_REQUIRE((long long)g4.seg[s].H * g4.seg[s].W * A < 0x7fffffffll, "fwd_live_maps: level %d too large", s);
+        lds = b > lds ? b : lds;
+    }
+    BD_REQUIRE(lds <= 160 * 1024 - 256, "fwd_live_maps: a level of %zu pixels does not fit the LDS bitmap", lds / 2);
+    for (int k = 0; k < depths; ++k) {
+        BD_REQUIRE(maps[k], "fwd_live_maps: null map %d", k);
+        p.map[k] = (int*)maps[k];
+        if (reset && hipMemsetAsync(maps[k], 0, FL_HDR * sizeof(int), (hipStream_t)stream) != hipSuccess) {
+            bd_set_error("fwd_live_maps: memset failed");
+            return BD_ELAUNCH;
+        }
+    }
+    if (d->N < 1 || g4.total < 1) return BD_OK;
+    BD_ONCE_PER_DEVICE((void)hipFuncSetAttribute(reinterpret_cast<const void*>(&fwd_live_kernel), hipFuncAttributeMaxDynamicSharedMemorySize,
+                                                 160 * 1024 - 256));
+    hipLaunchKernelGGL(fwd_live_kernel, dim3(d->N * g4.nseg), dim3(1024), lds, (hipStream_t)stream, p);
+    BD_CHECK_LAUNCH("bd_fwd_live_maps");
+    return BD_OK;
+}
diff --git a/basedet_amd/csrc/image_ops.hip b/basedet_amd/csrc/image_ops.hip
--- a/basedet_amd/csrc/image_ops.hip
+++ b/basedet_amd/csrc/image_ops.hip
@@ -29,7 +29,7 @@
 static thread_local const char* g_bd_last_kernel = "";
 void bd_note_kernel(const char* name) { g_bd_last_kernel = name; }
 extern "C" const char* bd_conv_last_kernel(void) { return g_bd_last_kernel; }
-extern "C" int bd_version(void) { return 106; }
+extern "C" int bd_version(void) { return 107; }
 
 namespace {
 
diff --git a/basedet_amd/models/engine.py b/basedet_amd/models/engine.py
--- a/basedet_amd/models/engine.py
+++ b/basedet_amd/models/engine.py
@@ -50,6 +50,7 @@
         self._gskip_ws = None
         self._chain = (None, None, False)
         self._chain_cache = {}
+        self._fwd_map_cache = {}
         self.fp8 = False
         self.fp8_dgrad = False
         self.fp8_wgrad = False
@@ -179,8 +180,21 @@
     def set_chain(self, gmap=None, dxmap=None, dx_clean=False):
         self._chain = (gmap, dxmap, bool(dx_clean) and dxmap is not None) if self.gskip else (None, None, False)
 
-    def forward(self, x, gin, gout, y, add=None, relu=False, bits=None, x8=None, y8=None, q_scale=1.0):
+    def fwd_map_desc(self, gin: Geom, gout: Geom, fmap, clean):
+        d = self.desc(gin, gout)
+        key = (id(d), fmap.data_ptr(), bool(clean))
+        c = self._fwd_map_cache.get(key)
+        if c is None:
+            if len(self._fwd_map_cache) > 64:
+                self._fwd_map_cache.clear()
+            c = self._fwd_map_cache[key] = (ops.fwd_map_desc(d, fmap, clean), d)
+        return c[0]
+
+    def forward(self, x, gin, gout, y, add=None, relu=False, bits=None, x8=None, y8=None, q_scale=1.0, fwd_map=None, fwd_clean=False):
         flags = (ops.EPI_RELU if relu else 0) | (ops.EPI_ADD_BEFORE if add is not None else 0)
+        if fwd_map is not None:
+            assert not self.fp8 and not self.fp8_1x1 and bits is None and y8 is None
+            return ops.conv2d_fwd(self.fwd_map_desc(gin, gout, fwd_map, fwd_clean), x, self.w_fwd, self.b, y, add=add, flags=flags)
         if self.fp8_1x1 and x8 is not None and ops.conv1x1_fp8_ok(self.desc(gin, gout), 0):
             return ops.conv1x1_fp8(self.desc(gin, gout), 0, x8, self.w_q8, self.w_scale8, self.b, y, add=add, bits=bits, y8=y8,
                                    q_scale=q_scale, flags=flags)
diff --git a/basedet_amd/models/retinanet.py b/basedet_amd/models/retinanet.py
--- a/basedet_amd/models/retinanet.py
+++ b/basedet_amd/models/retinanet.py
@@ -39,6 +39,8 @@
             for c in self.box_tower + [self.bbox_pred]:
                 c.gskip = True
         self.sparse_chain = bool(m.get("SPARSE_BOX_CHAIN", True))
+        self.sparse_box_fwd = (bool(m.get("SPARSE_BOX_FWD", True)) and type(self) is RetinaNet and nc >= 1 and nc <= 8
+                               and all(c.gskip for c in self.box_tower + [self.bbox_pred]))
         self._build_base_anchors()
 
     def _head_convs(self):
@@ -68,6 +70,14 @@
             if nb:
                 pl.g_map = [C.empty(((nb + 3) // 4,), torch.int32) for _ in range(nc)]
         pl.chain_epoch = None
+        pl.f_map = None
+        if self.sparse_box_fwd:
+            nb = ops.fwd_live_map_bytes(self.box_tower[0].desc(pl.pyr, pl.pyr))
+            if nb:
+                pl.f_map = [C.empty(((nb + 3) // 4,), torch.int32) for _ in range(nc)]
+        pl.fwd_epoch = None
+        pl.fwd_skip = None
+        pl.fwd_skipped = False
         tw = lambda: C.empty((pl.pyr.pixels, ch), torch.uint8)
         pl.cls_act8 = [tw() if c.fp8 else None for c in self.cls_tower]
         pl.box_act8 = [tw() if c.fp8 else None for c in self.box_tower]
@@ -85,10 +95,20 @@
     def head_forward(self, pl):
         concurrent = bool(self.cfg.MODEL.get("HEAD_TOWERS_CONCURRENT", True)) and self.weight_dtype != "fp8_e4m3"
         side = self.streams.aux() if concurrent else None
+        skip, pl.fwd_skip = pl.fwd_skip, None
+        if skip is not None and side is None:
+            join(self.streams.aux_stream)
+        if skip is None:
+            pl.fwd_epoch = None
+        pl.fwd_skipped = skip is not None
         with fork(side):
             t, t8 = pl.P, getattr(pl, "P8", None)
-            for c, a, a8 in zip(self.box_tower, pl.box_act, pl.box_act8):
-                c.forward(t, pl.pyr, pl.pyr, a, relu=True, x8=t8, y8=a8); t, t8 = a, a8
+            for i, (c, a, a8) in enumerate(zip(self.box_tower, pl.box_act, pl.box_act8)):
+                if skip is not None:
+                    c.forward(t, pl.pyr, pl.pyr, a, relu=True, fwd_map=pl.f_map[i], fwd_clean=skip[0])
+                else:
+                    c.forward(t, pl.pyr, pl.pyr, a, relu=True, x8=t8, y8=a8)
+                t, t8 = a, a8
             self.bbox_pred.forward(t, pl.pyr, pl.pyr, pl.offsets, x8=t8)
         t, t8 = pl.P, getattr(pl, "P8", None)
         for c, a, a8 in zip(self.cls_tower, pl.cls_act, pl.cls_act8):
@@ -111,6 +131,11 @@
         with fork(side):
             ops.retina_assign_encode(pl.anchors, gt, num_gt, thr[0], thr[1], m.MATCHER.ALLOW_LOW_QUALITY, m.BOX_REG.MEAN,
                                      m.BOX_REG.STD, pl.labels, pl.match_idx, pl.gt_offsets, pl.num_fg, ws)
+            if pl.f_map is not None and self.streams.aux() is not None:
+                clean = pl.fwd_epoch == self.plan_arena.epoch
+                pl.fwd_epoch = self.plan_arena.epoch
+                ops.fwd_live_maps(self.box_tower[0].desc(pl.pyr, pl.pyr), pl.labels, self.num_anchors, pl.f_map[::-1], reset=not clean)
+                pl.fwd_skip = (clean,)
         self.network_forward(pl)
         join(side)
         pl.loss_buf.zero_()
@@ -160,6 +185,13 @@
         pl.g_P8_ready = pl.g_P8 is not None and bool(wrote_p)
 
     def _debug_head(self, pl, out, lvl):
+        if getattr(pl, "fwd_skipped", False):
+            t = pl.P
+            for c, a in zip(self.box_tower, pl.box_act):
+                c.forward(t, pl.pyr, pl.pyr, a, relu=True); t = a
+            self.bbox_pred.forward(t, pl.pyr, pl.pyr, pl.offsets)
+            pl.fwd_skipped = False
+            pl.fwd_epoch = None
         for i in range(pl.pyr.nlev):
             for k in range(len(self.cls_tower)):
                 out[f"cls{k}_{i}"] = lvl(pl.cls_act[k], i)
diff --git a/basedet_amd/ops.py b/basedet_amd/ops.py
--- a/basedet_amd/ops.py
+++ b/basedet_amd/ops.py
@@ -138,6 +138,27 @@
         h.gskip_dxmap = dxmap.data_ptr()
         h.gskip_dxmap_bytes = dxmap.numel() * dxmap.element_size()
     h.gskip_dx_clean = int(bool(dx_clean))
+    return h
+
+
+def fwd_live_map_bytes(d):
+    return int(L().bd_fwd_live_map_bytes(C.byref(d)))
+
+
+def fwd_live_maps(d, labels, A, maps, reset=False):
+    if labels.dtype != torch.int32 or labels.numel() != d.N * d.out_pix_per_img * A:
+        raise _lib.BasedetHipError(f"fwd_live_maps: labels must be int32 with N * pixels * A = {d.N * d.out_pix_per_img * A} entries")
+    nb = min(m.numel() * m.element_size() for m in maps)
+    arr = (C.c_void_p * len(maps))(*[ptr(m).value for m in maps])
+    check(L().bd_fwd_live_maps(C.byref(d), ptr(labels), int(A), len(maps), arr, nb, int(bool(reset)), stream_ptr()), "bd_fwd_live_maps")
+    return maps
+
+
+def fwd_map_desc(d, fmap, clean=False):
+    h = ConvDesc.from_buffer_copy(d)
+    h.fwd_map = fmap.data_ptr()
+    h.fwd_map_bytes = fmap.numel() * fmap.element_size()
+    h.fwd_clean = int(bool(clean))
     return h
 
 
diff --git a/include/basedet_hip.h b/include/basedet_hip.h
--- a/include/basedet_hip.h
+++ b/include/basedet_hip.h
@@ -43,6 +43,9 @@
     void* gskip_dxmap;
     size_t gskip_dxmap_bytes;
     int32_t gskip_dx_clean;
+    void* fwd_map;
+    size_t fwd_map_bytes;
+    int32_t fwd_clean;
 } bd_conv_desc;
 
 const char* bd_last_error_string(void);
@@ -61,6 +64,9 @@
 size_t bd_conv2d_dgrad_gskip_bytes(const bd_conv_desc* d);
 size_t bd_conv2d_gskip_map_bytes(const bd_conv_desc* d, int of_dx);
 int bd_gskip_map_scan(const bd_conv_desc* d, int of_dx, const void* t, void* map, size_t map_bytes, bd_stream_t stream);
+size_t bd_fwd_live_map_bytes(const bd_conv_desc* d);
+int bd_fwd_live_maps(const bd_conv_desc* d, const int32_t* labels, int A, int depths, void* const* maps, size_t map_bytes, int reset,
+                     bd_stream_t stream);
 
 int bd_conv2d_fwd_bits(const bd_conv_desc* d, const void* x, const void* w_packed, const float* bias, const void* add, void* y,
                        uint32_t* ybits, int flags, bd_stream_t stream);
```

New measurement: 722.1 images/sec (median of 6 runs). 1.04x the previous value.
